# Lymphatus/caesium-clt

Hardware: AMD Instinct MI355X
Metric: megapixels/sec JPEG q=80 1920x1080 batch (higher is better)
Workload: dtype int32

## Files before the change

caesium-clt_amd/binding.py:

```python
import ctypes as C
import os

_HERE = os.path.dirname(os.path.abspath(__file__))
NPHASES = 8
NKERNELS = 36
PHASE_NAMES = ["decode", "pixel", "masks_flags_runs", "stats_tables", "sizes_scan", "pack", "stuff_assemble", "reserved"]


class CCSParameters(C.Structure):
    _fields_ = [("keep_metadata", C.c_bool), ("jpeg_quality", C.c_uint32), ("jpeg_chroma_subsampling", C.c_uint32),
                ("jpeg_progressive", C.c_bool), ("jpeg_optimize", C.c_bool), ("jpeg_preserve_icc", C.c_bool),
                ("png_quality", C.c_uint32), ("png_optimization_level", C.c_uint32), ("png_force_zopfli", C.c_bool),
                ("png_optimize", C.c_bool), ("gif_quality", C.c_uint32), ("webp_quality", C.c_uint32), ("webp_lossless", C.c_bool),
                ("tiff_compression", C.c_uint32), ("tiff_deflate_level", C.c_uint32), ("width", C.c_uint32), ("height", C.c_uint32)]


class CCSResult(C.Structure):
    _fields_ = [("success", C.c_bool), ("code", C.c_uint32), ("error_message", C.c_char_p)]


class CByteArray(C.Structure):
    _fields_ = [("data", C.POINTER(C.c_uint8)), ("length", C.c_size_t)]


class Timing(C.Structure):
    _fields_ = [("total_ms", C.c_float), ("phase_ms", C.c_float * NPHASES), ("kernel_ms", C.c_float * NKERNELS), ("in_bytes", C.c_uint64), ("out_bytes", C.c_uint64),
                ("pixels", C.c_uint64), ("coef_bytes", C.c_uint64), ("n_images", C.c_uint32), ("n_failed", C.c_uint32), ("n_seq_decoded", C.c_uint32), ("n_par_fallback", C.c_uint32), ("n_par_short", C.c_uint32), ("n_prog_decoded", C.c_uint32), ("n_refine_chains", C.c_uint32), ("n_search_extra", C.c_uint32), ("n_fused_lists", C.c_uint32), ("n_list_refine", C.c_uint32), ("n_ac_in_lists", C.c_uint32), ("n_list_runs", C.c_uint32)]


class PngTiming(C.Structure):
    _fields_ = [("total_ms", C.c_float), ("kernel_ms", C.c_float * 16), ("in_bytes", C.c_uint64), ("out_bytes", C.c_uint64), ("pixels", C.c_uint64),
                ("raw_bytes", C.c_uint64), ("n_images", C.c_uint32), ("n_failed", C.c_uint32), ("n_trials", C.c_uint32)]


class CaesiumError(RuntimeError):
    def __init__(self, code, message):
        super().__init__(f"[{code}] {message}")
        self.code = code


def library_path():
    return os.path.join(_HERE, "libcaesium_hip.so")


EXPORTS = ["cs_default_parameters", "cs_compress_in_memory", "cs_compress_to_size_in_memory", "cs_convert_in_memory",
           "cs_batch_compress", "cs_batch_extent", "cs_free_bytes", "cs_free_result", "csh_device_count", "csh_last_error", "csh_kernel_name", "csh_kernel_name_webp", "csh_release_cached_memory", "csh_warmup", "csh_batch_create",
           "csh_batch_run", "csh_batch_fetch", "csh_batch_destroy", "csh_batch_retain_dct", "csh_batch_set_quality", "csh_batch_rerun_encode", "cs_batch_compress_to_size", "csh_batch_geometry", "csh_batch_read_coefs",
           "csp_kernel_name", "csp_batch_create", "csp_batch_create_webp", "csp_batch_create_pixels", "csh_batch_create_pixels", "csh_batch_pixels", "csh_batch_create_from_pixels", "csp_png_to_jpeg", "csp_png_to_lossless_webp", "csp_batch_run", "csp_batch_fetch", "csp_batch_destroy", "csp_batch_geometry", "csp_batch_read_rows", "csp_batch_read_stream",
           "csp_batch_trials", "csp_batch_read_scores", "csp_batch_chunk_bits", "csh_batch_create_webp", "cs_batch_convert",
           "cswd_batch_create", "cswd_batch_run", "cswd_batch_pixels", "cswd_batch_read_pixels", "cswd_batch_alpha", "cswd_batch_read_rgba", "cswd_batch_destroy", "cswd_batch_frames", "cswd_batch_read_canvas", "cswd_batch_encode_anim", "cswd_rgba_join", "cswd_rgba_destroy", "csh_batch_create_webp_from_pixels", "csh_batch_create_from_pixels_rgb", "csl_encode_pixels", "csl_attach_alpha"]


def _declare(L):
    P = C.POINTER
    L.cs_default_parameters.argtypes = [P(CCSParameters)]
    L.cs_default_parameters.restype = None
    L.cs_compress_in_memory.argtypes = [C.c_char_p, C.c_size_t, P(CCSParameters), P(CByteArray)]
    L.cs_compress_in_memory.restype = CCSResult
    L.cs_compress_to_size_in_memory.argtypes = [C.c_char_p, C.c_size_t, P(CCSParameters), C.c_size_t, C.c_bool, P(CByteArray)]
    L.cs_compress_to_size_in_memory.restype = CCSResult
    L.cs_convert_in_memory.argtypes = [C.c_char_p, C.c_size_t, P(CCSParameters), C.c_uint32, P(CByteArray)]
    L.cs_convert_in_memory.restype = CCSResult
    L.cs_batch_compress.argtypes = [P(CByteArray), C.c_size_t, P(CCSParameters), C.c_int, P(CByteArray), P(CCSResult)]
    L.cs_batch_extent.argtypes = [P(CByteArray), C.c_size_t]
    L.cs_batch_extent.restype = C.c_size_t
    L.cs_free_bytes.argtypes = [P(CByteArray)]
    L.cs_free_bytes.restype = None
    L.cs_free_result.argtypes = [P(CCSResult)]
    L.cs_free_result.restype = None
    L.csh_last_error.restype = C.c_char_p
    L.csh_kernel_name.argtypes = [C.c_int]
    L.csh_kernel_name.restype = C.c_char_p
    L.csh_kernel_name_webp.argtypes = [C.c_int]
    L.csh_kernel_name_webp.restype = C.c_char_p
    L.csh_batch_create.argtypes = [P(CByteArray), C.c_size_t, P(CCSParameters), C.c_int, P(C.c_void_p)]
    L.csh_batch_run.argtypes = [C.c_void_p, P(Timing)]
    L.csh_batch_fetch.argtypes = [C.c_void_p, P(CByteArray), P(CCSResult)]
    L.csh_batch_retain_dct.argtypes = [C.c_void_p, C.c_int]
    L.csh_batch_set_quality.argtypes = [C.c_void_p, P(C.c_uint32)]
    L.csh_batch_rerun_encode.argtypes = [C.c_void_p, P(Timing)]
    L.cs_batch_compress_to_size.argtypes = [P(CByteArray), C.c_size_t, P(CCSParameters), C.c_size_t, C.c_bool, C.c_int, P(CByteArray), P(CCSResult)]
    L.csh_batch_destroy.argtypes = [C.c_void_p]
    L.csh_batch_destroy.restype = None
    L.csh_batch_geometry.argtypes = [C.c_void_p, C.c_size_t, C.c_int, C.c_int, P(C.c_int), P(C.c_int), P(C.c_int), P(C.c_int)]
    L.csh_batch_read_coefs.argtypes = [C.c_void_p, C.c_size_t, C.c_int, C.c_int, C.c_void_p]
    L.csh_batch_create_webp.argtypes = [P(CByteArray), C.c_size_t, P(CCSParameters), C.c_int, P(C.c_void_p)]
    L.cs_batch_convert.argtypes = [P(CByteArray), C.c_size_t, P(CCSParameters), C.c_uint32, C.c_int, P(CByteArray), P(CCSResult)]
    L.csp_kernel_name.argtypes = [C.c_int]
    L.csp_kernel_name.restype = C.c_char_p
    L.csp_batch_create.argtypes = [P(CByteArray), C.c_size_t, P(CCSParameters), C.c_int, P(C.c_void_p)]
    L.csp_batch_run.argtypes = [C.c_void_p, P(PngTiming)]
    L.csp_batch_fetch.argtypes = [C.c_void_p, P(CByteArray), P(CCSResult)]
    L.csp_batch_destroy.argtypes = [C.c_void_p]
    L.csp_batch_destroy.restype = None
    L.csp_batch_geometry.argtypes = [C.c_void_p, C.c_size_t, P(C.c_uint32), P(C.c_uint32), P(C.c_uint32)]
    L.csp_batch_read_rows.argtypes = [C.c_void_p, C.c_size_t, C.c_void_p]
    L.csp_batch_read_stream.argtypes = [C.c_void_p, C.c_size_t, C.c_int, C.c_void_p]
    L.csp_batch_read_scores.argtypes = [C.c_void_p, C.c_size_t, C.c_void_p, P(C.c_int)]
    L.csp_batch_chunk_bits.argtypes = [C.c_void_p, C.c_size_t, C.c_int, P(C.c_uint64), C.c_size_t, P(C.c_size_t)]
    L.csp_batch_trials.argtypes = [C.c_void_p, C.c_size_t, P(C.c_int), P(C.c_uint64), P(C.c_int), P(C.c_int)]
    L.cswd_batch_create.argtypes = [P(CByteArray), C.c_size_t, C.c_int, P(C.c_void_p)]
    L.cswd_batch_run.argtypes = [C.c_void_p]
    L.cswd_batch_pixels.argtypes = [C.c_void_p, C.c_size_t, P(C.c_void_p), P(C.c_uint32), P(C.c_uint32), P(C.c_uint32), P(C.c_char_p)]
    L.cswd_batch_read_pixels.argtypes = [C.c_void_p, C.c_size_t, C.c_void_p]
    L.cswd_batch_alpha.argtypes = [C.c_void_p, C.c_size_t, P(C.c_void_p), P(C.c_void_p)]
    L.cswd_batch_read_rgba.argtypes = [C.c_void_p, C.c_size_t, C.c_void_p]
    L.cswd_batch_destroy.argtypes = [C.c_void_p]
    L.cswd_batch_destroy.restype = None
    L.cswd_batch_frames.argtypes = [C.c_void_p, C.c_size_t, P(C.c_uint32), P(C.c_uint32), P(C.c_uint32)]
    L.cswd_batch_read_canvas.argtypes = [C.c_void_p, C.c_size_t, C.c_uint32, C.c_void_p]
# ... 381 lines not shown
```

caesium-clt_amd/csrc/batch.hpp:

```cpp
#pragma once
#include <array>
#include <chrono>
#include <map>
#include <string>
#include <vector>

#include "../../include/caesium_hip.h"
#include "devmem.hpp"
#include "jpeg_host.hpp"
#include "kernels.h"
#include "webp_kernels.h"

namespace csh {

struct Item {
    int code = 0;
    std::string msg;
    JpegInfo in;
    JpegInfo out;
    int image = -1;
    size_t file_size = 0;
    std::vector<uint8_t> meta_out;
};

struct DecodePlan {
    PinnedBytes bits_pool;
    std::vector<DecScan> dscans;
    std::vector<DevHuffSet> hsets;
    std::vector<ParHuffSet> phsets;
    std::vector<char> phset_fits;
    std::vector<ParHuffSet4> phsets4;
    std::vector<std::array<int8_t, 8>> slot4;
    bool use4 = true;
    std::vector<ParScan> pscans;
    std::vector<uint32_t> need_seq_init;
    std::vector<ProgChain> chains;
    std::vector<int> chain_scans;
    std::vector<RefineUnit> refine_units;
    uint32_t refine_hist = 0, refine_pos = 0, refine_max_blocks = 0;
    uint32_t total_sub = 0, max_sub = 0, max_par_blocks = 0, dc_total = 0;

    DevBuf<uint8_t> d_bits, d_clean;
    DevBuf<ParScan> d_pscans;
    DevBuf<uint64_t> d_pstate, d_relax_list[2], d_unstuff_off, d_blk_off, d_dc_off;
    DevBuf<uint32_t> d_unstuff_cnt, d_nblk, d_need_seq, d_need_seq_init, d_relax_cnt, d_scan_pending, d_cut_block, d_claim;
    DevBuf<uint16_t> d_hyp;
    DevBuf<int32_t> d_dcdiff;
    DevBuf<DecScan> d_dscans;
    DevBuf<ProgChain> d_chains;
    DevBuf<int> d_chain_scans;
    DevBuf<uint64_t> d_refine_hist;
    DevBuf<uint32_t> d_refine_pos, d_refine_prog;
    DevBuf<RefineUnit> d_refine_units;
    DevBuf<DevHuffSet> d_hsets;
    DevBuf<ParHuffSet> d_phsets;
    DevBuf<ParHuffSet4> d_phsets4;
};

struct PixelPlan {
    std::vector<PlaneWork> pwork;
    std::vector<ResizeWork> rwork;
    std::vector<ResizeTap> rtaps;
    std::vector<float> rweights;
    uint64_t rgb_bytes = 0, tmp_floats = 0, max_tmp = 0, max_dst = 0;
    uint32_t max_row_in = 0, max_out_w = 0, max_nh = 0;
    uint32_t max_src_px = 0;
    uint64_t plane_bytes = 0, oplane_bytes = 0;
    uint32_t max_quads = 0;
    bool any_layout = false, any_layout_rgb = false;
    bool any_space_rgb = false;

    DevBuf<uint8_t> d_planes, d_oplanes, d_rgb;
    DevBuf<PlaneWork> d_pwork;
    DevBuf<ResizeWork> d_rwork;
    DevBuf<ResizeTap> d_rtaps;
    DevBuf<float> d_rweights, d_rtmp;
    DevBuf<int16_t> d_dct_raw;
};

struct Stage {
    uint32_t work0 = 0, nwork = 0, slot0 = 0, nslots = 0, ech0 = 0, nech = 0, table0 = 0, ntables = 0, plan0 = 0, nplans = 0, nzc0 = 0, nnzc = 0, ls0 = 0, nls = 0, ts0 = 0, nts = 0, rs0 = 0, nrs = 0, lr0 = 0, nlr = 0, rr0 = 0, nrr = 0;
    bool nz_build[2] = {true, true}, nz_filter[2] = {true, true};
};
struct SearchImg {
    int cand_work[64]; int ncand;
    int Al_luma = 0, Al_chroma = 0;
    uint64_t best_luma = 0, best_chroma = 0;
    int split_luma = 0, split_chroma = 0;
    bool luma_on = false, chroma_on = false;
    bool fixed = false;
};

struct EncodePlan {
    std::vector<EncScan> script;
    std::vector<ScanWork> swork;
    uint32_t nslots = 0, nlist_slots = 0, ntok_slots = 0;
    uint32_t nref_slots = 0;
    uint32_t last_run_refine = 0;
    uint32_t list_run = CSH_LIST_RUN;
    uint32_t nlist_runs = 0, nref_runs = 0;
    bool ac_runs_slot = false;
    uint32_t last_run_list_runs = 0;
    uint64_t total_corr = 0;
    uint64_t total_units = 0, total_words = 0;
    uint32_t max_units = 0;
    int ntables = 0;
    std::vector<TokPlan> plans;
    std::vector<int> plan_comp, plan_image;
    std::vector<EChunk> echunks;
    uint64_t tok_cap = 0;
    uint32_t tok_scale = 1;
    std::vector<TokRegion> regions;
    std::vector<uint32_t> region_est;
    uint32_t hist_rows = 0;
    std::vector<NzList> nzlists;
    std::vector<NzSet> nzsets;
    std::vector<int> nzset_of;
    std::vector<uint32_t> nzset_built;
    std::vector<int> nzset_comp, nzset_image;
    std::vector<NzChunk> nzchunks;
    std::vector<NzChunk> nzchunks_fused;
    uint32_t n_fused = 0;
    uint32_t last_run_fused = 0;
    uint32_t n_ac_lists = 0;
    uint32_t last_run_ac_lists = 0;
    std::vector<uint8_t> nzset_ac_lists;
    std::vector<uint32_t> nz_est, nz_worst;
    uint32_t nz_nrec = 0;
    uint64_t nz_cap = 0;
    bool search = false;
    enum { ST_1 = 0, ST_1B = 1, ST_2 = 2, ST_2B = 3, ST_2C = 4, ST_N = 5 };
    Stage stage[ST_N];
    void stage_begin(Stage &sg) {
        sg.work0 = uint32_t(swork.size()); sg.slot0 = nslots; sg.ech0 = uint32_t(echunks.size()); sg.table0 = uint32_t(ntables); sg.plan0 = uint32_t(plans.size());
        sg.nzc0 = uint32_t(nzchunks.size()); sg.ls0 = nlist_slots; sg.ts0 = ntok_slots; sg.rs0 = nref_slots; sg.lr0 = nlist_runs; sg.rr0 = nref_runs;
    }
    void stage_end(Stage &sg) {
        sg.nwork = uint32_t(swork.size()) - sg.work0; sg.nslots = nslots - sg.slot0; sg.nech = uint32_t(echunks.size()) - sg.ech0;
        sg.ntables = uint32_t(ntables) - sg.table0; sg.nplans = uint32_t(plans.size()) - sg.plan0;
        sg.nnzc = uint32_t(nzchunks.size()) - sg.nzc0; sg.nls = nlist_slots - sg.ls0; sg.nts = ntok_slots - sg.ts0; sg.nrs = nref_slots - sg.rs0; sg.nlr = nlist_runs - sg.lr0; sg.nrr = nref_runs - sg.rr0;
    }
    std::vector<SearchImg> simg;
    std::vector<uint8_t> work_active;
    uint32_t n_gated_runs = 0;
    std::vector<uint32_t> img_list, img_nlist, h_cost;
    std::map<std::array<int, 5>, int> cand_script;
    std::vector<uint8_t> hdr_pool;
    std::vector<uint32_t> hdr_off;

    DevBuf<uint8_t> d_hdr, d_tail, d_scan_tmp, d_work_active;
    DevBuf<EncScan> d_script;
    DevBuf<ScanWork> d_swork;
    DevBuf<uint32_t> d_slot_work;
    DevBuf<EChunk> d_echunks;
    DevBuf<SlotRec> d_slots;
    DevBuf<TokPlan> d_plans;
    DevBuf<uint64_t> d_corr, d_symbits, d_eobbits, d_tok_off, d_chunk_off, d_scan_raw_off;
    DevBuf<uint32_t> d_tok_cursor;
    DevBuf<TokRegion> d_regions;
    DevBuf<uint16_t> d_eobrun, d_slot_hist;
    DevBuf<uint32_t> d_img_list, d_img_nlist, d_scan_cost, d_slot_raw, d_slot_eobh, d_long_runs, d_long_cnt, d_tokens, d_chunk_ntok, d_chunk_bits, d_raw, d_scan_pad, d_chunk_ff, d_hdr_off;
    DevBuf<DevEncTable> d_tables;
    DevBuf<NzList> d_nzlists;
    DevBuf<NzSet> d_nzsets;
    DevBuf<NzChunk> d_nzchunks, d_nzchunks_fused;
    DevBuf<uint32_t> d_nz_pool, d_nz_cursor, d_nz_chunk_off, d_nz_chunk_cnt, d_list_slots, d_tok_slots, d_ref_slots, d_list_runs, d_ref_runs;
};

struct TrellisPlan {
    bool trellis = false, dering = false;
    Stage tstage;
    std::vector<TrellisWork> twork;
    std::vector<TrellisRun> truns;
    uint32_t t_units = 0, t_max_rows = 0;
    std::vector<uint32_t> trows;
    bool t_sort = false;
    bool nz_once = false;

    DevBuf<TrellisWork> d_twork;
    DevBuf<TrellisRun> d_truns;
    DevBuf<uint32_t> d_tqueue, d_trows, d_tperm, d_tspill;
    DevBuf<uint8_t> d_tblk_cnt;
    DevBuf<uint16_t> d_tblk_off;
    DevBuf<uint64_t> d_tlambda, d_tdcbt;
};

struct WebpTail {
    uint32_t webp_mb_bytes = 768;
    std::vector<csw::WebpImg> wimgs;
    uint64_t wwork_bytes = 0, wlevels = 0;
    uint32_t wmax_luma = 0, wmax_mbh = 0;

    DevBuf<csw::WebpImg> d_wimgs;
    DevBuf<uint8_t> d_wwork, d_wscratch, d_wprobs, d_wupdate;
    DevBuf<uint32_t> d_wpart, d_wstats;
    DevBuf<int16_t> d_wlevels;
};

struct Outputs {
    uint64_t raw_bytes_cap = 0, out_cap = 0;
    DevBuf<uint8_t> d_out;
    DevBuf<uint64_t> d_img_off;
    DevBuf<uint32_t> d_img_size, d_img_size_pad, d_status, d_overflow;
    std::vector<uint32_t> h_img_size;
    std::vector<uint64_t> h_img_off;
    std::vector<uint32_t> h_status;
    bool ran = false;
};

}

struct csh_batch {
    int device = 0;
    hipStream_t stream = 0;
    bool have_stream = false;
    CCSParameters params;
    std::vector<csh::Item> items;
    int nimg = 0;
    bool lossless = false;
    bool rgb_out = false;
    bool webp = false;
    int test_pool_shift = -1;
    bool progressive = true;
    bool retain_dct = false;
    bool have_dct = false;
    int q_base = 0;

    std::vector<csh::ImgDesc> imgs;
    std::vector<csh::DevQuant> quants;
    uint32_t ntiles = 0, ntiles_in = 0, ntiles_out = 0, max_tiles = 0, max_dummy = 0;
    csh::DevBuf<csh::ImgDesc> d_imgs;
    csh::DevBuf<csh::DevQuant> d_quants;
    csh::DevBuf<int16_t> d_coef;

    csh::DecodePlan dec;
    csh::PixelPlan pix;
    csh::EncodePlan enc;
    csh::TrellisPlan tr;
    csh::WebpTail wp;
    csh::Outputs out;

    ~csh_batch() { if (have_stream) { (void)hipStreamSynchronize(stream); (void)hipStreamDestroy(stream); } }
};

namespace csh {

enum KernelSlot {
    KS_MEMSET_COEF, KS_UNSTUFF, KS_DEC_SPEC, KS_DEC_RELAX0, KS_DEC_RELAX, KS_DEC_WRITE, KS_DC_SCATTER, KS_REFINE_CHAINS, KS_DECODE_PROG_SEQ,
    KS_IDCT_PLANE, KS_RESIZE, KS_XFORM_DIRECT, KS_RESAMPLE_FDCT, KS_FIX_DUMMY, KS_MEMSET_ENC, KS_TRELLIS_STATS, KS_TRELLIS_AC, KS_TRELLIS_DC,
    KS_NZLIST, KS_TOKENS, KS_LIST_STATS, KS_AC_RUNS, KS_GEN_TABLES, KS_CHUNK_SIZES, KS_SCAN_CHUNK_BITS, KS_SCAN_LAYOUT, KS_PACK, KS_LIST_PACK,
    KS_FF_COUNT, KS_SCAN_SEARCH, KS_LAYOUT, KS_SCAN_IMAGES, KS_EMIT, KS_SPARE0, KS_SPARE1, KS_SPARE2, KS_COUNT,
    KS_WEBP_YUV = KS_XFORM_DIRECT, KS_WEBP_ENCODE = KS_RESAMPLE_FDCT, KS_WEBP_ASSEMBLE = KS_FIX_DUMMY
};
struct KernelSlotRow { KernelSlot slot; const char *name; int phase; };
constexpr KernelSlotRow kKernelSlots[] = {
    {KS_MEMSET_COEF, "memset_coef", 0},        {KS_UNSTUFF, "unstuff", 0},                 {KS_DEC_SPEC, "k_dec_spec", 0},
    {KS_DEC_RELAX0, "k_dec_relax0", 0},        {KS_DEC_RELAX, "k_dec_relax1_4", 0},        {KS_DEC_WRITE, "k_dec_write", 0},
    {KS_DC_SCATTER, "k_dc_scatter", 0},        {KS_REFINE_CHAINS, "k_refine_chains", 0},   {KS_DECODE_PROG_SEQ, "k_decode_prog+seq", 0},
    {KS_IDCT_PLANE, "k_idct_plane", 1},        {KS_RESIZE, "resize", 1},                   {KS_XFORM_DIRECT, "k_xform_direct", 1},
    {KS_RESAMPLE_FDCT, "k_resample+k_plane_fdct", 1}, {KS_FIX_DUMMY, "k_fix_dummy", 1},    {KS_MEMSET_ENC, "memset_enc", 2},
    {KS_TRELLIS_STATS, "trellis_stats", 1},    {KS_TRELLIS_AC, "k_trellis_ac", 1},         {KS_TRELLIS_DC, "k_trellis_dc", 1},
    {KS_NZLIST, "k_nzlist", 2},                {KS_TOKENS, "k_tokens", 2},                 {KS_LIST_STATS, "k_list_stats", 2},
    {KS_AC_RUNS, "k_ac_runs", 2},              {KS_GEN_TABLES, "k_gen_tables", 3},         {KS_CHUNK_SIZES, "k_chunk_sizes", 4},
    {KS_SCAN_CHUNK_BITS, "scan_chunk_bits", 4}, {KS_SCAN_LAYOUT, "scan_layout", 4},        {KS_PACK, "k_pack", 5},
    {KS_LIST_PACK, "k_list_pack", 5},          {KS_FF_COUNT, "k_ff_count", 6},             {KS_SCAN_SEARCH, "scan_search_stage2", 7},
    {KS_LAYOUT, "k_layout", 6},                {KS_SCAN_IMAGES, "scan_images", 6},         {KS_EMIT, "k_emit", 6},
    {KS_SPARE0, "", 7},                        {KS_SPARE1, "", 7},                         {KS_SPARE2, "", 7}};
constexpr bool kernel_slots_in_order() {
    for (int i = 0; i < int(sizeof kKernelSlots / sizeof kKernelSlots[0]); i++) if (kKernelSlots[i].slot != i) return false;
    return true;
}
static_assert(sizeof kKernelSlots / sizeof kKernelSlots[0] == CSH_NKERNELS && int(KS_COUNT) == int(CSH_NKERNELS), "one row per csh_timing.kernel_ms slot");
static_assert(kernel_slots_in_order(), "row i of kKernelSlots describes slot i");

struct PlanSwitches {
    std::string profile;
    bool nz_once = true;
    bool tr_sort = true;
    int prog_par = -1;
    bool fused_420 = true;
    bool nz_fused = true;
    bool ref_list = true;
    uint32_t list_run = CSH_LIST_RUN;
    bool ac_runs_slot = false;
    bool ac_tiles = false;
    static PlanSwitches read();
};

struct Laps {
    const bool trace;
    std::chrono::steady_clock::time_point at = std::chrono::steady_clock::now();
    std::string text;
    Laps();
    void lap(const char *what);
};

struct BatchPlanner {
    csh_batch *const b;
    const CByteArray *const inputs;
    const size_t count;
    const CCSParameters *const p;
    const csp_pixels *const px;
    const PlanSwitches sw;
    const bool progressive;
    uint16_t qout_nat[64];
    int script_base3 = 0, script_base1 = 0;
    std::map<int, int> other_scripts;
    std::vector<std::pair<std::vector<uint8_t>, int>> hset_keys;
    std::map<std::vector<uint16_t>, int> quant_index;
    uint64_t plane_off = 64, oplane_off = 0;

    BatchPlanner(csh_batch *b, const CByteArray *inputs, size_t count, const CCSParameters *p, const csp_pixels *px);
    void begin();
    void parse();
    int reserve_pinned();
    int plan_image(size_t n);
    int plan_search_stages();
    int plan_trellis();
    void finish_descriptors();
    int upload(Laps &laps);

private:
    void image_geometry(Item &it, ImgDesc &im);
    int decode_scans(Item &it, ImgDesc &im, const uint8_t *d);
    int huff_set(const JScan &js);
    void place_blocks(ParScan &ps, const JpegInfo &in, const JScan &js, uint32_t units, bool dc_rows, bool subseqs);
    int sequential_split(const Item &it, const ImgDesc &im, const uint8_t *d, int img_index, bool &par_ok);
    bool progressive_plan(const Item &it, const ImgDesc &im, int img_index);
    void plane_work(ImgDesc &im, const JpegInfo &in, const JpegInfo &o, int img_index, bool resized);
    void resize_work(const JpegInfo &in, const JpegInfo &o, int img_index);
    void output_scans(Item &it, ImgDesc &im, int img_index, size_t in_len);
    void frame_header(Item &it);
    template <class Fill> int enc_scan(const std::array<int, 5> &key, Fill fill);
    int space_script(int ncomp, int space, int &ns);
    int cand_index(int comp, int Ss, int Se, int Ah, int Al, int cls = -1);
    int dc_scan_index(int ncomp);
    int seq1_index(int comp, int cls = -1);
    uint32_t nz_list(int img_index, int comp, int Al, const ImgDesc &im, size_t in_len);
    void add_works(Item &it, ImgDesc &im, int img_index, const std::vector<int> &list, size_t in_len, const JpegInfo &o, bool stats_only = false);
    template <class Make> void add_stage(int sid, Make make);
    template <class Add> void splits(const ImgDesc &im, Add &add, int i0, int i1, bool whole);
};

void layout_token_pool(csh_batch *b);

int run_once(csh_batch *b, csh_timing *t, bool requant_only);

int search_costs(csh_batch *b, AsmCtx &a, int stage);
uint32_t search_gate(csh_batch *b, int stage, int (*want)(const SearchImg &));
int search_decide(csh_batch *b, int stage);
int search_lists(csh_batch *b);

}
```

caesium-clt_amd/csrc/batch_plan.cpp:

```cpp
#include <algorithm>
#include <atomic>
#include <cmath>
#include <thread>

#include "batch.hpp"
#include "resize_host.h"
#include "result.h"

namespace csh {

static void build_dev_huff(const HuffSpec &h, DevHuff &d) {
    memset(&d, 0, sizeof d);
    for (int l = 0; l < 18; l++) d.maxcode[l] = -1;
    if (!h.present) return;
    int code = 0, p = 0;
    for (int l = 1; l <= 16; l++) {
        if (h.bits[l]) {
            d.valptr[l] = p - code;
            for (int i = 0; i < h.bits[l]; i++, p++, code++)
                if (l <= 9) {
                    int base = code << (9 - l);
                    for (int k = 0; k < (1 << (9 - l)); k++) d.look[(base + k) & 511] = uint16_t((l << 8) | h.vals[p]);
                }
            d.maxcode[l] = code - 1;
// ... 114 lines not shown
static int plan_item(Item &it, const CCSParameters &p, bool lossless, bool to_rgb) {
    const JpegInfo &in = it.in;
    if (in.ncomp != 1 && in.ncomp != 3 && in.ncomp != 4) { it.msg = "unsupported component count"; return CS_ERR_JPEG_FEATURE; }
    if (uint64_t(in.width) * uint64_t(in.height) > (1ull << 28)) { it.msg = "image dimensions too large for the device path"; return CS_ERR_JPEG_FEATURE; }
    const bool other_space = in.space != CSH_CS_GREY && in.space != CSH_CS_YCC;
    const bool converted = other_space && to_rgb;
    it.out = JpegInfo();
    JpegInfo &o = it.out;
    o.width = in.width; o.height = in.height; o.ncomp = converted ? 3 : in.ncomp;
    o.space = converted ? CSH_CS_YCC : in.space;
    if (other_space && !converted) { o.write_jfif = false; o.write_adobe = in.adobe_transform; }
    if (p.width || p.height) {
        if (lossless) { it.msg = "resize + lossless transcode not on the device path"; return CS_ERR_UNSUPPORTED; }
        csh_compute_dimensions(in.width, in.height, int(p.width), int(p.height), o.width, o.height);
        if (o.width > 65500 || o.height > 65500 || uint64_t(o.width) * uint64_t(o.height) > (1ull << 28)) { it.msg = "resize target too large for JPEG"; return CS_ERR_JPEG_FEATURE; }
    }
    if (in.ncomp >= 3 && (!lossless || in.ncomp == 4)) {
        int blocks = 0;
        for (int c = 0; c < in.ncomp; c++) {
            const JComp &k = in.comp[c];
            blocks += k.h * k.v;
            if (in.hmax % k.h || in.vmax % k.v) { it.msg = "fractional chroma sampling ratio (component factors do not divide the largest ones)"; return CS_ERR_JPEG_FEATURE; }
            if (in.hmax / k.h > 4 || in.vmax / k.v > 4) { it.msg = "chroma sampling ratio above 4"; return CS_ERR_JPEG_FEATURE; }
        }
        if (blocks > 10) { it.msg = "more than 10 blocks per MCU"; return CS_ERR_JPEG_FEATURE; }
    }
    if (lossless) {
        for (int c = 0; c < in.ncomp; c++)
            if (memcmp(in.comp[c].qt, in.qt[in.comp[c].tq], sizeof in.comp[c].qt)) { it.msg = "a component was decoded with a quantisation table that its slot no longer holds"; return CS_ERR_JPEG_FEATURE; }
        for (int c = 0; c < in.ncomp; c++) o.comp[c] = in.comp[c];
        jpeg_geometry(o);
        return 0;
    }
    int ss = int(p.jpeg_chroma_subsampling);
    if (ss == 0) ss = 420;
    static const char kRgbIds[] = "RGB", kCmykIds[] = "CMYK";
    for (int c = 0; c < o.ncomp; c++) {
        o.comp[c].id = o.space == CSH_CS_RGB ? kRgbIds[c] : (o.space == CSH_CS_CMYK ? kCmykIds[c] : c + 1);
        o.comp[c].h = o.comp[c].v = 1; o.comp[c].tq = table_class(o.space, c);
    }
    if (o.space == CSH_CS_YCC || o.space == CSH_CS_YCCK) {
        int h = 1, v = 1;
        if (ss == 420) { h = 2; v = 2; }
        else if (ss == 422) { h = 2; v = 1; }
        else if (ss == 411) { h = 4; v = 1; }
        else if (ss != 444) { it.msg = "unknown output chroma subsampling"; return CS_ERR_JPEG_FEATURE; }
        o.comp[0].h = h; o.comp[0].v = v;
        if (o.space == CSH_CS_YCCK) { o.comp[3].h = h; o.comp[3].v = v; }
    }
    jpeg_geometry(o);
    return 0;
}

void layout_token_pool(csh_batch *b) {
    b->enc.regions.resize(b->enc.region_est.size());
    if (b->test_pool_shift < 0) b->test_pool_shift = getenv("CSH_TEST_POOL_SHIFT") ? std::min(16, std::max(0, atoi(getenv("CSH_TEST_POOL_SHIFT")))) : 0;
    const int shift = b->test_pool_shift;
    uint64_t at = 0;
    for (size_t i = 0; i < b->enc.regions.size(); i++) {
        const uint64_t cap = std::min<uint64_t>(std::max<uint64_t>((uint64_t(b->enc.region_est[i]) * b->enc.tok_scale) >> shift, 64), 0xFFFFFFF0ull);
        b->enc.regions[i].base = at; b->enc.regions[i].cap = uint32_t(cap); b->enc.regions[i].pad = 0;
        at += (cap + 3) & ~uint64_t(3);
    }
    b->enc.tok_cap = at + 64;
    at = 0;
    for (size_t i = 0; i < b->enc.nzlists.size(); i++) {
        const uint64_t cap = std::min<uint64_t>(std::max<uint64_t>((uint64_t(b->enc.nz_est[i]) * b->enc.tok_scale) >> shift, 64), b->enc.nz_worst[i]);
        b->enc.nzlists[i].base = at; b->enc.nzlists[i].cap = uint32_t(cap);
        at += (cap + 3) & ~uint64_t(3);
    }
    b->enc.nz_cap = at + 64;
}

PlanSwitches PlanSwitches::read() {
    auto is = [](const char *name, const char *v) { const char *e = getenv(name); return e && !strcmp(e, v); };
    PlanSwitches s;
    const char *penv = getenv("CSH_PROFILE");
    s.profile = penv && *penv ? penv : "mozjpeg";
    s.nz_once = !is("CSH_NZ_ONCE", "0");
    s.tr_sort = !is("CSH_TR_SORT", "0");
    s.nz_fused = !is("CSH_NZ_FUSED", "0");
    s.ac_tiles = is("CSH_AC_TILES", "1");
    s.ref_list = is("CSH_REF_LIST", "1") || (s.ref_list && !is("CSH_REF_LIST", "0"));
    const char *pp = getenv("CSH_PROG_PAR");
    s.prog_par = pp && !strcmp(pp, "0") ? 0 : (pp && !strcmp(pp, "1") ? 1 : -1);
    s.fused_420 = !getenv("CSH_NO_FUSED_420");
    if (const char *lr = getenv("CSH_LIST_RUN")) { if (*lr) s.list_run = uint32_t(std::min(32, std::max(1, atoi(lr)))); }
    s.ac_runs_slot = is("CSH_AC_RUNS", "slot");
    return s;
}

Laps::Laps() : trace(getenv("CSH_TRACE") != nullptr) {}
void Laps::lap(const char *what) {
    if (!trace) return;
    const auto now = std::chrono::steady_clock::now();
    char buf[64];
    snprintf(buf, sizeof buf, " %s %.1f", what, std::chrono::duration<double, std::milli>(now - at).count());
    text += buf; at = now;
}

BatchPlanner::BatchPlanner(csh_batch *b_, const CByteArray *inputs_, size_t count_, const CCSParameters *p_, const csp_pixels *px_)
    : b(b_), inputs(inputs_), count(count_), p(p_), px(px_), sw(PlanSwitches::read()), progressive(p_->jpeg_progressive) {}

void BatchPlanner::begin() {
    b->items.resize(count);
    quality_table(int(p->jpeg_quality), qout_nat);
    DevQuant qo; make_quant(qout_nat, qo);
    b->quants.push_back(qo);
    b->q_base = int(b->quants.size()) - 1;
    for (int q = 1; q <= 100; q++) { uint16_t tq[64]; quality_table(q, tq); DevQuant dq; make_quant(tq, dq); b->quants.push_back(dq); }
    b->progressive = progressive;
    b->enc.list_run = sw.list_run;
    b->enc.ac_runs_slot = sw.ac_runs_slot;

    add_script(b->enc.script, 3, true, CSH_CS_YCC);
    add_script(b->enc.script, 1, true, CSH_CS_GREY);
    add_script(b->enc.script, 3, false, CSH_CS_YCC);
    add_script(b->enc.script, 1, false, CSH_CS_GREY);
    script_base3 = progressive ? 0 : 16; script_base1 = progressive ? 10 : 17;
    const bool webp = b->webp, rgb_out = b->rgb_out;
    const std::string &profile = sw.profile;
    b->enc.search = progressive && !webp && !rgb_out && profile != "plain";
    const bool lossy_jpeg = !b->lossless && !webp && !rgb_out;
    b->tr.trellis = lossy_jpeg && (profile == "mozjpeg" || profile == "mozjpeg-trellis");
    b->tr.dering = lossy_jpeg && (profile == "mozjpeg" || profile == "mozjpeg-dering");
    b->tr.nz_once = b->tr.trellis && progressive && sw.nz_once && sw.tr_sort;
}

template <class Fill>
int BatchPlanner::enc_scan(const std::array<int, 5> &key, Fill fill) {
    auto f = b->enc.cand_script.find(key);
    if (f != b->enc.cand_script.end()) return f->second;
    EncScan e;
    memset(&e, 0, sizeof e);
    fill(e);
    b->enc.script.push_back(e);
    return b->enc.cand_script[key] = int(b->enc.script.size()) - 1;
}
int BatchPlanner::space_script(int ncomp, int space, int &ns) {
    ns = progressive ? (space == CSH_CS_YCC ? 10 : 2 + 4 * ncomp) : 1;
    if (space == CSH_CS_YCC) return script_base3;
    if (space == CSH_CS_GREY) return script_base1;
    auto f = other_scripts.find(space);
    if (f == other_scripts.end()) {
        f = other_scripts.emplace(space, int(b->enc.script.size())).first;
        add_script(b->enc.script, ncomp, progressive, space);
    }
    return f->second;
}
int BatchPlanner::cand_index(int comp, int Ss, int Se, int Ah, int Al, int cls) {
    const int ycc = comp ? 1 : 0;
    if (cls < 0) cls = ycc;
    return enc_scan({cls == ycc ? comp : comp + 16 * (1 + cls), Ss, Se, Ah, Al}, [&](EncScan &e) {
        const int id = cls;
        e.ncomp = 1; e.comp[0] = comp; e.Ss = Ss; e.Se = Se; e.Ah = Ah; e.Al = Al;
        e.ntables = 1; e.dht_id[0] = 0x10 | id; e.sos_tdta[0] = id;
    });
}
int BatchPlanner::dc_scan_index(int ncomp) {
    return enc_scan({-ncomp, 0, 0, 0, 0}, [&](EncScan &e) {
        e.ncomp = ncomp;
        for (int k = 0; k < ncomp; k++) {
            e.comp[k] = k;
            const int id = k ? 1 : 0;
            int idx = -1;
            for (int t = 0; t < e.ntables; t++) if (e.dht_id[t] == id) idx = t;
            if (idx < 0) { idx = e.ntables; e.dht_id[e.ntables++] = id; }
            e.dc_tbl[k] = idx; e.sos_tdta[k] = id << 4;
        }
    });
}
int BatchPlanner::seq1_index(int comp, int cls) {
    const int ycc = comp ? 1 : 0;
    if (cls < 0) cls = ycc;
    return enc_scan({cls == ycc ? comp : comp + 16 * (1 + cls), 0, 63, -1, -1}, [&](EncScan &e) {
        const int id = cls;
        e.ncomp = 1; e.comp[0] = comp; e.Ss = 0; e.Se = 63; e.sequential = 1;
        e.ntables = 2; e.dht_id[0] = id; e.dht_id[1] = 0x10 | id; e.dc_tbl[0] = 0; e.ac_tbl[0] = 1; e.sos_tdta[0] = (id << 4) | id;
    });
}

static uint64_t blocks_of(const ImgDesc &im) {
    uint64_t n = 0;
    for (int k = 0; k < im.ncomp; k++) n += uint64_t(im.out[k].real_bw) * im.out[k].real_bh;
    return n;
}

uint32_t BatchPlanner::nz_list(int img_index, int comp, int Al, const ImgDesc &im, size_t in_len) {
    if (b->enc.nzset_of.size() < size_t(img_index + 1) * CSH_MAX_COMPS) b->enc.nzset_of.resize(size_t(img_index + 1) * CSH_MAX_COMPS, -1);
    int &si = b->enc.nzset_of[size_t(img_index) * CSH_MAX_COMPS + size_t(comp)];
    const uint32_t nu = uint32_t(im.out[comp].real_bw * im.out[comp].real_bh);
    if (si < 0) {
        NzSet S;
        memset(&S, 0, sizeof S);
        for (int L = 0; L < CSH_NZ_LEVELS; L++) S.list[L] = 0xFFFFFFFFu;
        S.cnt_base = 0xFFFFFFFFu;
        S.nunits = nu; S.real_bw = im.out[comp].real_bw; S.bw = im.out[comp].bw; S.tile_base = im.out[comp].tile_base;
        si = int(b->enc.nzsets.size());
        b->enc.nzsets.push_back(S); b->enc.nzset_built.push_back(0u); b->enc.nzset_comp.push_back(comp); b->enc.nzset_image.push_back(img_index);
    }
    const uint64_t blocks_all = blocks_of(im);
    static const uint32_t kShare[CSH_NZ_LEVELS] = {20, 16, 12, 9};
    for (int L : {0, Al}) {
        if (b->enc.nzsets[size_t(si)].list[L] != 0xFFFFFFFFu) continue;
        const uint32_t nch = (nu + 255) / 256;
        NzList R;
        memset(&R, 0, sizeof R);
        R.chunk0 = b->enc.nz_nrec; b->enc.nz_nrec += nch;
        b->enc.nzsets[size_t(si)].list[L] = uint32_t(b->enc.nzlists.size());
        b->enc.nzlists.push_back(R);
        const uint64_t est = uint64_t(in_len) * kShare[L] / 8 * nu / std::max<uint64_t>(1, blocks_all) + nu + 4ull * nch + 256;
        const uint64_t worst = uint64_t(nu) * 64 + 4ull * nch;
        b->enc.nz_est.push_back(uint32_t(std::min<uint64_t>(est, worst)));
        b->enc.nz_worst.push_back(uint32_t(std::min<uint64_t>(worst, 0xFFFFFFF0ull)));
    }
    return b->enc.nzsets[size_t(si)].list[Al];
}

void BatchPlanner::add_works(Item &it, ImgDesc &im, int img_index, const std::vector<int> &list, size_t in_len, const JpegInfo &o, bool stats_only) {
    const int w_first = int(b->enc.swork.size());
    uint32_t nz_need[CSH_MAX_COMPS] = {0, 0, 0}, nz_gate[CSH_MAX_COMPS] = {0, 0, 0};
    for (int sidx : list) {
        const EncScan &e = b->enc.script[sidx];
        ScanWork w;
        memset(&w, 0, sizeof w);
        w.image = img_index; w.scan = sidx;
        w.out_off = 0xFFFFFFFFu;
        const bool from_list = e.Ss > 0 && !e.sequential && e.Ah == 0;
        const bool ref_list = sw.ref_list && e.Ss > 0 && !e.sequential && e.Ah != 0;
        w.list = 0xFFFFFFFFu; w.rs_base = 0xFFFFFFFFu; w.lr_base = 0xFFFFFFFFu; w.rr_base = 0xFFFFFFFFu;
        if (from_list || ref_list) {
            if (e.Al >= CSH_NZ_LEVELS) { it.code = CS_ERR_JPEG_FEATURE; it.msg = "internal: output scan script outside what the list coder carries"; }
            else {
                w.list = nz_list(img_index, e.comp[0], e.Al, im, in_len);
                if (!nz_need[e.comp[0]]) nz_gate[e.comp[0]] = uint32_t(b->enc.swork.size());
                nz_need[e.comp[0]] |= 1u << e.Al;
            }
        }
        if (e.Ss == 0 && e.ncomp > 1) w.nunits = uint32_t(im.omcus_x * im.omcus_y);
        else w.nunits = uint32_t(im.out[e.comp[0]].real_bw * im.out[e.comp[0]].real_bh);
        w.unit_base = uint32_t(b->enc.total_units);
        b->enc.total_units += w.nunits;
        w.corr_base = 0xFFFFFFFFu;
        if (e.Ss > 0 && !e.sequential && e.Ah) { w.corr_base = uint32_t(b->enc.total_corr); b->enc.total_corr += w.nunits; }
        w.word_base = uint32_t(b->enc.total_words);
        if (e.Ss) b->enc.total_words += (w.nunits + 63) / 64;
        w.table_base = uint32_t(b->enc.ntables);
        b->enc.ntables += e.ntables;
        b->enc.max_units = std::max(b->enc.max_units, w.nunits);
        {
            const uint32_t nch = (w.nunits + 255) / 256;
            w.first_chunk = b->enc.nslots; b->enc.nslots += nch;
            w.hist_row0 = b->enc.hist_rows; b->enc.hist_rows += nch * uint32_t(e.ntables);
            uint32_t &cursor = (from_list && w.list != 0xFFFFFFFFu) ? b->enc.nlist_slots : b->enc.ntok_slots;
            w.ls_base = cursor; cursor += nch;
            if (ref_list && w.list != 0xFFFFFFFFu) { w.rs_base = b->enc.nref_slots; b->enc.nref_slots += nch; }
            const uint32_t nruns = (nch + b->enc.list_run - 1) / b->enc.list_run;
            if (from_list && w.list != 0xFFFFFFFFu) { w.lr_base = b->enc.nlist_runs; b->enc.nlist_runs += nruns; }
            if (ref_list && w.list != 0xFFFFFFFFu) { w.rr_base = b->enc.nref_runs; b->enc.nref_runs += nruns; }
        }
        if (e.Ss == 0 || e.sequential) {
            uint32_t blocks = 0;
            for (int k = 0; k < e.ncomp; k++) blocks += e.ncomp > 1 ? uint32_t(o.comp[e.comp[k]].h * o.comp[e.comp[k]].v) : 1u;
            const uint32_t per_unit = e.sequential ? blocks * 20u : (e.Ah ? (blocks + 14u) / 15u : blocks);
            for (uint32_t j = 0; j < (w.nunits + 255) / 256; j++) b->enc.echunks.push_back(EChunk{uint32_t(b->enc.swork.size()), 0, 1, j, 0, uint32_t(b->enc.region_est.size())});
            b->enc.region_est.push_back(stats_only ? 64u : w.nunits * per_unit + 64);
        }
        b->enc.swork.push_back(w);
    }
    for (int c = 0; c < im.ncomp; c++) {
        if (!nz_need[c]) continue;
        const int si = b->enc.nzset_of[size_t(img_index) * CSH_MAX_COMPS + size_t(c)];
        uint32_t levels = stats_only ? (nz_need[c] | 1u) : ((nz_need[c] | 1u) & ~b->enc.nzset_built[size_t(si)]);
        b->enc.nzset_built[size_t(si)] |= levels;
        if (!stats_only && b->tr.nz_once && (levels & 1u)) levels = (levels & ~1u) | CSH_NZ_COMPACT0;
        const uint32_t nu = b->enc.nzsets[size_t(si)].nunits;
        for (uint32_t j = 0; levels && j < (nu + 255) / 256; j++) b->enc.nzchunks.push_back(NzChunk{uint32_t(si), j, levels, nz_gate[c]});
    }
    for (int c = 0; c < im.ncomp; c++) {
        int nac = 0;
        for (int sidx : list) { const EncScan &e = b->enc.script[sidx]; if (e.Ss > 0 && !e.sequential && e.Ah && e.comp[0] == c) { nac++; if (e.Al > 3 && !sw.ref_list) nac = 99; } }
        const bool too_many = !sw.ref_list && nac > CSH_TK_MAXSLOT;
        if (too_many) { it.code = CS_ERR_JPEG_FEATURE; it.msg = "internal: output scan script outside what the token kernel carries"; }
        const uint32_t nu = uint32_t(im.out[c].real_bw * im.out[c].real_bh);
        if (!nac || too_many) continue;
        const uint64_t blocks_all = blocks_of(im);
        const uint64_t scripts = b->enc.search ? uint64_t(nac + 1) / 2 : 1;
        const uint64_t est = uint64_t(in_len) * 3 * scripts * nu / std::max<uint64_t>(1, blocks_all) + uint64_t(nu) * nac + 1024;
        if (sw.ref_list) {
            for (size_t k = 0; k < list.size(); k++) {
                const EncScan &e = b->enc.script[list[k]];
                if (e.Ss > 0 && !e.sequential && e.Ah && e.comp[0] == c && b->enc.swork[size_t(w_first) + k].rs_base != 0xFFFFFFFFu) b->enc.swork[size_t(w_first) + k].region = uint32_t(b->enc.region_est.size());
            }
            b->enc.region_est.push_back(stats_only ? 64u : uint32_t(std::min<uint64_t>(est, 0x3FFFFFFFu)));
            continue;
        }
        TokPlan P;
        memset(&P, 0, sizeof P);
        P.nunits = nu; P.real_bw = im.out[c].real_bw; P.bw = im.out[c].bw; P.tile_base = im.out[c].tile_base;
        P.work0 = 0xFFFFFFFFu;
        for (size_t k = 0; k < list.size(); k++) {
            const EncScan &e = b->enc.script[list[k]];
            if (!(e.Ss > 0 && !e.sequential && e.Ah && e.comp[0] == c)) continue;
            const ScanWork &w = b->enc.swork[size_t(w_first) + k];
            if (P.work0 == 0xFFFFFFFFu) P.work0 = uint32_t(w_first) + uint32_t(k);
            AcSlot &a = P.s[P.nslot++];
            a.unit_base = w.unit_base; a.word_base = w.word_base; a.first_chunk = w.first_chunk; a.table_base = w.table_base; a.nunits_work = w.nunits; a.corr_base = w.corr_base;
            a.Ss = uint8_t(e.Ss); a.Se = uint8_t(e.Se); a.Ah = uint8_t(e.Ah); a.Al = uint8_t(e.Al);
        }
        for (uint32_t j = 0; j < (nu + 255) / 256; j++) b->enc.echunks.push_back(EChunk{uint32_t(img_index), uint16_t(c), 0, j, uint32_t(b->enc.plans.size()), uint32_t(b->enc.region_est.size())});
        b->enc.region_est.push_back(stats_only ? 64u : uint32_t(std::min<uint64_t>(est, 0x3FFFFFFFu)));
        b->enc.plan_comp.push_back(c); b->enc.plan_image.push_back(img_index);
        b->enc.plans.push_back(P);
    }
}

void BatchPlanner::parse() {
    std::atomic<size_t> next{0};
    auto worker = [&]() {
        for (size_t n; (n = next++) < count;) {
            Item &it = b->items[n];
            it.file_size = inputs[n].length;
            int type = sniff(inputs[n].data, inputs[n].length);
            if (type == CS_TYPE_UNKN) { it.code = CS_ERR_UNKNOWN_TYPE; it.msg = "unknown file type"; }
            else if (type != CS_TYPE_JPEG) { it.code = CS_ERR_UNSUPPORTED; it.msg = "this input format has no device path in this build (built: JPEG, PNG)"; }
            else it.code = parse_jpeg(inputs[n].data, inputs[n].length, it.in, it.msg);
        }
    };
    size_t nthreads = std::min<size_t>(std::min<size_t>(16, std::max(1u, std::thread::hardware_concurrency())), (count + 15) / 16);
    std::vector<std::thread> pool;
    for (size_t t = 1; t < nthreads; t++) pool.emplace_back(worker);
    worker();
    for (auto &t : pool) t.join();
}

int BatchPlanner::reserve_pinned() {
    size_t total = 0;
    for (size_t n = 0; n < count; n++) total += inputs[n].length;
    if (total + total / 16 + (64u << 10) >= 0xF0000000ull) { csh_set_error("csh_batch_create: more than 3.75 GiB of input in one device batch (cs_batch_extent sizes groups)"); return CS_ERR_POOL_OVERFLOW; }
    if (!b->dec.bits_pool.reserve(total + total / 16 + (64u << 10))) { csh_set_error("out of pinned host memory"); return CS_ERR_NO_DEVICE; }
    return 0;
}

void BatchPlanner::image_geometry(Item &it, ImgDesc &im) {
    const JpegInfo &in = it.in, &o = it.out;
    im.width = in.width; im.height = in.height; im.ncomp = o.ncomp; im.ncomp_in = in.ncomp;
    im.mcus_x = in.mcus_x; im.mcus_y = in.mcus_y;
    im.progressive_in = in.progressive;
    for (int c = 0; c < in.ncomp; c++) {
        fill_geom(in.comp[c], im.in[c], b->ntiles_in);
        std::vector<uint16_t> key(in.comp[c].qt, in.comp[c].qt + 64);
        auto f = quant_index.find(key);
        if (f == quant_index.end()) {
            DevQuant q; make_quant(key.data(), q);
            f = quant_index.emplace(key, int(b->quants.size())).first;
            b->quants.push_back(q);
        }
        im.qt_in[c] = f->second;
        b->max_tiles = std::max<uint32_t>(b->max_tiles, im.in[c].ntiles);
    }
    for (int c = 0; c < o.ncomp; c++) {
        if (b->lossless) im.out[c] = im.in[c];
        else fill_geom(o.comp[c], im.out[c], b->ntiles_out);
        im.comp_id[c] = o.comp[c].id;
        im.qt_out[c] = 0;
        b->max_tiles = std::max<uint32_t>(b->max_tiles, im.out[c].ntiles);
        uint32_t nd = uint32_t(im.out[c].bw * im.out[c].bh - im.out[c].real_bw * im.out[c].real_bh);
        b->max_dummy = std::max(b->max_dummy, nd);
    }
    im.omcus_x = o.mcus_x; im.omcus_y = o.mcus_y;
    im.enc_w = o.width; im.enc_h = o.height;
// ... 529 lines not shown
    for (size_t i = 0; i < b->enc.nzsets.size(); i++) b->enc.nzsets[i].tile_base = b->imgs[size_t(b->enc.nzset_image[i])].out[b->enc.nzset_comp[i]].tile_base;
    {
        b->enc.nzchunks_fused = b->enc.nzchunks;
        const bool allowed = sw.nz_fused && !b->lossless && !b->webp && !b->rgb_out && !(b->tr.trellis && progressive && !b->tr.nz_once);
        std::vector<uint8_t> fused(b->enc.nzsets.size(), 0);
        const bool lists_only = progressive && !sw.ac_tiles && sw.ref_list && sw.nz_once && sw.tr_sort && (!b->tr.trellis || (b->tr.t_sort && b->tr.nz_once));
        std::vector<uint8_t> planned(b->enc.nzsets.size(), 0);
        for (size_t i = 0; i < b->enc.plans.size(); i++) {
            const size_t at = size_t(b->enc.plan_image[i]) * CSH_MAX_COMPS + size_t(b->enc.plan_comp[i]);
            if (at < b->enc.nzset_of.size() && b->enc.nzset_of[at] >= 0) planned[size_t(b->enc.nzset_of[at])] = 1;
        }
        b->enc.nzset_ac_lists.assign(b->enc.nzsets.size(), 0);
        for (PlaneWork &w : b->pix.pwork) {
            w.ac_lists = 0u;
            const size_t at = size_t(w.image) * CSH_MAX_COMPS + size_t(w.comp);
            const int si = allowed && at < b->enc.nzset_of.size() ? b->enc.nzset_of[at] : -1;
            if (si < 0) continue;
            const NzSet &S = b->enc.nzsets[size_t(si)];
            if (S.real_bw != S.bw || S.list[0] == 0xFFFFFFFFu) continue;
            w.nzset = uint32_t(si); fused[size_t(si)] = 1; b->enc.n_fused++;
            if (lists_only && !planned[size_t(si)]) { w.ac_lists = 1u; b->enc.nzset_ac_lists[size_t(si)] = 1; b->enc.n_ac_lists++; }
        }
        for (TrellisWork &tw : b->tr.twork) tw.ac_lists = (tw.nzset != 0xFFFFFFFFu && b->enc.nzset_ac_lists[tw.nzset]) ? 1u : 0u;
        for (NzChunk &ch : b->enc.nzchunks_fused) if (fused[ch.set]) ch.levels &= ~1u;
        auto flags = [&](Stage &sg) {
            for (int f = 0; f < 2; f++) {
                const std::vector<NzChunk> &v = f ? b->enc.nzchunks_fused : b->enc.nzchunks;
                sg.nz_build[f] = sg.nz_filter[f] = false;
                for (uint32_t i = sg.nzc0; i < sg.nzc0 + sg.nnzc; i++) { sg.nz_build[f] |= (v[i].levels & 1u) != 0u; sg.nz_filter[f] |= (v[i].levels & ~1u) != 0u; }
            }
        };
        for (Stage &sg : b->enc.stage) flags(sg);
        flags(b->tr.tstage);
    }
    for (ParScan &ps : b->dec.pscans)
        for (int m = 0; m < ps.nb_mcu && m < 10; m++) {
            int dcs = ps.dct[m] & 3, acs = 4 + (ps.act[m] & 3);
            if (b->dec.use4) { dcs = std::max<int>(0, b->dec.slot4[ps.huff_set][dcs]); acs = std::max<int>(0, b->dec.slot4[ps.huff_set][acs]); }
            ps.sel |= uint64_t(dcs | (acs << 3)) << (6 * m);
        }
    {
        std::vector<int> last(b->dec.chains.size(), -1);
        for (int s = 0;; s++) {
            bool any = false;
            for (size_t c = 0; c < b->dec.chains.size(); c++)
                if (b->dec.chains[c].refine && b->dec.chains[c].count > s) {
                    RefineUnit u; u.chain = int(c); u.s = s; u.prev = last[c];
                    last[c] = int(b->dec.refine_units.size());
                    b->dec.refine_units.push_back(u);
                    any = true;
                }
            if (!any) break;
        }
    }
    b->ntiles = b->ntiles_in + b->ntiles_out;
    b->pix.plane_bytes = plane_off;
    b->pix.oplane_bytes = oplane_off;
    b->out.out_cap = b->out.raw_bytes_cap;
    layout_token_pool(b);
}

int BatchPlanner::upload(Laps &laps) {
    hipStream_t st = b->stream;
    if (!b->nimg) return 0;
    b->dec.bits_pool.flush_copies();
    laps.lap("copy_in");
    if (b->dec.d_bits.alloc(b->dec.bits_pool.size()) || (b->dec.bits_pool.size() && hipMemcpyAsync(b->dec.d_bits.p, b->dec.bits_pool.p, b->dec.bits_pool.size(), hipMemcpyHostToDevice, st) != hipSuccess) ||
        b->d_imgs.upload(b->imgs, st) || b->dec.d_dscans.upload(b->dec.dscans, st) || b->dec.d_chains.upload(b->dec.chains, st) || b->dec.d_chain_scans.upload(b->dec.chain_scans, st) ||
        b->dec.d_hsets.upload(b->dec.hsets, st) || b->dec.d_phsets.upload(b->dec.phsets, st) || (b->dec.use4 && b->dec.d_phsets4.upload(b->dec.phsets4, st)) || b->d_quants.upload(b->quants, st) || b->pix.d_pwork.upload(b->pix.pwork, st) ||
        b->enc.d_script.upload(b->enc.script, st) || b->enc.d_swork.upload(b->enc.swork, st) || b->enc.d_slot_work.alloc(size_t(b->enc.nslots) + 1) || b->enc.d_slots.alloc(size_t(b->enc.nslots) + 1) || b->enc.d_plans.upload(b->enc.plans, st) || b->enc.d_echunks.upload(b->enc.echunks, st) || b->enc.d_hdr.upload(b->enc.hdr_pool, st) ||
        b->enc.d_hdr_off.upload(b->enc.hdr_off, st) || b->dec.d_pscans.upload(b->dec.pscans, st) || b->pix.d_rwork.upload(b->pix.rwork, st) || b->pix.d_rtaps.upload(b->pix.rtaps, st) ||
        b->pix.d_rweights.upload(b->pix.rweights, st) || b->pix.d_rgb.alloc(b->pix.rgb_bytes + 64) || b->pix.d_rtmp.alloc((resize_is_fused(b->pix.max_row_in) ? 0 : b->pix.tmp_floats) + 16) || b->dec.d_need_seq_init.upload(b->dec.need_seq_init, st))
        return CS_ERR_NO_DEVICE;
    size_t nchunks = b->dec.bits_pool.size() / 64 + 1, nst = size_t(b->dec.total_sub) + b->dec.pscans.size() + 1;
    if (b->dec.d_clean.alloc(b->dec.bits_pool.size() + 64) || b->dec.d_unstuff_cnt.alloc(nchunks + 1) || b->dec.d_unstuff_off.alloc(nchunks + 2) ||
        b->dec.d_pstate.alloc(nst) || b->dec.d_relax_list[0].alloc(nst) || b->dec.d_relax_list[1].alloc(nst) || b->dec.d_relax_cnt.alloc(512) || b->dec.d_scan_pending.alloc(b->dec.pscans.size() + 1) || b->dec.d_cut_block.alloc(b->dec.pscans.size() + 1) || b->dec.d_claim.alloc(size_t(b->dec.total_sub) + 1) || b->dec.d_hyp.alloc((size_t(b->dec.total_sub) + 1) * 10) ||
        b->dec.d_nblk.alloc(size_t(b->dec.total_sub) + 1) || b->dec.d_blk_off.alloc(size_t(b->dec.total_sub) + 2) || b->dec.d_need_seq.alloc(b->nimg + 1) ||
        b->dec.d_dcdiff.alloc(size_t(b->dec.dc_total) + 1) || b->dec.d_dc_off.alloc(size_t(b->dec.dc_total) + 2) ||
        b->dec.d_refine_hist.alloc(size_t(b->dec.refine_hist) + 1) || b->dec.d_refine_pos.alloc(size_t(b->dec.refine_pos) + 1) || b->dec.d_refine_units.upload(b->dec.refine_units, st) ||
        b->dec.d_refine_prog.alloc(b->dec.refine_units.size() + 1))
        return CS_ERR_NO_DEVICE;
    if (b->d_coef.alloc(size_t(b->ntiles) * CSH_TILE_I16) || b->pix.d_planes.alloc(b->pix.plane_bytes + 64) || b->pix.d_oplanes.alloc(b->pix.oplane_bytes + 64) ||
        b->enc.d_symbits.alloc(b->enc.total_words + 1) || b->enc.d_eobbits.alloc(b->enc.total_words + 1) ||
        b->enc.d_long_runs.alloc(2 * (b->enc.total_units / 512 + b->enc.swork.size() + 16)) || b->enc.d_long_cnt.alloc(4) || b->enc.d_tail.alloc(b->enc.total_units + 1) || b->enc.d_eobrun.alloc(b->enc.total_units + 1) || b->enc.d_corr.alloc(b->enc.total_corr + 1) ||
        b->enc.d_tok_off.alloc(4 * size_t(b->enc.nslots) + 4) || b->enc.d_chunk_ntok.alloc(4 * size_t(b->enc.nslots) + 4) || b->enc.d_slot_hist.alloc(size_t(b->enc.hist_rows) * 256 + 256) ||
        b->enc.d_slot_raw.alloc(size_t(b->enc.nslots) + 1) || b->enc.d_img_list.upload(b->enc.img_list, st) || b->enc.d_img_nlist.upload(b->enc.img_nlist, st) || b->enc.d_scan_cost.alloc(b->enc.swork.size() + 1) || b->enc.d_slot_eobh.alloc(16 * size_t(b->enc.nslots) + 16) || b->enc.d_chunk_bits.alloc(size_t(b->enc.nslots) + 1) || b->enc.d_chunk_off.alloc(size_t(b->enc.nslots) + 2) || b->enc.d_tok_cursor.alloc(b->enc.region_est.size() + 1) || b->enc.d_regions.upload(b->enc.regions, st) ||
        b->enc.d_tables.alloc(b->enc.ntables) || b->enc.d_scan_pad.alloc(b->enc.swork.size() + 1) ||
        b->enc.d_nzlists.upload(b->enc.nzlists, st) || b->enc.d_nzsets.upload(b->enc.nzsets, st) || b->enc.d_nzchunks.upload(b->enc.nzchunks, st) || (b->enc.n_fused && b->enc.d_nzchunks_fused.upload(b->enc.nzchunks_fused, st)) || b->enc.d_list_slots.alloc(size_t(b->enc.nlist_slots) + 1) || b->enc.d_tok_slots.alloc(size_t(b->enc.ntok_slots) + 1) || b->enc.d_ref_slots.alloc(size_t(b->enc.nref_slots) + 1) || b->enc.d_list_runs.alloc(size_t(b->enc.nlist_runs) + 1) || b->enc.d_ref_runs.alloc(size_t(b->enc.nref_runs) + 1) ||
        b->enc.d_nz_cursor.alloc(b->enc.nzlists.size() + 1) || b->enc.d_nz_chunk_off.alloc(size_t(b->enc.nz_nrec) + 1) || b->enc.d_nz_chunk_cnt.alloc(size_t(b->enc.nz_nrec) + 1) ||
        b->enc.d_scan_raw_off.alloc(b->enc.swork.size() + 2) || b->out.d_img_size.alloc(b->nimg + 1) || b->out.d_img_size_pad.alloc(b->nimg + 1) ||
        b->out.d_img_off.alloc(b->nimg + 2) || b->out.d_status.alloc(b->nimg) || b->out.d_overflow.alloc(4))
        return CS_ERR_NO_DEVICE;
    if (hipMemsetAsync(b->enc.d_slots.p, 0, (size_t(b->enc.nslots) + 1) * sizeof(SlotRec), st) != hipSuccess ||
        hipMemsetAsync(b->enc.d_slot_work.p, 0, (size_t(b->enc.nslots) + 1) * sizeof(uint32_t), st) != hipSuccess) { csh_set_error("hipMemsetAsync failed"); return CS_ERR_NO_DEVICE; }
    launch_make_slots(st, b->enc.d_swork.p, uint32_t(b->enc.swork.size()), b->enc.d_script.p, b->enc.d_nzlists.p, b->enc.d_slots.p, b->enc.d_slot_work.p, b->enc.d_list_slots.p, b->enc.d_tok_slots.p, b->enc.d_ref_slots.p, b->enc.d_list_runs.p, b->enc.d_ref_runs.p, b->enc.list_run);
    if (b->tr.trellis && (b->tr.d_trows.upload(b->tr.trows, st) || (b->tr.t_sort && (b->tr.d_tperm.alloc(size_t(b->tr.t_units) + 1) || b->tr.d_tblk_cnt.alloc(size_t(b->tr.t_units) + 1) || (b->tr.nz_once && b->tr.d_tblk_off.alloc(size_t(b->tr.t_units) + 1)))))) return CS_ERR_NO_DEVICE;
    if (b->tr.trellis && (b->tr.d_twork.upload(b->tr.twork, st) || b->tr.d_truns.upload(b->tr.truns, st) || b->tr.d_tqueue.alloc(1) || b->tr.d_tlambda.alloc(size_t(b->tr.t_units) + 1) || b->tr.d_tdcbt.alloc(size_t(b->tr.t_units) + 1) ||
                       b->tr.d_tspill.alloc(trellis_spill_words(trellis_ac_slots())) || b->pix.d_dct_raw.alloc(size_t(b->ntiles_out) * CSH_TILE_I16)))
        return CS_ERR_NO_DEVICE;
    for (size_t n = 0; px && n < count; n++) {
        const Item &it = b->items[n];
        if (it.image < 0) continue;
        const ResizeWork &rw = b->pix.rwork[size_t(it.image)];
        if (rw.image != it.image) { csh_set_error("internal: resize work out of order"); return CS_ERR_NO_DEVICE; }
        if (hipMemcpyAsync(b->pix.d_rgb.p + rw.rgb_src_off, px[n].device_pixels, size_t(px[n].width) * px[n].height * px[n].channels, hipMemcpyDeviceToDevice, st) != hipSuccess) { csh_set_error("pixel copy failed"); return CS_ERR_NO_DEVICE; }
    }
    laps.lap("alloc+enqueue");
    if (hipStreamSynchronize(st) != hipSuccess) { csh_set_error("upload failed"); return CS_ERR_NO_DEVICE; }
    laps.lap("upload_wait");
    return 0;
}

}
```

caesium-clt_amd/csrc/batch_run.cpp:

```cpp
#include <algorithm>

#include "batch.hpp"

namespace csh {
namespace {

class KernelMarks {
    hipEvent_t ev[CSH_NKERNELS + 1];
    int created = 0, next = 0;
    const hipStream_t st;

public:
    explicit KernelMarks(hipStream_t s) : st(s) {}
    KernelMarks(const KernelMarks &) = delete;
    KernelMarks &operator=(const KernelMarks &) = delete;
    ~KernelMarks() { for (int i = 0; i < created; i++) (void)hipEventDestroy(ev[i]); }
    int start() {
        for (; created <= CSH_NKERNELS; created++) CSH_CHECK(hipEventCreate(&ev[created]));
        CSH_CHECK(hipEventRecord(ev[0], st));
        return 0;
    }
    int claim(KernelSlot slot, hipEvent_t *e) {
        if (int(slot) != next || next >= CSH_NKERNELS) {
            csh_set_error("internal: timing mark '%s' out of order (slot %d is next)", slot < KS_COUNT ? kKernelSlots[slot].name : "?", next);
// ... 102 lines not shown
                eobrun_cleared = b->enc.d_eobrun.n != 0;
            }
            launch_dec_dense(st, 1, nps, b->dec.max_sub, da);
            da.zero_bytes = 0; da.zero2_bytes = 0;
            MARK(KS_DEC_RELAX0);
            const int kMaxRounds = int(b->dec.d_relax_cnt.n) - 2;
            int R = 0;
            for (int group = 12; nps && R < kMaxRounds; group = 8) {
                for (int g = 0; g < group && R < kMaxRounds; g++, R++)
                    launch_dec_relax_list(st, b->dec.d_clean.p, b->dec.d_pscans.p, b->dec.total_sub, da.huffs, da.compact, b->dec.d_pstate.p, b->dec.d_nblk.p, b->dec.d_relax_list[R & 1].p,
                                          b->dec.d_relax_cnt.p + R, b->dec.d_relax_list[(R & 1) ^ 1].p, b->dec.d_relax_cnt.p + R + 1, b->dec.d_pstate.n, b->dec.d_claim.p, uint32_t(R + 1));
                uint32_t left = 0;
                CSH_CHECK(hipMemcpyAsync(&left, b->dec.d_relax_cnt.p + R, sizeof left, hipMemcpyDeviceToHost, st));
                CSH_CHECK(hipStreamSynchronize(st));
                if (!left) break;
            }
            if (nps) {
                if (b->dec.d_scan_pending.zero(st)) return -1;
                launch_dec_mark_pending(st, b->dec.d_pscans.p, b->dec.total_sub, b->dec.d_relax_list[R & 1].p, b->dec.d_relax_cnt.p + R, b->dec.d_scan_pending.p);
                da.hyp = b->dec.d_hyp.p; da.scan_pending = b->dec.d_scan_pending.p;
                launch_dec_dense(st, 3, nps, b->dec.max_sub, da);
                launch_dec_chain(st, b->dec.d_pscans.p, nps, b->dec.d_pstate.p, b->dec.d_nblk.p, b->dec.d_hyp.p, b->dec.d_scan_pending.p, b->dec.d_need_seq.p);
            }
            MARK(KS_DEC_RELAX);
            if (nps) launch_exclusive_scan(st, b->dec.d_nblk.p, b->dec.d_blk_off.p, b->dec.total_sub, b->enc.d_scan_tmp.p, b->enc.d_scan_tmp.n);
            launch_dec_dense(st, 2, nps, b->dec.max_sub, da);
            MARK(KS_DEC_WRITE);
            if (nps) launch_exclusive_scan(st, reinterpret_cast<uint32_t *>(b->dec.d_dcdiff.p), b->dec.d_dc_off.p, b->dec.dc_total, b->enc.d_scan_tmp.p, b->enc.d_scan_tmp.n);
            launch_dc_scatter(st, b->dec.d_pscans.p, nps, b->dec.max_par_blocks, b->d_imgs.p, b->dec.d_dc_off.p, b->d_coef.p, b->dec.d_need_seq.p, b->dec.d_cut_block.p);
            launch_dc_refine(st, b->dec.d_clean.p, b->dec.d_pscans.p, nps, b->dec.max_par_blocks, b->d_imgs.p, b->d_coef.p, b->dec.d_need_seq.p);
            MARK(KS_DC_SCATTER);
        }
        launch_refine_chains(st, b->dec.d_clean.p, b->dec.d_pscans.p, b->dec.d_phsets.p, b->dec.d_dscans.p, b->dec.d_chains.p, b->dec.d_chain_scans.p, int(b->dec.chains.size()), b->dec.d_refine_units.p,
                             int(b->dec.refine_units.size()), b->dec.refine_max_blocks, b->d_imgs.p, b->d_coef.p, b->dec.d_need_seq.p, b->dec.d_refine_hist.p, b->dec.d_refine_pos.p, b->dec.d_refine_prog.p);
        MARK(KS_REFINE_CHAINS);
        launch_decode_prog(st, b->dec.d_clean.p, b->dec.d_pscans.p, b->dec.d_phsets.p, b->dec.d_dscans.p, b->dec.d_chains.p, b->dec.d_chain_scans.p, int(b->dec.chains.size()), b->d_imgs.p,
                           b->d_coef.p, b->dec.d_need_seq.p);
        launch_decode_seq(st, b->dec.d_bits.p, b->d_imgs.p, b->dec.d_dscans.p, b->dec.d_hsets.p, b->d_coef.p, nimg, b->dec.d_need_seq.p);
        MARK(KS_DECODE_PROG_SEQ);
        return 0;
    }

    int planes() {
        int nw = b->lossless ? 0 : int(b->pix.pwork.size());
        launch_idct_plane(st, b->d_imgs.p, b->pix.d_pwork.p, nw, b->max_tiles, b->d_quants.p, b->d_coef.p, b->pix.d_planes.p);
        MARK(KS_IDCT_PLANE);
        launch_resize(st, b->d_imgs.p, b->pix.d_rwork.p, int(b->pix.rwork.size()), b->pix.d_rtaps.p, b->pix.d_rweights.p, b->pix.d_planes.p, b->pix.d_rgb.p, b->pix.d_rtmp.p,
                      b->pix.max_src_px, b->pix.max_tmp, b->pix.max_dst, b->pix.max_row_in, b->pix.max_out_w, b->pix.max_nh, !(b->webp || b->rgb_out), b->pix.any_layout_rgb, b->pix.any_space_rgb);
        MARK(KS_RESIZE);
        return 0;
    }
    int pixels() {
        const int nw = b->lossless ? 0 : int(b->pix.pwork.size());
        int16_t *rawp = ((b->retain_dct || b->tr.trellis) && !b->lossless) ? b->pix.d_dct_raw.p : nullptr;
        NzFuse nzf;
        memset(&nzf, 0, sizeof nzf);
        fused = nw && b->enc.n_fused;
        if (fused) {
            if (b->enc.d_nz_cursor.zero(st) || b->enc.d_nz_chunk_cnt.zero(st)) return -1;
            nzf.nzsets = b->enc.d_nzsets.p; nzf.nzlists = b->enc.d_nzlists.p; nzf.nz_pool = b->enc.d_nz_pool.p; nzf.nz_cursor = b->enc.d_nz_cursor.p;
            nzf.nz_chunk_off = b->enc.d_nz_chunk_off.p; nzf.nz_chunk_cnt = b->enc.d_nz_chunk_cnt.p; nzf.overflow = b->out.d_overflow.p;
            nzf.blk_cnt = (b->tr.trellis && b->tr.t_sort) ? b->tr.d_tblk_cnt.p : nullptr;
            nzf.blk_off = (nzf.blk_cnt && b->tr.nz_once) ? b->tr.d_tblk_off.p : nullptr;
        }
        if (nw && getenv("CSH_DEBUG") && (uint32_t(atoi(getenv("CSH_DEBUG"))) & 32768u))
            CSH_CHECK(hipMemsetAsync(b->d_coef.p + size_t(b->ntiles_in) * CSH_TILE_I16, 0x5A, size_t(b->ntiles - b->ntiles_in) * CSH_TILE_I16 * sizeof(int16_t), st));
        launch_xform_direct(st, b->d_imgs.p, b->pix.d_pwork.p, nw, b->max_tiles, b->d_quants.p, b->d_coef.p, b->d_coef.p, rawp, b->ntiles_in, b->tr.dering, nzf);
        MARK(KS_XFORM_DIRECT);
        launch_resample_plane(st, b->d_imgs.p, b->pix.d_pwork.p, nw, b->pix.max_quads, b->pix.d_planes.p, b->pix.d_oplanes.p);
        if (b->pix.any_layout) launch_resample_any(st, b->d_imgs.p, b->pix.d_pwork.p, nw, b->pix.max_quads, b->pix.d_planes.p, b->pix.d_oplanes.p);
        launch_plane_fdct(st, b->d_imgs.p, b->pix.d_pwork.p, nw, b->max_tiles, b->d_quants.p, b->pix.d_oplanes.p, b->d_coef.p, rawp, b->ntiles_in, b->tr.dering, nzf);
        launch_resample_fdct_420(st, b->d_imgs.p, b->pix.d_pwork.p, nw, b->max_tiles, b->d_quants.p, b->pix.d_planes.p, b->d_coef.p, rawp, b->ntiles_in, b->tr.dering, nzf);
        MARK(KS_RESAMPLE_FDCT);
        if (!b->lossless) launch_fix_dummy(st, b->d_imgs.p, nimg, b->max_dummy, b->d_coef.p);
        MARK(KS_FIX_DUMMY);
        return 0;
    }

    void fill_enc_ctx() {
        memset(&c, 0, sizeof c);
        c.imgs = b->d_imgs.p; c.script = b->enc.d_script.p; c.work = b->enc.d_swork.p; c.nwork = int(b->enc.swork.size());
        c.echunks = b->enc.d_echunks.p; c.plans = b->enc.d_plans.p; c.nechunks = uint32_t(b->enc.echunks.size()); c.slot_work = b->enc.d_slot_work.p; c.slots = b->enc.d_slots.p; c.nslots = b->enc.nslots;
        c.coef = b->d_coef.p; c.sym_bits = b->enc.d_symbits.p; c.eob_bits = b->enc.d_eobbits.p; c.tail = b->enc.d_tail.p;
        c.eobrun = b->enc.d_eobrun.p; c.long_runs = b->enc.d_long_runs.p; c.long_cnt = b->enc.d_long_cnt.p; c.corr = b->enc.d_corr.p;
        c.tokens = b->enc.d_tokens.p; c.regions = b->enc.d_regions.p; c.tok_cursor = b->enc.d_tok_cursor.p; c.tok_off = b->enc.d_tok_off.p; c.chunk_ntok = b->enc.d_chunk_ntok.p; c.slot_hist = b->enc.d_slot_hist.p; c.slot_raw = b->enc.d_slot_raw.p; c.slot_eobh = b->enc.d_slot_eobh.p;
        c.chunk_bits = b->enc.d_chunk_bits.p; c.chunk_off = b->enc.d_chunk_off.p; c.tables = b->enc.d_tables.p;
        c.raw = b->enc.d_raw.p; c.raw_words = raw_chunks * 16; c.status = b->out.d_status.p; c.overflow = b->out.d_overflow.p;
        c.nzlists = b->enc.d_nzlists.p; c.nzsets = b->enc.d_nzsets.p; c.nz_pool = b->enc.d_nz_pool.p; c.nz_cursor = b->enc.d_nz_cursor.p; c.nz_chunk_off = b->enc.d_nz_chunk_off.p; c.nz_chunk_cnt = b->enc.d_nz_chunk_cnt.p;
        c.debug = getenv("CSH_DEBUG") ? uint32_t(atoi(getenv("CSH_DEBUG"))) : 0u;
    }
    void fill_asm_ctx() {
        memset(&a, 0, sizeof a);
        a.imgs = b->d_imgs.p; a.script = b->enc.d_script.p; a.work = b->enc.d_swork.p; a.nimg = nimg;
        a.nwork = b->tr.trellis ? int(b->tr.tstage.work0) : c.nwork;
        a.tables = b->enc.d_tables.p; a.chunk_off = b->enc.d_chunk_off.p; a.scan_pad_bytes = b->enc.d_scan_pad.p; a.scan_raw_off = b->enc.d_scan_raw_off.p;
        a.raw = b->enc.d_raw.p; a.raw_chunks = raw_chunks; a.chunk_ff = b->enc.d_chunk_ff.p;
        a.hdr_pool = b->enc.d_hdr.p; a.hdr_off = b->enc.d_hdr_off.p; a.img_size = b->out.d_img_size.p; a.img_size_pad = b->out.d_img_size_pad.p;
        a.img_off = b->out.d_img_off.p; a.out = b->out.d_out.p; a.out_cap = b->out.out_cap; a.status = b->out.d_status.p; a.overflow = b->out.d_overflow.p;
        a.img_list = b->enc.d_img_list.p; a.img_nlist = b->enc.d_img_nlist.p; a.scan_cost = b->enc.d_scan_cost.p;
    }
    void fill_trellis_ctx(TrellisCtx &tc) {
        memset(&tc, 0, sizeof tc);
        tc.imgs = b->d_imgs.p; tc.quant = b->d_quants.p; tc.work = b->tr.d_twork.p; tc.nwork = int(b->tr.twork.size()); tc.runs = b->tr.d_truns.p; tc.nruns = uint32_t(b->tr.truns.size());
        tc.tables = b->enc.d_tables.p; tc.raw = b->pix.d_dct_raw.p; tc.raw_tile0 = b->ntiles_in; tc.coef = b->d_coef.p; tc.dcrec = b->tr.d_tlambda.p; tc.dcbt = b->tr.d_tdcbt.p;
        tc.spill = b->tr.d_tspill.p; tc.nslots = uint32_t(b->tr.d_tspill.n / trellis_spill_words(1)); tc.max_rows = b->tr.t_max_rows;
        tc.queue = b->tr.d_tqueue.p;
        tc.rows = b->tr.d_trows.p; tc.nrows = uint32_t(b->tr.trows.size());
        if (b->tr.t_sort) { tc.blk_cnt = b->tr.d_tblk_cnt.p; tc.perm = b->tr.d_tperm.p; }
        if (b->tr.t_sort && b->tr.nz_once) {
            tc.nz_pool = b->enc.d_nz_pool.p; tc.nzlists = b->enc.d_nzlists.p; tc.nzsets = b->enc.d_nzsets.p; tc.nz_chunk_off = b->enc.d_nz_chunk_off.p; tc.nz_chunk_cnt = b->enc.d_nz_chunk_cnt.p;
            tc.blk_off = b->tr.d_tblk_off.p;
        }
        tc.ac_lists = fused ? 1u : 0u;
        tc.debug = getenv("CSH_TR_DEBUG") ? uint32_t(atoi(getenv("CSH_TR_DEBUG"))) : 0u;
    }

    int encode_begin() {
        fill_enc_ctx();
        launch_reset_works(st, b->enc.d_swork.p, c.nwork);
        if (!fused && (b->enc.d_nz_cursor.zero(st) || b->enc.d_nz_chunk_cnt.zero(st))) return -1;
        if (b->enc.d_symbits.zero(st) || b->enc.d_eobbits.zero(st) || (!eobrun_cleared && b->enc.d_eobrun.zero(st)) || b->enc.d_tables.zero(st) || b->enc.d_tok_cursor.zero(st) || b->enc.d_slot_eobh.zero(st) || b->enc.d_scan_pad.zero(st)) return -1;
#ifdef CSH_EMUL
        if (b->enc.d_raw.zero(st)) return -1;
#else
        if ((c.debug & 8192u) && b->enc.d_raw.zero(st)) return -1;
#endif
        MARK(KS_MEMSET_ENC);
        return 0;
    }

    void count_list_runs(const Stage &sg, bool gate) {
        for (uint32_t wi = sg.work0; (sg.nlr || sg.nrr) && wi < sg.work0 + sg.nwork; wi++) {
            const ScanWork &w = b->enc.swork[wi];
            if ((w.lr_base != 0xFFFFFFFFu || w.rr_base != 0xFFFFFFFFu) && (!gate || b->enc.work_active[wi])) b->enc.last_run_list_runs += ((w.nunits + 255u) / 256u + b->enc.list_run - 1u) / b->enc.list_run;
        }
    }

    void set_stage(const Stage &sg) {
        c.echunks = b->enc.d_echunks.p + sg.ech0; c.nechunks = sg.nech; c.slot0 = sg.slot0; c.nslots = sg.nslots;
        c.nzchunks = (fused ? b->enc.d_nzchunks_fused.p : b->enc.d_nzchunks.p) + sg.nzc0; c.nnzchunks = sg.nnzc;
        c.nz_build = sg.nz_build[fused ? 1 : 0]; c.nz_filter = sg.nz_filter[fused ? 1 : 0];
        c.list_slots = b->enc.d_list_slots.p + sg.ls0; c.nlist_slots = sg.nls; c.tok_slots = b->enc.d_tok_slots.p + sg.ts0; c.ntok_slots = sg.nts;
        c.ref_slots = b->enc.d_ref_slots.p + sg.rs0; c.nref_slots = sg.nrs;
        c.list_runs = b->enc.d_list_runs.p + sg.lr0; c.nlist_runs = sg.nlr; c.ref_runs = b->enc.d_ref_runs.p + sg.rr0; c.nref_runs = sg.nrr; c.list_run = b->enc.list_run;
        c.ac_runs_slot = b->enc.ac_runs_slot ? 1u : 0u;
    }

    int trellis() {
        const Stage &tg = b->tr.tstage;
        set_stage(tg);
        c.stats_only = 1;
        if (b->enc.d_long_cnt.zero(st)) return -1;
        c.nz_blk_cnt = b->tr.t_sort ? b->tr.d_tblk_cnt.p : nullptr;
        c.nz_blk_off = (b->tr.t_sort && b->tr.nz_once) ? b->tr.d_tblk_off.p : nullptr;
        launch_nzlist(st, c);
        c.nz_blk_cnt = nullptr; c.nz_blk_off = nullptr;
        if (b->tr.t_sort) {
            TrellisCtx ts;
            memset(&ts, 0, sizeof ts);
            ts.work = b->tr.d_twork.p; ts.nwork = int(b->tr.twork.size()); ts.blk_cnt = b->tr.d_tblk_cnt.p; ts.perm = b->tr.d_tperm.p;
            launch_trellis_sort(st, ts);
        }
        launch_tokens(st, c);
        launch_list_stats(st, c);
        count_list_runs(tg, false);
        launch_ac_runs(st, c);
        launch_gen_tables(st, b->enc.d_tables.p + tg.table0, int(tg.ntables));
        c.stats_only = 0;
        if (b->enc.d_nz_cursor.zero(st)) return -1;
        MARK(KS_TRELLIS_STATS);
        TrellisCtx tc;
        fill_trellis_ctx(tc);
        if (b->tr.d_tqueue.zero(st)) return -1;
        launch_trellis_ac(st, tc);
        MARK(KS_TRELLIS_AC);
        launch_trellis_dc(st, tc);
        launch_fix_dummy(st, b->d_imgs.p, nimg, b->max_dummy, b->d_coef.p);
        MARK(KS_TRELLIS_DC);
        return 0;
    }

    int stage(const Stage &sg, bool mark, bool gate) {
#define SMARK(slot) do { if (mark) MARK(slot); } while (0)
        set_stage(sg);
        c.work_active = gate ? b->enc.d_work_active.p : nullptr;
        a.work0 = int(sg.work0); a.nwork_run = int(sg.nwork);
        if (b->enc.d_long_cnt.zero(st)) return -1;
        launch_nzlist(st, c);
        SMARK(KS_NZLIST);
        launch_list_refine(st, c);
        for (uint32_t wi = sg.work0; sg.nrs && wi < sg.work0 + sg.nwork; wi++)
            if (b->enc.swork[wi].rs_base != 0xFFFFFFFFu && (!gate || b->enc.work_active[wi])) b->enc.last_run_refine++;
        count_list_runs(sg, gate);
        launch_tokens(st, c);
        SMARK(KS_TOKENS);
        launch_list_stats(st, c);
        SMARK(KS_LIST_STATS);
        launch_ac_runs(st, c);
        SMARK(KS_AC_RUNS);
        launch_gen_tables(st, b->enc.d_tables.p + sg.table0, int(sg.ntables));
        SMARK(KS_GEN_TABLES);
        launch_chunk_sizes(st, c);
        SMARK(KS_CHUNK_SIZES);
        launch_exclusive_scan(st, b->enc.d_chunk_bits.p + sg.slot0, b->enc.d_chunk_off.p + sg.slot0, sg.nslots, b->enc.d_scan_tmp.p, b->enc.d_scan_tmp.n);
        SMARK(KS_SCAN_CHUNK_BITS);
        launch_scan_sizes(st, a);
        launch_exclusive_scan(st, b->enc.d_scan_pad.p, b->enc.d_scan_raw_off.p, uint64_t(a.nwork), b->enc.d_scan_tmp.p, b->enc.d_scan_tmp.n);
        launch_scan_place(st, a);
        launch_zero_edges(st, c);
        SMARK(KS_SCAN_LAYOUT);
        launch_pack(st, c);
        SMARK(KS_PACK);
        launch_list_pack(st, c);
        SMARK(KS_LIST_PACK);
        launch_ff_count(st, a);
        SMARK(KS_FF_COUNT);
#undef SMARK
        return 0;
    }

    int gated_stage(int sid, int (*want)(const SearchImg &)) {
        if (!search_gate(b, sid, want)) return 0;
        b->enc.n_gated_runs++;
        if (b->enc.d_work_active.upload(b->enc.work_active, st)) return -1;
        if (stage(b->enc.stage[sid], false, true) || search_costs(b, a, sid)) return -1;
        return search_decide(b, sid);
    }
    int search() {
        b->enc.n_gated_runs = 0;
        if (search_costs(b, a, EncodePlan::ST_1) || search_decide(b, EncodePlan::ST_1)) return -1;
        if (gated_stage(EncodePlan::ST_1B, [](const SearchImg &si) { return si.luma_on ? 1 : 0; })) return -1;
        if (stage(b->enc.stage[EncodePlan::ST_2], false, false)) return -1;
        if (search_costs(b, a, EncodePlan::ST_2) || search_decide(b, EncodePlan::ST_2)) return -1;
        for (int sid : {int(EncodePlan::ST_2B), int(EncodePlan::ST_2C)})
            if (gated_stage(sid, [](const SearchImg &si) { return (si.luma_on ? 1 : 0) | (si.chroma_on ? 2 : 0); })) return -1;
        if (search_lists(b)) return -1;
        return 0;
    }

    int emit() {
        MARK(KS_SCAN_SEARCH);
        launch_layout(st, a);
        MARK(KS_LAYOUT);
        launch_exclusive_scan(st, b->out.d_img_size_pad.p, b->out.d_img_off.p, uint64_t(nimg), b->enc.d_scan_tmp.p, b->enc.d_scan_tmp.n);
        MARK(KS_SCAN_IMAGES);
        launch_emit(st, a);
        MARK(KS_EMIT);
        return 0;
    }

    int finish(bool phases) {
        CSH_CHECK(hipStreamSynchronize(st));
        CSH_CHECK(hipGetLastError());
        if (t && marks.read(t, phases)) return -1;
        if (t && !phases) t->n_images = uint32_t(nimg);
        return 0;
    }

    int webp() {
        const int nwimg = int(b->wp.wimgs.size());
        uint64_t out_bytes = 0;
        std::vector<uint64_t> off(size_t(b->nimg) + 1, 0);
        for (auto &wi : b->wp.wimgs) {
            const uint64_t cap = 4096 + uint64_t(wi.mbw) * wi.mbh * (b->wp.webp_mb_bytes + 2);
            wi.out_cap = uint32_t(std::min<uint64_t>(cap, 0xFFFFFF00u)); wi.out_off = out_bytes;
            off[wi.image] = out_bytes;
            out_bytes += (wi.out_cap + 63) & ~uint64_t(63);
            const int q = int(b->params.webp_quality);
            wi.quality = q < 0 ? 0 : q > 100 ? 100 : q;
        }
        off[b->nimg] = out_bytes;
        if (b->out.d_out.n < out_bytes + 64 && b->out.d_out.alloc(out_bytes + 64)) return -1;
        if ((b->wp.d_wscratch.n < out_bytes + 64 && b->wp.d_wscratch.alloc(out_bytes + 64)) || (b->wp.d_wpart.n < size_t(b->nimg) * 9 + 9 && b->wp.d_wpart.alloc(size_t(b->nimg) * 9 + 9)) ||
            (b->wp.d_wstats.n < size_t(b->nimg) * 2112 + 8 && (b->wp.d_wstats.alloc(size_t(b->nimg) * 2112 + 8) || b->wp.d_wprobs.alloc(size_t(b->nimg) * 1056 + 8) || b->wp.d_wupdate.alloc(size_t(b->nimg) * 1056 + 8))))
            return -1;
        if (b->wp.d_wstats.zero(st)) return -1;
        if (b->wp.d_wimgs.upload(b->wp.wimgs, st) || (b->wp.d_wwork.n < b->wp.wwork_bytes + 64 && b->wp.d_wwork.alloc(b->wp.wwork_bytes + 64)) ||
            (b->wp.d_wlevels.n < b->wp.wlevels + 64 && b->wp.d_wlevels.alloc(b->wp.wlevels + 64)))
            return -1;
        CSH_CHECK(hipMemcpyAsync(b->out.d_img_off.p, off.data(), off.size() * sizeof(uint64_t), hipMemcpyHostToDevice, st));
        if (b->out.d_img_size.zero(st)) return -1;
        csw::launch_webp_yuv(st, b->wp.d_wimgs.p, nwimg, b->wp.wmax_luma, b->pix.d_rgb.p, b->wp.d_wwork.p);
        MARK(KS_WEBP_YUV);
        hipEvent_t mid;
        if (marks.claim(KS_WEBP_ENCODE, &mid)) return -1;
        if (csw::launch_webp_encode(st, b->wp.wimgs.data(), nwimg, b->wp.d_wimgs.p, b->wp.d_wwork.p, b->wp.d_wlevels.p, b->wp.d_wscratch.p, b->wp.d_wpart.p, b->out.d_out.p, b->out.d_img_size.p, b->out.d_status.p, mid)) return -1;
        MARK(KS_WEBP_ASSEMBLE);
        return finish(false);
    }
};

}

int run_once(csh_batch *b, csh_timing *t, bool requant_only) {
    Run r(b, t);
    b->enc.last_run_list_runs = 0;
    b->enc.last_run_fused = 0; b->enc.last_run_refine = 0; b->enc.last_run_ac_lists = 0;
    if (r.pools() || r.marks.start()) return -1;
    const bool from_pixels = requant_only && b->tr.dering;
    if (requant_only && !from_pixels) {
        if (r.requant()) return -1;
    } else {
        if (from_pixels ? r.skip_decode() : r.decode()) return -1;
        if (r.planes()) return -1;
        if (b->webp) return r.webp();
        if (b->rgb_out) return (r.marks.mark(KS_XFORM_DIRECT) || r.finish(false)) ? -1 : 0;
        if (r.pixels()) return -1;
    }
    if (r.encode_begin()) return -1;
    b->enc.last_run_fused = r.fused ? b->enc.n_fused : 0u;
    b->enc.last_run_ac_lists = r.fused ? b->enc.n_ac_lists : 0u;
    if (b->tr.trellis ? r.trellis() : r.marks.skip_to(KS_NZLIST)) return -1;
    r.fill_asm_ctx();
    if (r.stage(b->enc.stage[0], true, false)) return -1;
    if (b->enc.search && r.search()) return -1;
    return (r.emit() || r.finish(true)) ? -1 : 0;
}

}
```

caesium-clt_amd/csrc/k_aclist.hip:

```cpp
#include "kernels.h"
#include "wave.h"

namespace csh {

#define CSH_LP_WORDS 1024

__device__ __forceinline__ static uint32_t lbitlen(uint32_t v) { return 32u - uint32_t(__clz(v)); }
__device__ __forceinline__ static int lwave() { return int(threadIdx.x) / CSP_WAVE_THREADS; }

#define CSH_NZ_HALF 16
__device__ __forceinline__ static uint4 nz_load(const EncCtx &c, const NzSet &S, uint32_t u, int bx, int by, uint32_t oct) {
    uint4 q; q.x = q.y = q.z = q.w = 0u;
    if (u < S.nunits) {
        const int b = by * S.bw + bx;
        q = *reinterpret_cast<const uint4 *>(c.coef + (size_t(S.tile_base) + size_t(b >> 6)) * CSH_TILE_I16 + size_t((b & 63) * CSH_BLK_STRIDE) + size_t(oct) * CSH_OCT_STRIDE);
    }
    return q;
}
__device__ __forceinline__ static uint32_t nz_mask8(const uint4 &q, uint32_t oct) {
    uint32_t m = 0;
    m |= (q.x & 0xFFFFu) ? 1u : 0u;   m |= (q.x >> 16) ? 2u : 0u;
    m |= (q.y & 0xFFFFu) ? 4u : 0u;   m |= (q.y >> 16) ? 8u : 0u;
    m |= (q.z & 0xFFFFu) ? 16u : 0u;  m |= (q.z >> 16) ? 32u : 0u;
    m |= (q.w & 0xFFFFu) ? 64u : 0u;  m |= (q.w >> 16) ? 128u : 0u;
    return oct ? m : (m & ~1u);
}
__device__ __forceinline__ static void nz_load_half(const EncCtx &c, const NzSet &S, uint32_t u0, int half, LV<uint4> (&q)[CSH_NZ_HALF]) {
    LFOR(l) {
        const uint32_t oct = uint32_t(l & 7);
        uint32_t u = u0 + 128u * uint32_t(half) + uint32_t(l >> 3);
        int by = int(u) / S.real_bw, bx = int(u) - by * S.real_bw;
        CSH_UNROLL
        for (int s = 0; s < CSH_NZ_HALF; s++) {
            q[s][l] = nz_load(c, S, u, bx, by, oct);
            u += 8u; bx += 8;
            while (bx >= S.real_bw) { bx -= S.real_bw; by++; }
        }
    }
}
__device__ __forceinline__ static void nz_count_half(const NzSet &S, uint32_t u0, int half, const LV<uint4> (&q)[CSH_NZ_HALF], LV<uint32_t> &cnt) {
    LFOR(l) {
        const uint32_t oct = uint32_t(l & 7);
        uint32_t n = 0;
        CSH_UNROLL
        for (int s = 0; s < CSH_NZ_HALF; s++)
            n += uint32_t(__popc(nz_mask8(q[s][l], oct))) + ((oct == 7u && u0 + 128u * uint32_t(half) + 8u * uint32_t(s) + uint32_t(l >> 3) < S.nunits) ? 1u : 0u);
        cnt[l] += n;
    }
}
__device__ __forceinline__ static void nz_write_half(const NzSet &S, uint32_t u0, int half, const LV<uint4> (&q)[CSH_NZ_HALF], uint32_t *dst, uint32_t run, uint8_t *blk_cnt, uint16_t *blk_off) {
    CSH_UNROLL
    for (int s = 0; s < CSH_NZ_HALF; s++) {
        LV<uint32_t> mk, cl;
        LFOR(l) {
            const uint32_t oct = uint32_t(l & 7);
            mk[l] = nz_mask8(q[s][l], oct);
            cl[l] = uint32_t(__popc(mk[l])) + ((oct == 7u && u0 + 128u * uint32_t(half) + 8u * uint32_t(s) + uint32_t(l >> 3) < S.nunits) ? 1u : 0u);
        }
        uint32_t tot;
        const LV<uint32_t> ex = lscan(cl, tot);
        if (blk_cnt) {
            LV<uint32_t> first = ex;
            for (int d = 0; d < 7; d++) first = lprev(first, 0u);
            LFOR(l) {
                const uint32_t blk = 16u * 8u * uint32_t(half) + 8u * uint32_t(s) + uint32_t(l >> 3);
                if ((l & 7) == 7 && u0 + blk < S.nunits) blk_cnt[u0 + blk] = uint8_t(ex[l] + cl[l] - 1u - first[l]);
                if ((l & 7) == 7 && u0 + blk < S.nunits && blk_off) blk_off[u0 + blk] = uint16_t(run + first[l]);
            }
        }
        LFOR(l) {
            const uint32_t oct = uint32_t(l & 7);
            const uint32_t blk = 16u * 8u * uint32_t(half) + 8u * uint32_t(s) + uint32_t(l >> 3);
            const uint32_t base = (8u * oct) | (blk << 23);
            const uint32_t w[4] = {q[s][l].x, q[s][l].y, q[s][l].z, q[s][l].w};
            uint32_t o = run + ex[l];
            CSH_UNROLL
            for (int i = 0; i < 8; i++)
                if ((mk[l] >> i) & 1u) {
                    const int h = (i & 1) ? (int(w[i >> 1]) >> 16) : (int(w[i >> 1] << 16) >> 16);
                    const uint32_t a = h == -32768 ? 32767u : uint32_t(h < 0 ? -h : h);
                    dst[o++] = (base + uint32_t(i)) | (h < 0 ? 128u : 0u) | (a << 8);
                }
            if (oct == 7u && u0 + blk < S.nunits) dst[o] = CSH_NZ_END | (base & 0x7F800000u);
        }
// ... 392 lines not shown
                }
            }
            pos += tot;
            const uint32_t done = uint32_t(pos >> 5) - ww;
            if (done > CSH_LP_WORDS - 640) {
                CSP_WAVE_SYNC();
                LFOR(l) for (uint32_t q = uint32_t(l); q < done; q += 64) {
                    const uint32_t v = buf[q];
                    if (first_flush && q == 0) { if (v) atomicOr(out + ww, v); } else out[ww + q] = v;
                }
                const uint32_t partial = buf[done];
                CSP_WAVE_SYNC();
                LFOR(l) for (int q = l; q < CSH_LP_WORDS; q += 64) buf[q] = (q == 0) ? partial : 0u;
                CSP_WAVE_SYNC();
                ww += done; first_flush = false;
            }
        }
    }
#ifdef CSH_EMUL
    {
        const uint64_t want = (raw_bit0 & 31u) + (c.chunk_off[cs0 + nrun] - c.chunk_off[cs0]) + pad;
        if (c.overflow[1] ? pos > want : pos != want) { fprintf(stderr, "k_list_pack: a run does not end where its sizes say\n"); abort(); }
    }
#endif
    CSP_WAVE_SYNC();
    const uint32_t last = uint32_t((pos + 31) >> 5) - ww;
    LFOR(l) for (uint32_t q = uint32_t(l); q < last; q += 64) {
        const uint32_t v = buf[q];
        if ((first_flush && q == 0) || q == last - 1) { if (v) atomicOr(out + ww + q, v); } else out[ww + q] = v;
    }
}

struct RefCarry { uint32_t runH, runN, base, prevN, prevNZ; };
__device__ __forceinline__ static uint32_t ref_isN(uint32_t e, uint32_t Ss, uint32_t Se) { const uint32_t k = e & 127u; return (k >= Ss && k <= Se && ((e >> 8) & 0x7FFFu) == 1u) ? 1u : 0u; }
__device__ __forceinline__ static uint32_t ref_isH(uint32_t e, uint32_t Ss, uint32_t Se) { const uint32_t k = e & 127u; return (k >= Ss && k <= Se && ((e >> 8) & 0x7FFFu) >= 2u) ? 1u : 0u; }
__device__ __forceinline__ static uint32_t ref_same(uint32_t key, uint32_t blk) { return (key >> 6) == blk + 1u ? (key & 63u) : 0u; }
template <bool WITH_ZQ>
__device__ __forceinline__ static void ref_step(const LV<uint32_t> (&e)[4], uint32_t Ss, uint32_t Se, RefCarry &C, LV<uint32_t> (&hex)[4], LV<uint32_t> (&z)[4], LV<uint32_t> (&zp)[4],
                                                LV<uint32_t> (&zq)[4]) {
    LV<uint32_t> cnt;
    LFOR(l) {
        uint32_t s = 0;
        CSH_UNROLL
        for (int q = 0; q < 4; q++) s += ref_isH(e[q][l], Ss, Se) | (ref_isN(e[q][l], Ss, Se) << 16);
        cnt[l] = s;
    }
    uint32_t tot;
    const LV<uint32_t> ex = lscan(cnt, tot);
    LV<uint32_t> kb[4];
    LFOR(l) {
        uint32_t ph = C.runH + (ex[l] & 0xFFFFu), pn = C.runN + (ex[l] >> 16);
        CSH_UNROLL
        for (int q = 0; q < 4; q++) {
            kb[q][l] = (e[q][l] & CSH_NZ_END) ? ((ph << 14) | pn) + 1u : 0u;
            hex[q][l] = ph; z[q][l] = pn;
            ph += ref_isH(e[q][l], Ss, Se); pn += ref_isN(e[q][l], Ss, Se);
        }
    }
    C.runH += tot & 0xFFFFu; C.runN += tot >> 16;
    lscan_last4(kb, C.base);
    LFOR(l) {
        CSH_UNROLL
        for (int q = 0; q < 4; q++) {
            const uint32_t b = kb[q][l] ? kb[q][l] - 1u : 0u, blk = (e[q][l] >> 23) & 255u, nz = ref_isH(e[q][l], Ss, Se) | ref_isN(e[q][l], Ss, Se);
            const uint32_t h = hex[q][l] - (b >> 14), n = z[q][l] - (b & 0x3FFFu);
            hex[q][l] = h;
            z[q][l] = nz ? (e[q][l] & 127u) - Ss - h - n : 0u;
            const uint32_t key = ((blk + 1u) << 6) | z[q][l];
            zp[q][l] = ref_isN(e[q][l], Ss, Se) ? key : 0u;
            if (WITH_ZQ) zq[q][l] = nz ? key : 0u;
        }
    }
    lscan_last4(zp, C.prevN);
    if (WITH_ZQ) lscan_last4(zq, C.prevNZ);
    LFOR(l) {
        CSH_UNROLL
        for (int q = 0; q < 4; q++) {
            const uint32_t blk = (e[q][l] >> 23) & 255u;
            zp[q][l] = ref_same(zp[q][l], blk);
            if (WITH_ZQ) zq[q][l] = ref_same(zq[q][l], blk);
        }
    }
}
__global__ void __launch_bounds__(256, 5) k_list_refine(EncCtx c) {
    CSH_SHARED alignas(16) uint32_t s_hist[4][4][256];
    CSH_SHARED uint32_t s_lastn[4][256];
    CSH_SHARED uint32_t s_nh[4][256];
    CSH_SHARED uint32_t s_corr[4][256][2];
    const int wv = int(uni(uint32_t(lwave())));
    const uint32_t idx = blockIdx.x * 4u + uint32_t(wv);
    if (idx >= c.nref_runs) return;
    const uint32_t cs0 = c.ref_runs[idx];
    const SlotRec r = c.slots[cs0];
    if (c.work_active && !c.work_active[r.work]) return;
    const uint32_t nrun = run_chunks(c, r);
    const uint64_t lbase = c.nzlists[r.nzlist].base;
    ListSlot nx = list_chunk(c, lbase, r.nzrec);
    const TokRegion rg = c.regions[r.region];
    uint32_t *hist = &s_hist[wv][0][0], *lastn = s_lastn[wv], *nh = s_nh[wv], *corr = &s_corr[wv][0][0];
    LFOR(l) {
        uint4 zero; zero.x = zero.y = zero.z = zero.w = 0u;
        for (int i = 4 * l; i < 1024; i += 256) *reinterpret_cast<uint4 *>(hist + i) = zero;
    }
    const uint32_t Ss = r.Ss, Se = r.Se;
    LV<uint32_t> freq[4];
    LFOR(l) { freq[0][l] = 0u; freq[1][l] = 0u; freq[2][l] = 0u; freq[3][l] = 0u; }
    for (uint32_t ci = 0; ci < nrun; ci++) {
        const ListSlot ls = nx;
        if (ci + 1u < nrun) nx = list_chunk(c, lbase, r.nzrec + ci + 1u);
        const uint32_t cs = cs0 + ci, j = r.j + ci, unit0 = r.unit0 + 256u * ci, corr0 = r.corr0 + 256u * ci, hist_row = r.hist_row + ci * uint32_t(r.ntables);
        const uint32_t left = r.nunits_work - 256u * j, nun = left < 256u ? left : 256u;
        CSP_WAVE_SYNC();
        LFOR(l) for (int i = l; i < 256; i += 64) { lastn[i] = 0u; nh[i] = 0u; corr[2 * i] = 0u; corr[2 * i + 1] = 0u; }
        CSP_WAVE_SYNC();
        RefCarry C;
        C.runH = C.runN = C.base = C.prevN = C.prevNZ = 0u;
        LV<uint32_t> ntok;
        LFOR(l) ntok[l] = 0u;
        {
        LV<uint32_t> x[4];
        LFOR(l) list_load4(ls, 4u * uint32_t(l), x[0][l], x[1][l], x[2][l], x[3][l]);
        for (uint32_t g0 = 0; g0 < ls.n; g0 += 256) {
            LV<uint32_t> e[4], hex[4], z[4], zp[4], zq[4];
            LFOR(l) { e[0][l] = x[0][l]; e[1][l] = x[1][l]; e[2][l] = x[2][l]; e[3][l] = x[3][l]; }
            if (g0 + 256u < ls.n) LFOR(l) list_load4(ls, g0 + 256u + 4u * uint32_t(l), x[0][l], x[1][l], x[2][l], x[3][l]);
            ref_step<false>(e, Ss, Se, C, hex, z, zp, zq);
            LFOR(l) {
                uint32_t *h = hist + 256 * (l & 3);
                CSH_UNROLL
                for (int q = 0; q < 4; q++) {
                    const uint32_t v = e[q][l], blk = (v >> 23) & 255u;
                    if (ref_isH(v, Ss, Se)) {
                        atomicMax(&nh[blk], hex[q][l] + 1u);
                        if (v & 0x100u) atomicOr(&corr[2u * blk + (hex[q][l] >> 5)], 0x80000000u >> (hex[q][l] & 31u));
                    } else if (ref_isN(v, Ss, Se)) {
                        const uint32_t zr = z[q][l] - zp[q][l];
                        atomicMax(&lastn[blk], ((v & 127u) << 6) | hex[q][l]);
                        atomicAdd(&h[((zr & 15u) << 4) | 1u], 1u);
                        if (zr >> 4) atomicAdd(&h[0xF0], zr >> 4);
                        ntok[l] += 1u + (zr >> 4);
                    }
                }
            }
        }
        }
        CSP_WAVE_SYNC();
        for (uint32_t w4 = 0; w4 < 4; w4++) {
            LFOR(l) {
                const uint32_t i = 64u * w4 + uint32_t(l);
                if (i < nun) {
                    const uint32_t ln = lastn[i];
                    if (ls.n && (ln >> 6) != Se) ntok[l] += 1u;
                    c.tail[unit0 + i] = uint8_t(nh[i] - (ln & 63u));
                    c.corr[corr0 + i] = (uint64_t(corr[2u * i]) << 32) | corr[2u * i + 1u];
                }
            }
            const uint64_t ms = lballot([&](int b) { const uint32_t i = 64u * w4 + uint32_t(b); return i < nun && lastn[i] != 0u; });
            const uint64_t me = lballot([&](int b) { const uint32_t i = 64u * w4 + uint32_t(b); return i < nun && (lastn[i] >> 6) != Se; });
            LFOR(l) if (l == 0 && j * 4u + w4 < ((r.nunits_work + 63u) >> 6)) { c.sym_bits[r.word_base + j * 4u + w4] = ms; c.eob_bits[r.word_base + j * 4u + w4] = me; }
        }
        const uint32_t total = lsum32(ntok);
        hist_flush(hist, c.slot_hist + size_t(hist_row) * 256u, freq);
        LFOR(l) if (l == 0) c.slot_raw[cs] = C.runN + C.runH;
        if (c.stats_only) continue;
        uint32_t rel = 0;
        LFOR(l) if (l == 0) rel = atomicAdd(&c.tok_cursor[r.region], total);
        rel = uni(rel);
        const bool ok = uint64_t(rel) + total <= rg.cap;
        LFOR(l) {
            if (l < 4) { c.tok_off[cs * 4u + uint32_t(l)] = rg.base + rel; c.chunk_ntok[cs * 4u + uint32_t(l)] = (ok && l == 0) ? total : 0u; }
            if (l == 0 && !ok) c.overflow[1] = 1;
        }
        if (!ok) continue;
        uint32_t *tk = c.tokens + rg.base + rel;
        C.runH = C.runN = C.base = C.prevN = C.prevNZ = 0u;
        uint32_t curc = 0, at = 0;
        for (uint32_t g0 = 0; g0 < ls.n; g0 += 256) {
            LV<uint32_t> e[4], hex[4], z[4], zp[4], zq[4], cur[4], nt;
            LFOR(l) list_load4(ls, g0 + 4u * uint32_t(l), e[0][l], e[1][l], e[2][l], e[3][l]);
            ref_step<true>(e, Ss, Se, C, hex, z, zp, zq);
            LFOR(l) {
                uint32_t s = 0;
                CSH_UNROLL
                for (int q = 0; q < 4; q++) {
                    const uint32_t v = e[q][l], blk = (v >> 23) & 255u, lastk = lastn[blk] >> 6, isN = ref_isN(v, Ss, Se);
                    uint32_t nz = 0, n = 0;
                    if ((isN | ref_isH(v, Ss, Se)) && (v & 127u) <= lastk) { nz = ((z[q][l] - zp[q][l]) >> 4) - ((zq[q][l] - zp[q][l]) >> 4); n = nz + isN; }
                    cur[q][l] = n ? ((blk + 1u) << 6) | hex[q][l] : 0u;
                    if ((v & CSH_NZ_END) && lastk != Se) n = 1u;
                    zq[q][l] = nz | (n << 8);
                    s += n;
                }
                nt[l] = s;
            }
            lscan_last4(cur, curc);
            uint32_t tot;
            const LV<uint32_t> ex = lscan(nt, tot);
            LFOR(l) {
                uint32_t o = at + ex[l];
                CSH_UNROLL
                for (int q = 0; q < 4; q++) {
                    const uint32_t v = e[q][l], blk = (v >> 23) & 255u, nz = zq[q][l] & 255u, n = zq[q][l] >> 8;
                    if (!n) continue;
                    const uint32_t cu = ref_same(cur[q][l], blk);
                    if (v & CSH_NZ_END) {
                        if (o < total) tk[o] = TK_EOB | (blk << 3) | ((nh[blk] - cu) << 16) | (cu << 22);
                        o++;
                        continue;
                    }
                    uint32_t cnt = hex[q][l] - cu, from = cu;
                    for (uint32_t t = 0; t < nz; t++) {
                        if (o < total) tk[o] = TK_REF | (blk << 3) | (cnt << 16) | (from << 22) | (1u << 28);
                        o++; cnt = 0u; from = hex[q][l];
                    }
                    if (n > nz) {
                        if (o < total) tk[o] = TK_REF | (blk << 3) | (((z[q][l] - zp[q][l]) & 15u) << 11) | ((v & 128u) ? 0u : (1u << 15)) | (cnt << 16) | (from << 22);
                        o++;
                    }
                }
            }
            at += tot;
        }
#ifdef CSH_EMUL
        if (at != total) { fprintf(stderr, "k_list_refine: pass 2 made %u tokens, pass 1 counted %u\n", at, total); abort(); }
#endif
    }
    freq_flush(c.tables[r.table_base].freq, freq);
}

__global__ void k_reset_works(ScanWork *work, int nwork) {
    const int j = int(blockIdx.x * blockDim.x + threadIdx.x);
    if (j >= nwork) return;
    work[j].out_off = 0xFFFFFFFFu; work[j].raw_bytes = 0; work[j].hdr_bytes = 0; work[j].ff_bytes = 0; work[j].no_room = 0;
}

void launch_nzlist(hipStream_t st, const EncCtx &c) {
    if (!c.nnzchunks) return;
    if (c.nz_build) CSH_LAUNCH_PHASED(k_nzlist, 3, dim3(c.nnzchunks), dim3(2 * CSP_WAVE_THREADS), st, c);
    if (c.nz_filter) CSH_LAUNCH(k_nzfilter, dim3(c.nnzchunks), dim3(CSP_WAVE_THREADS), st, c);
}
void launch_list_stats(hipStream_t st, const EncCtx &c) { if (c.nlist_runs) CSH_LAUNCH(k_list_stats, dim3((c.nlist_runs + 3) / 4), dim3(4 * CSP_WAVE_THREADS), st, c); }
void launch_list_refine(hipStream_t st, const EncCtx &c) { if (c.nref_runs) CSH_LAUNCH(k_list_refine, dim3((c.nref_runs + 3) / 4), dim3(4 * CSP_WAVE_THREADS), st, c); }
void launch_list_pack(hipStream_t st, const EncCtx &c) { if (c.nlist_runs) CSH_LAUNCH(k_list_pack, dim3((c.nlist_runs + 3) / 4), dim3(4 * CSP_WAVE_THREADS), st, c); }
__global__ void __launch_bounds__(64) k_make_slots(const ScanWork *works, uint32_t nworks, const EncScan *script, const NzList *nzlists, SlotRec *slots, uint32_t *slot_work, uint32_t *list_slots,
                                                   uint32_t *tok_slots, uint32_t *ref_slots, uint32_t *list_runs, uint32_t *ref_runs, uint32_t list_run) {
    const uint32_t wi = blockIdx.x;
    if (wi >= nworks) return;
    const ScanWork &w = works[wi];
    const EncScan &e = script[w.scan];
    const uint32_t nch = (w.nunits + 255u) / 256u;
    const bool prog_ac = e.Ss > 0 && !e.sequential, has_list = w.list != 0xFFFFFFFFu;
    const bool ref_list = has_list && prog_ac && e.Ah;
    const bool listed = has_list && !ref_list;
    for (uint32_t j = threadIdx.x; j < nch; j += blockDim.x) {
        SlotRec r;
        r.work = wi; r.j = j; r.nch = nch; r.first_chunk = w.first_chunk; r.unit0 = w.unit_base + 256u * j;
        r.nun = w.nunits - 256u * j < 256u ? w.nunits - 256u * j : 256u; r.table_base = w.table_base; r.ntables = uint16_t(e.ntables);
        r.flags = uint16_t((prog_ac ? 1 : 0) | (prog_ac && e.Ah ? 2 : 0) | (listed ? 4 : 0) | (ref_list ? 8 : 0));
        r.hist_row = w.hist_row0 + j * uint32_t(e.ntables);
        r.word_base = w.word_base; r.unit_base = w.unit_base; r.nunits_work = w.nunits;
        r.Ss = uint8_t(e.Ss); r.Se = uint8_t(e.Se); r.Ah = uint8_t(e.Ah); r.Al = uint8_t(e.Al); r.corr0 = w.corr_base == 0xFFFFFFFFu ? 0u : w.corr_base + 256u * j;
        r.nzlist = has_list ? w.list : 0u; r.nzrec = has_list ? nzlists[w.list].chunk0 + j : 0u; r.region = ref_list ? w.region : 0u;
        slots[w.first_chunk + j] = r;
        slot_work[w.first_chunk + j] = wi;
        (listed ? list_slots : tok_slots)[w.ls_base + j] = w.first_chunk + j;
        if (ref_list) ref_slots[w.rs_base + j] = w.first_chunk + j;
        if (listed && j % list_run == 0u) list_runs[w.lr_base + j / list_run] = w.first_chunk + j;
        if (ref_list && j % list_run == 0u) ref_runs[w.rr_base + j / list_run] = w.first_chunk + j;
    }
}
__global__ void __launch_bounds__(64) k_rebind_slots(const ScanWork *works, uint32_t nworks, const NzList *nzlists, SlotRec *slots) {
    const uint32_t wi = blockIdx.x;
    if (wi >= nworks) return;
    const ScanWork &w = works[wi];
    if (w.list == 0xFFFFFFFFu) return;
    const uint32_t nch = (w.nunits + 255u) / 256u, chunk0 = nzlists[w.list].chunk0;
    for (uint32_t j = threadIdx.x; j < nch; j += blockDim.x) { slots[w.first_chunk + j].nzlist = w.list; slots[w.first_chunk + j].nzrec = chunk0 + j; }
}
void launch_rebind_slots(hipStream_t st, const ScanWork *works, uint32_t nworks, const NzList *nzlists, SlotRec *slots) {
    if (nworks) CSH_LAUNCH(k_rebind_slots, dim3(nworks), dim3(64), st, works, nworks, nzlists, slots);
}
void launch_make_slots(hipStream_t st, const ScanWork *works, uint32_t nworks, const EncScan *script, const NzList *nzlists, SlotRec *slots, uint32_t *slot_work, uint32_t *list_slots,
                       uint32_t *tok_slots, uint32_t *ref_slots, uint32_t *list_runs, uint32_t *ref_runs, uint32_t list_run) {
    if (!nworks) return;
    CSH_LAUNCH(k_make_slots, dim3(nworks), dim3(64), st, works, nworks, script, nzlists, slots, slot_work, list_slots, tok_slots, ref_slots, list_runs, ref_runs, list_run);
}

void launch_reset_works(hipStream_t st, ScanWork *work, int nwork) { if (nwork) CSH_LAUNCH(k_reset_works, dim3((nwork + 255) / 256), dim3(256), st, work, nwork); }

}
```

caesium-clt_amd/csrc/k_entropy.hip:

```cpp
#include "kernels.h"
#include "wave.h"

namespace csh {

#define CSH_PK_WORDS 1024

__device__ __forceinline__ static uint64_t band_mask(int Ss, int Se) { return (~0ull >> (63 - Se)) & (~0ull << Ss); }
__device__ __forceinline__ static int msb64(uint64_t v) { return 63 - __clzll(v); }
__device__ __forceinline__ static int bitlen32(unsigned v) { return 32 - __clz(v); }
__device__ __forceinline__ static int lane_id() { return int(threadIdx.x & 63); }

__device__ __forceinline__ static int unit_block(const CompGeom &g, uint32_t u) {
    int by = int(u) / g.real_bw, bx = int(u) - by * g.real_bw;
    return by * g.bw + bx;
}
__device__ __forceinline__ static bool get_bit(const uint64_t *w, uint32_t i) { return (w[i >> 6] >> (i & 63)) & 1; }

#ifndef CSH_EMUL
template <class Op>
__device__ __forceinline__ static uint32_t wave_scan_dpp(uint32_t v, Op op) {
    v = op(v, uint32_t(__builtin_amdgcn_update_dpp(0, int(v), 0x111, 0xf, 0xf, false)));
    v = op(v, uint32_t(__builtin_amdgcn_update_dpp(0, int(v), 0x112, 0xf, 0xf, false)));
    v = op(v, uint32_t(__builtin_amdgcn_update_dpp(0, int(v), 0x114, 0xf, 0xf, false)));
    v = op(v, uint32_t(__builtin_amdgcn_update_dpp(0, int(v), 0x118, 0xf, 0xf, false)));
    v = op(v, uint32_t(__builtin_amdgcn_update_dpp(0, int(v), 0x142, 0xa, 0xf, false)));
    v = op(v, uint32_t(__builtin_amdgcn_update_dpp(0, int(v), 0x143, 0xc, 0xf, false)));
    return v;
}
__device__ __forceinline__ static uint32_t wave_incl_sum(uint32_t v) { return wave_scan_dpp(v, [](uint32_t a, uint32_t b) { return a + b; }); }
__device__ __forceinline__ static uint32_t wave_last(uint32_t v) { return uint32_t(__builtin_amdgcn_readlane(int(v), 63 - __clzll((unsigned long long)__ballot(1)))); }
#endif

__device__ __forceinline__ static uint64_t wave_or64(uint64_t v) {
#ifdef CSH_EMUL
    (void)v;
    return ~0ull;
#else
    auto bor = [](uint32_t a, uint32_t b) { return a | b; };
    const uint32_t lo = wave_last(wave_scan_dpp(uint32_t(v), bor)), hi = wave_last(wave_scan_dpp(uint32_t(v >> 32), bor));
    return (uint64_t(hi) << 32) | lo;
#endif
}
__device__ __forceinline__ static uint32_t wave_incl_scan(const uint32_t *in, int lane) {
#ifdef CSH_EMUL
    uint32_t s = 0;
    for (int i = 0; i <= lane; i++) s += in[i] & 0xFFFFu;
    return s;
#else
    return wave_incl_sum(in[lane]);
#endif
}

struct TokOut {
    uint32_t *pool;
    uint32_t pos;
    bool dry;
    __device__ __forceinline__ void put(uint32_t t) { if (!dry) pool[pos] = t; pos++; }
};

template <bool EMIT>
struct TokSink {
    uint32_t n;
    uint32_t pend;
    bool has_pend;
    TokOut out;
    uint32_t *hist;
    int h0;
    uint32_t rawbits;
    static constexpr bool kValues = true;
    __device__ __forceinline__ void begin() { n = 0; pend = 0; has_pend = false; }
    __device__ __forceinline__ void flush() { if (has_pend) { if (EMIT) out.put(pend); n++; has_pend = false; } }
    __device__ __forceinline__ void sym(int t, int s) {
        flush();
        pend = TK_SYM | (uint32_t(s) << 3) | (uint32_t(t) << 11); has_pend = true;
        if (EMIT) atomicAdd(&hist[(h0 + t) * 257 + s], 1u);
    }
    __device__ __forceinline__ void syms(int t, int s, int cnt) { for (int i = 0; i < cnt; i++) sym(t, s); }
    __device__ __forceinline__ void raw(unsigned v, int nb) {
        if (EMIT) rawbits += uint32_t(nb);
        while (nb > 0) {
            int have = has_pend ? int((pend >> 13) & 15u) : 0;
            if (has_pend && have == 15) { flush(); have = 0; }
            if (!has_pend) { pend = TK_RAW; has_pend = true; }
            const int take = nb < 15 - have ? nb : 15 - have;
// ... 680 lines not shown
        for (int i = l; i < 256; i += 64) { ocode[i] = 0; osize[i] = 0; ovals[i] = 0; }
    }
    CSP_WAVE_SYNC();
    LV<uint32_t> f[5], cs[5], g[5];
    for (int j = 0; j < 5; j++) LFOR(l) { const int e = l + 64 * j; f[j][l] = e < n ? freq0[e] : 0u; cs[j][l] = 0; g[j][l] = uint32_t(e); if (e < n) grp[e] = uint16_t(e); }
    CSP_WAVE_SYNC();
    for (;;) {
        LV<uint64_t> key;
        LFOR(l) {
            uint64_t k1 = ~0ull;
            for (int j = 0; j < 5; j++) { const uint64_t k = (uint64_t(f[j][l]) << 32) | uint32_t(~uint32_t(l + 64 * j)); if (f[j][l] && k < k1) k1 = k; }
            key[l] = k1;
        }
        const uint64_t k1 = lmin64(key);
        const int c1 = int(~uint32_t(k1));
        LFOR(l) {
            uint64_t k2 = ~0ull;
            for (int j = 0; j < 5; j++) { const uint64_t k = (uint64_t(f[j][l]) << 32) | uint32_t(~uint32_t(l + 64 * j)); if (f[j][l] && l + 64 * j != c1 && k < k2) k2 = k; }
            key[l] = k2;
        }
        const uint64_t k2 = lmin64(key);
        if (k2 == ~0ull) break;
        const int c2 = int(~uint32_t(k2));
        const uint32_t f2 = uint32_t(k2 >> 32);
        const uint32_t g1 = grp[c1], g2 = grp[c2];
        CSP_WAVE_SYNC();
        for (int j = 0; j < 5; j++) LFOR(l) {
            const int e = l + 64 * j;
            if (e == c1) f[j][l] += f2;
            if (e == c2) f[j][l] = 0;
            if (e < n && (g[j][l] == g1 || g[j][l] == g2)) { cs[j][l]++; if (g[j][l] != g1) { g[j][l] = g1; grp[e] = uint16_t(g1); } }
        }
        CSP_WAVE_SYNC();
    }
    for (int j = 0; j < 5; j++) LFOR(l) {
        const int e = l + 64 * j;
        if (e < n) {
            csz[e] = uint16_t(cs[j][l]);
            if (cs[j][l]) atomicAdd(&bits[cs[j][l] > 32 ? 32 : cs[j][l]], 1u);
            if (e < n - 1 && cs[j][l] >= 1 && cs[j][l] <= 32) atomicAdd(&bits[33], 1u);
        }
    }
    CSP_WAVE_SYNC();
    {
        LV<uint32_t> before[5];
        for (int j = 0; j < 5; j++) LFOR(l) before[j][l] = 0;
        for (int q = 0; q < n - 1; q++) {
            const uint32_t cq = csz[q];
            for (int j = 0; j < 5; j++) LFOR(l) before[j][l] += (cq >= 1 && cq <= 32 && (cq < cs[j][l] || (cq == cs[j][l] && q < l + 64 * j))) ? 1u : 0u;
        }
        for (int j = 0; j < 5; j++) LFOR(l) { const int e = l + 64 * j; if (e < n - 1 && cs[j][l] >= 1 && cs[j][l] <= 32) ovals[before[j][l]] = uint8_t(symof[e]); }
    }
    LFOR(l) if (l == 0) {
        for (int i = 32; i > 16; i--)
            while (bits[i] > 0) {
                int j = i - 2; while (bits[j] == 0) j--;
                bits[i] -= 2; bits[i - 1]++; bits[j + 1] += 2; bits[j]--;
            }
        int i = 16; while (i > 0 && bits[i] == 0) i--;
        if (i > 0) bits[i]--;
    }
    CSP_WAVE_SYNC();
    const int nsym = int(bits[33]);
    LFOR(lane) for (int p = lane; p < nsym; p += 64) {
        int code = 0, st = 0, len = 0, mine = 0;
        for (int l = 1; l <= 16; l++) {
            const int bl = int(bits[l]);
            if (!len && p < st + bl) { len = l; mine = code + (p - st); }
            code = (code + bl) << 1; st += bl;
        }
        if (len) { ocode[ovals[p]] = uint16_t(mine); osize[ovals[p]] = uint8_t(len); }
    }
    CSP_WAVE_SYNC();
    LFOR(lane) {
        if (lane <= 16) T.bits[lane] = lane ? uint8_t(bits[lane]) : 0;
        if (lane == 0) T.nsym = nsym;
        for (int i = lane; i < 256; i += 64) { T.vals[i] = ovals[i]; T.code[i] = ocode[i]; T.size[i] = osize[i]; T.lut[i] = (uint32_t(osize[i]) << 16) | ocode[i]; }
    }
}
void launch_gen_tables(hipStream_t st, DevEncTable *tables, int ntables) {
    if (ntables) CSH_LAUNCH(k_gen_tables, dim3((ntables + 3) / 4), dim3(4 * CSP_WAVE_THREADS), st, tables, ntables);
}

struct Pieces { uint32_t v[3], n[3]; };
struct TokenCtx {
    const uint32_t *lut;
    uint32_t lut_stride;
    const uint16_t *eobrun;
    const uint64_t *corr;
};
#define CSH_LUT_STRIDE uint32_t(sizeof(DevEncTable) / 4)
__device__ __forceinline__ static void corr_pieces(Pieces &p, uint64_t corr, uint32_t t) {
    const uint32_t cnt = (t >> 16) & 63u, cur = (t >> 22) & 63u;
    if (!cnt) return;
    const uint64_t bits = (corr << cur) >> (64u - cnt);
    if (cnt > 32) { p.v[1] = uint32_t(bits >> 32); p.n[1] = cnt - 32; p.v[2] = uint32_t(bits); p.n[2] = 32; }
    else { p.v[2] = uint32_t(bits); p.n[2] = cnt; }
}
template <int MODE = 0>
__device__ __forceinline__ static Pieces token_pieces(uint32_t t, const TokenCtx &x) {
    Pieces p;
    p.v[0] = p.v[1] = p.v[2] = 0; p.n[0] = p.n[1] = p.n[2] = 0;
    uint32_t kind = t & 7u;
    if (MODE == 1) { if (kind == TK_RAW) return p; kind = kind == TK_ACF ? uint32_t(TK_ACF) : uint32_t(TK_EOB); }
    if (MODE == 2) { if (kind == TK_RAW) return p; kind = kind == TK_REF ? uint32_t(TK_REF) : uint32_t(TK_EOB); }
    if (MODE == 3) kind = kind == TK_SYM ? uint32_t(TK_SYM) : uint32_t(TK_RAW);
    if (kind == TK_SYM) {
        const uint32_t e = x.lut[((t >> 11) & 3u) * x.lut_stride + ((t >> 3) & 255u)], nr = (t >> 13) & 15u;
        p.v[0] = ((e & 0xFFFFu) << nr) | (t >> 17); p.n[0] = (e >> 16) + nr;
    } else if (kind == TK_RAW) { p.v[0] = t >> 17; p.n[0] = (t >> 13) & 15u; }
    else if (kind == TK_ACF) {
        const uint32_t r = (t >> 3) & 63u, nb = (t >> 9) & 15u, zr = r >> 4;
        if (zr) {
            const uint32_t z = x.lut[0xF0], zc = z & 0xFFFFu, zl = z >> 16;
            p.v[0] = zc; p.n[0] = zl;
            if (zr > 1) { p.v[0] = (zc << zl) | zc; p.n[0] = 2 * zl; }
            if (zr > 2) { p.v[1] = zc; p.n[1] = zl; }
        }
        const uint32_t e = x.lut[((r & 15u) << 4) | nb];
        p.v[2] = ((e & 0xFFFFu) << nb) | ((t >> 13) & 0xFFFFu); p.n[2] = (e >> 16) + nb;
    } else if (kind == TK_REF) {
        const uint32_t unit = (t >> 3) & 255u;
        if (t & (1u << 28)) { const uint32_t e = x.lut[0xF0]; p.v[0] = e & 0xFFFFu; p.n[0] = e >> 16; }
        else { const uint32_t e = x.lut[(((t >> 11) & 15u) << 4) | 1u]; p.v[0] = ((e & 0xFFFFu) << 1) | ((t >> 15) & 1u); p.n[0] = (e >> 16) + 1; }
        if ((t >> 16) & 63u) corr_pieces(p, x.corr[unit], t);
    } else {
        const uint32_t unit = (t >> 3) & 255u;
        const uint32_t run = x.eobrun[unit];
        if (run) {
            const int nb = bitlen32(run) - 1;
            const uint32_t e = x.lut[nb << 4];
            p.v[0] = ((e & 0xFFFFu) << nb) | (run & ((1u << nb) - 1u)); p.n[0] = (e >> 16) + uint32_t(nb);
        }
        if ((t >> 16) & 63u) corr_pieces(p, x.corr[unit], t);
    }
    return p;
}
__device__ __forceinline__ static TokenCtx token_ctx(const EncCtx &c, const SlotRec &r) {
    TokenCtx x;
    x.lut = c.tables[r.table_base].lut; x.lut_stride = CSH_LUT_STRIDE;
    x.eobrun = c.eobrun + r.unit0;
    x.corr = c.corr + r.corr0;
    return x;
}
__device__ __forceinline__ static void load4(const uint32_t *tk, uint32_t i, uint32_t n, uint32_t (&t)[4]) {
    CSH_UNROLL
    for (int q = 0; q < 4; q++) t[q] = i + uint32_t(q) < n ? tk[i + uint32_t(q)] : uint32_t(TK_RAW);
}

__global__ void __launch_bounds__(256) k_chunk_sizes(EncCtx c) {
    const uint32_t cs = c.slot0 + blockIdx.x * 4u + (threadIdx.x >> 6);
    const int lane = lane_id();
    if (cs >= c.slot0 + c.nslots) return;
    const SlotRec r = c.slots[cs];
    if (c.work_active && !c.work_active[r.work]) { if (lane == 0) c.chunk_bits[cs] = 0; return; }
#ifdef CSH_EMUL
    if (lane) return;
    uint32_t bits = c.slot_raw[cs];
    for (uint32_t t = 0; t < r.ntables; t++)
        for (uint32_t sy = 0; sy < 256; sy++) bits += uint32_t(c.slot_hist[size_t(r.hist_row + t) * 256u + sy]) * c.tables[r.table_base + t].size[sy];
    if (r.flags & 1u) for (uint32_t nb = 0; nb < 15; nb++) bits += c.slot_eobh[cs * 16u + nb] * (uint32_t(c.tables[r.table_base].size[nb << 4]) + nb);
    c.chunk_bits[cs] = bits;
#else
    uint32_t bits = lane == 0 ? c.slot_raw[cs] : 0u;
    for (uint32_t t = 0; t < r.ntables; t++) {
        const uint2 h = reinterpret_cast<const uint2 *>(c.slot_hist + size_t(r.hist_row + t) * 256u)[lane];
        const uint32_t z = reinterpret_cast<const uint32_t *>(c.tables[r.table_base + t].size)[lane];
        bits += (h.x & 0xFFFFu) * (z & 255u) + (h.x >> 16) * ((z >> 8) & 255u) + (h.y & 0xFFFFu) * ((z >> 16) & 255u) + (h.y >> 16) * (z >> 24);
    }
    if ((r.flags & 1u) && lane < 15) bits += c.slot_eobh[cs * 16u + uint32_t(lane)] * (uint32_t(c.tables[r.table_base].size[lane << 4]) + uint32_t(lane));
    CSH_UNROLL
    for (int o = 32; o >= 1; o >>= 1) bits += uint32_t(__shfl_xor(int(bits), o, 64));
    if (lane == 0) c.chunk_bits[cs] = bits;
#endif
}

__device__ __forceinline__ static void or_bits(uint32_t *words, uint64_t pos, uint32_t v, uint32_t n) {
    v &= n >= 32 ? 0xFFFFFFFFu : ((1u << n) - 1u);
    const uint64_t t = uint64_t(v) << (64u - n - uint32_t(pos & 31u));
    const uint32_t hi = uint32_t(t >> 32), lo = uint32_t(t);
    if (hi) atomicOr(words + (pos >> 5), hi);
    if (lo) atomicOr(words + (pos >> 5) + 1, lo);
}
#define CSH_WAVE_FENCE() do { __builtin_amdgcn_fence(__ATOMIC_ACQ_REL, "wavefront"); __builtin_amdgcn_wave_barrier(); } while (0)
template <int MODE>
__device__ __forceinline__ static bool token_main(uint32_t t, const TokenCtx &x, uint32_t &v, uint32_t &n) {
    v = 0; n = 0;
    const uint32_t kind = t & 7u;
    if (kind == TK_RAW) { v = t >> 17; n = (t >> 13) & 15u; return true; }
    if (MODE == 3) {
        const uint32_t e = x.lut[((t >> 11) & 3u) * x.lut_stride + ((t >> 3) & 255u)], nr = (t >> 13) & 15u;
        v = ((e & 0xFFFFu) << nr) | (t >> 17); n = (e >> 16) + nr;
        return true;
    }
    if (MODE == 1 && kind == TK_ACF) {
        const uint32_t r = (t >> 3) & 63u, nb = (t >> 9) & 15u;
        if (r >> 4) return false;
        const uint32_t e = x.lut[(r << 4) | nb];
        v = ((e & 0xFFFFu) << nb) | ((t >> 13) & 0xFFFFu); n = (e >> 16) + nb;
        return true;
    }
    const uint32_t unit = (t >> 3) & 255u, cnt = (t >> 16) & 63u, cur = (t >> 22) & 63u;
    if (MODE == 2 && kind == TK_REF) {
        if (t & (1u << 28)) { const uint32_t e = x.lut[0xF0]; v = e & 0xFFFFu; n = e >> 16; }
        else { const uint32_t e = x.lut[(((t >> 11) & 15u) << 4) | 1u]; v = ((e & 0xFFFFu) << 1) | ((t >> 15) & 1u); n = (e >> 16) + 1; }
    } else {
        const uint32_t run = x.eobrun[unit];
        if (run) {
            const int nb = bitlen32(run) - 1;
            const uint32_t e = x.lut[nb << 4];
            v = ((e & 0xFFFFu) << nb) | (run & ((1u << nb) - 1u)); n = (e >> 16) + uint32_t(nb);
        }
    }
    if (MODE == 2 && cnt) {
        if (n + cnt > 32) return false;
        const uint32_t bits = uint32_t((x.corr[unit] << cur) >> (64u - cnt));
        v = (n ? (v << cnt) : 0u) | bits; n += cnt;
    }
    return true;
}

#ifndef CSH_EMUL
struct PackState { uint32_t *buf, *out; uint64_t pos; uint32_t ww; bool first_flush; };
template <int MODE>
__device__ __forceinline__ static void pack_segments(const EncCtx &c, const TokenCtx &x, PackState &S, uint32_t cs, uint32_t pad, int lane) {
    uint32_t *buf = S.buf, *out = S.out;
    uint64_t pos = S.pos;
    uint32_t ww = S.ww;
    bool first_flush = S.first_flush;
    const uint32_t seg_n = lane < 4 ? c.chunk_ntok[cs * 4u + uint32_t(lane)] : 0u;
    const unsigned long long seg_o = lane < 4 ? c.tok_off[cs * 4u + uint32_t(lane)] : 0ull;
    auto step = [&](const uint32_t (&t)[4], uint32_t i, uint32_t n, bool last_seg) {
        {
            uint32_t v4[4], n4[4];
            bool slow = false;
            CSH_UNROLL
            for (int q = 0; q < 4; q++) {
                slow |= !token_main<MODE>(t[q], x, v4[q], n4[q]);
                if (pad && last_seg && i + uint32_t(q) == n) { v4[q] = (1u << pad) - 1u; n4[q] = pad; }
            }
            if (!__ballot(slow) && !(c.debug & 4096u)) {
                const uint32_t len1 = n4[0] + n4[1] + n4[2] + n4[3];
                const uint32_t incl1 = wave_incl_sum(len1);
                uint64_t at1 = pos + incl1 - len1 - uint64_t(ww) * 32u;
                CSH_UNROLL
                for (int q = 0; q < 4; q++) if (n4[q]) { or_bits(buf, at1, v4[q], n4[q]); at1 += n4[q]; }
                pos += wave_last(incl1);
                goto slide;
            }
        }
        {
        Pieces p[4];
        uint32_t len = 0;
        CSH_UNROLL
        for (int q = 0; q < 4; q++) {
            p[q] = token_pieces<MODE>(t[q], x);
            if (pad && last_seg && i + uint32_t(q) == n) { p[q].v[0] = (1u << pad) - 1u; p[q].n[0] = pad; }
            len += p[q].n[0] + p[q].n[1] + p[q].n[2];
        }
        const uint32_t incl = wave_incl_sum(len);
        uint64_t at = pos + incl - len - uint64_t(ww) * 32u;
        CSH_UNROLL
        for (int q = 0; q < 4; q++) {
            CSH_UNROLL
            for (int k = 0; k < 3; k++) if (p[q].n[k]) { or_bits(buf, at, p[q].v[k], p[q].n[k]); at += p[q].n[k]; }
        }
        pos += wave_last(incl);
        }
    slide:
        const uint32_t done = uint32_t(pos >> 5) - ww;
        if (done > CSH_PK_WORDS - 770) {
            CSH_WAVE_FENCE();
            for (uint32_t q = uint32_t(lane); q < done; q += 64) {
                const uint32_t v = buf[q];
                if (first_flush && q == 0) { if (v) atomicOr(out + ww, v); } else out[ww + q] = v;
            }
            const uint32_t partial = buf[done];
            CSH_WAVE_FENCE();
            for (int q = lane; q < CSH_PK_WORDS; q += 64) buf[q] = (q == 0) ? partial : 0u;
            CSH_WAVE_FENCE();
            ww += done; first_flush = false;
        }
    };
    uint32_t n[4]; const uint32_t *tk[4];
    CSH_UNROLL
    for (int seg = 0; seg < 4; seg++) {
        n[seg] = uint32_t(__builtin_amdgcn_readlane(int(seg_n), seg));
        tk[seg] = c.tokens + ((unsigned long long)uint32_t(__builtin_amdgcn_readlane(int(uint32_t(seg_o)), seg)) | ((unsigned long long)uint32_t(__builtin_amdgcn_readlane(int(uint32_t(seg_o >> 32)), seg)) << 32));
    }
    const uint32_t b1 = n[0], b2 = b1 + n[1], b3 = b2 + n[2], total = b3 + n[3];
    const uint32_t n_ext = total + (pad ? 1u : 0u);
    for (uint32_t g0 = 0; g0 < n_ext; g0 += 256) {
        uint32_t t[4];
        CSH_UNROLL
        for (int q = 0; q < 4; q++) {
            const uint32_t g = g0 + 4u * uint32_t(lane) + uint32_t(q);
            const uint32_t *src = g >= b3 ? tk[3] + (g - b3) : g >= b2 ? tk[2] + (g - b2) : g >= b1 ? tk[1] + (g - b1) : tk[0] + g;
            t[q] = g < total ? *src : uint32_t(TK_RAW);
        }
        step(t, g0 + 4u * uint32_t(lane), total, true);
    }
    S.pos = pos; S.ww = ww; S.first_flush = first_flush;
}
#endif
// ... 90 lines not shown
```

caesium-clt_amd/csrc/kernels.h:

```cpp
#pragma once
#include "gpu_rt.h"
#include "types.h"

namespace csh {

__host__ __device__ static inline int coef_off(int k) { return (k >> 3) * CSH_OCT_STRIDE + (k & 7); }
__host__ __device__ static inline size_t coef_index(uint32_t tile_base, int b, int k) {
    return (size_t(tile_base) + size_t(b >> 6)) * CSH_TILE_I16 + size_t((b & 63) * CSH_BLK_STRIDE) + size_t(coef_off(k));
}

#define CSH_RAW_OCT 8
__host__ __device__ static inline size_t raw_index(uint32_t tile_base, int b) { return size_t(tile_base) * CSH_TILE_I16 + size_t(b) * 64; }

__device__ __forceinline__ static int csh_plane_at(const uint8_t *p, int pitch, int cw, int ch, int y, int x) {
    y = y < 0 ? 0 : (y > ch - 1 ? ch - 1 : y);
    x = x < 0 ? 0 : (x > cw - 1 ? cw - 1 : x);
    return p[size_t(y) * pitch + x];
}
__device__ __forceinline__ static int csh_upsample_at(const uint8_t *p, int pitch, int cw, int ch, UpDesc u, int r, int xx) {
    switch (u.cls) {
    case CSH_UP_COPY: return csh_plane_at(p, pitch, cw, ch, r, xx);
    case CSH_UP_H2V1: {
        const int cx = xx >> 1, nb = (xx & 1) ? cx + 1 : cx - 1;
        return (3 * csh_plane_at(p, pitch, cw, ch, r, cx) + csh_plane_at(p, pitch, cw, ch, r, nb) + ((xx & 1) ? 2 : 1)) >> 2;
// ... 45 lines not shown

struct NzFuse {
    const NzSet *nzsets; const NzList *nzlists;
    uint32_t *nz_pool, *nz_cursor, *nz_chunk_off, *nz_chunk_cnt;
    uint8_t *blk_cnt; uint16_t *blk_off;
    uint32_t *overflow;
};
void launch_xform_direct(hipStream_t st, const ImgDesc *imgs, const PlaneWork *work, int nwork, int max_tiles, const DevQuant *quant,
                         const int16_t *coef_in, int16_t *coef_out, int16_t *dct_raw, uint32_t raw_tile0, bool dering, const NzFuse &nzf);
void launch_requant(hipStream_t st, const ImgDesc *imgs, const PlaneWork *work, int nwork, int max_tiles, const DevQuant *quant, const int16_t *dct_raw,
                    uint32_t raw_tile0, int16_t *coef_out);
void launch_idct_plane(hipStream_t st, const ImgDesc *imgs, const PlaneWork *work, int nwork, int max_tiles, const DevQuant *quant,
                       const int16_t *coef_in, uint8_t *planes);
void launch_resample_plane(hipStream_t st, const ImgDesc *imgs, const PlaneWork *work, int nwork, uint32_t max_quads, const uint8_t *planes, uint8_t *oplanes);
void launch_plane_fdct(hipStream_t st, const ImgDesc *imgs, const PlaneWork *work, int nwork, int max_tiles, const DevQuant *quant,
                       const uint8_t *oplanes, int16_t *coef_out, int16_t *dct_raw, uint32_t raw_tile0, bool dering, const NzFuse &nzf);
void launch_resample_fdct_420(hipStream_t st, const ImgDesc *imgs, const PlaneWork *work, int nwork, int max_tiles, const DevQuant *quant,
                              const uint8_t *planes, int16_t *coef_out, int16_t *dct_raw, uint32_t raw_tile0, bool dering, const NzFuse &nzf);
void launch_resample_any(hipStream_t st, const ImgDesc *imgs, const PlaneWork *work, int nwork, uint32_t max_quads, const uint8_t *planes, uint8_t *oplanes);
void launch_fix_dummy(hipStream_t st, const ImgDesc *imgs, int nimg, int max_blocks, int16_t *coef_out);

bool resize_is_fused(uint32_t max_row_in);
void launch_resize(hipStream_t st, const ImgDesc *imgs, const ResizeWork *work, int nwork, const ResizeTap *taps, const float *weights,
                   uint8_t *planes, uint8_t *rgb, float *tmp, uint32_t max_src_px, uint64_t max_tmp, uint64_t max_dst, uint32_t max_row_in, uint32_t max_out_w, uint32_t max_nh, bool to_planes,
                   bool any_layout = false, bool any_space = false);

struct EncCtx {
    const ImgDesc *imgs;
    const EncScan *script;
    const ScanWork *work;
    int nwork;
    const EChunk *echunks;
    uint32_t nechunks;
    const TokPlan *plans;
    const uint32_t *slot_work;
    const SlotRec *slots;
    uint32_t slot0, nslots;
    const int16_t *coef;
    uint64_t *sym_bits;
    uint64_t *eob_bits;
    uint8_t *tail;
    uint16_t *eobrun;
    uint32_t *long_runs, *long_cnt;
    uint64_t *corr;
    uint32_t *tokens;
    const TokRegion *regions;
    uint32_t *tok_cursor;
    uint64_t *tok_off;
    uint32_t *chunk_ntok;
    uint16_t *slot_hist;
    uint32_t *slot_raw;
    uint32_t *slot_eobh;
    uint32_t *chunk_bits;
    const uint64_t *chunk_off;
    DevEncTable *tables;
    uint32_t *raw;
    uint64_t raw_words;
    uint32_t *status;
    uint32_t *overflow;
    uint32_t debug;
    uint32_t stats_only;
    const uint8_t *work_active;
    const NzList *nzlists;
    const NzSet *nzsets;
    const NzChunk *nzchunks;
    uint32_t nnzchunks;
    uint32_t *nz_pool;
    uint32_t *nz_cursor;
    uint32_t *nz_chunk_off;
    uint32_t *nz_chunk_cnt;
    uint8_t *nz_blk_cnt;
    uint16_t *nz_blk_off;
    const uint32_t *list_slots;
    uint32_t nlist_slots;
    const uint32_t *tok_slots;
    uint32_t ntok_slots;
    const uint32_t *ref_slots;
    uint32_t nref_slots;
    const uint32_t *list_runs;
    uint32_t nlist_runs;
    const uint32_t *ref_runs;
    uint32_t nref_runs;
    uint32_t list_run;
    uint32_t ac_runs_slot;
    uint32_t nz_build, nz_filter;
};
enum : uint32_t { TK_SYM = 0u, TK_RAW = 1u, TK_ACF = 2u, TK_REF = 3u, TK_EOB = 4u };
void launch_tokens(hipStream_t st, const EncCtx &c);
void launch_ac_runs(hipStream_t st, const EncCtx &c);
void launch_gen_tables(hipStream_t st, DevEncTable *tables, int ntables);
void launch_chunk_sizes(hipStream_t st, const EncCtx &c);
void launch_zero_edges(hipStream_t st, const EncCtx &c);
void launch_pack(hipStream_t st, const EncCtx &c);
void launch_nzlist(hipStream_t st, const EncCtx &c);
void launch_list_stats(hipStream_t st, const EncCtx &c);
void launch_list_refine(hipStream_t st, const EncCtx &c);
void launch_list_pack(hipStream_t st, const EncCtx &c);
void launch_nz_to_tiles(hipStream_t st, const NzSet *nzsets, const NzList *nzlists, const uint32_t *nz_pool, const uint32_t *nz_chunk_off, const uint32_t *nz_chunk_cnt,
                        uint32_t set, uint32_t nchunks, int16_t *coef);
void launch_reset_works(hipStream_t st, ScanWork *work, int nwork);

#ifndef CSH_LIST_RUN
#define CSH_LIST_RUN 8
#endif
#ifndef CSH_TR_WG
#define CSH_TR_WG 256
#endif
#ifndef CSH_TR_RUN
#define CSH_TR_RUN 8
#endif
struct TrellisCtx {
    const ImgDesc *imgs;
    const DevQuant *quant;
    const TrellisWork *work;
    int nwork;
    const TrellisRun *runs;
    uint32_t nruns;
    uint32_t *queue;
    uint32_t nslots;
    const DevEncTable *tables;
    const int16_t *raw;
    uint32_t raw_tile0;
    int16_t *coef;
    uint64_t *dcrec;
    uint64_t *dcbt;
    uint32_t *spill;
    uint32_t max_rows;
    const uint8_t *blk_cnt;
    uint32_t *perm;
    const uint32_t *rows;
    uint32_t nrows;
    uint32_t debug;
    uint32_t *nz_pool;
    const NzList *nzlists;
    const NzSet *nzsets;
    const uint32_t *nz_chunk_off, *nz_chunk_cnt;
    const uint16_t *blk_off;
    uint32_t ac_lists;
};
void launch_trellis_sort(hipStream_t st, const TrellisCtx &c);
void launch_trellis_ac(hipStream_t st, const TrellisCtx &c);
void launch_trellis_dc(hipStream_t st, const TrellisCtx &c);
uint32_t trellis_ac_slots();
size_t trellis_spill_words(uint32_t nslots);

void launch_exclusive_scan(hipStream_t st, const uint32_t *in, uint64_t *out, uint64_t n, void *tmp, size_t tmp_bytes);
size_t exclusive_scan_tmp_bytes(uint64_t n);

struct AsmCtx {
    const ImgDesc *imgs;
    const EncScan *script;
    ScanWork *work;
    int nwork, nimg, scans_per_image;
    int work0, nwork_run;
    const uint32_t *img_list;
    const uint32_t *img_nlist;
    uint32_t *scan_cost;
    const DevEncTable *tables;
    const uint64_t *chunk_off;
    uint32_t *scan_pad_bytes;
    uint64_t *scan_raw_off;
    const uint32_t *raw;
    uint64_t raw_chunks;
    uint32_t *chunk_ff;
    const uint8_t *hdr_pool;
    const uint32_t *hdr_off;
    uint32_t *img_size_pad;
    uint32_t *img_size;
    uint64_t *img_off;
    uint8_t *out;
    uint64_t out_cap;
    uint32_t *status;
    uint32_t *overflow;
};
void launch_scan_cost(hipStream_t st, const AsmCtx &a);
void launch_scan_sizes(hipStream_t st, const AsmCtx &a);
void launch_scan_place(hipStream_t st, const AsmCtx &a);
void launch_ff_count(hipStream_t st, const AsmCtx &a);
void launch_layout(hipStream_t st, const AsmCtx &a);
void launch_emit(hipStream_t st, const AsmCtx &a);
// ... 3 lines not shown
```

caesium-clt_amd/csrc/pipeline.cpp:

```cpp
#include <algorithm>
#include <atomic>
#include <cmath>
#include <cstdarg>
#include <memory>
#include <thread>

#include "batch.hpp"
#include "../../include/vp8_tables.h"
#include "resize_host.h"

static thread_local char g_err[512];
void csh_set_error(const char *fmt, ...) {
    va_list ap;
    va_start(ap, fmt);
    vsnprintf(g_err, sizeof g_err, fmt, ap);
    va_end(ap);
}
extern "C" const char *csh_last_error(void) { return g_err; }

#ifdef CSH_EMUL
thread_local dim3 threadIdx, blockIdx, blockDim, gridDim;
int csh_emul_reverse = 0;
thread_local int csh_emul_phase = 0;
extern "C" void csh_emul_set_reverse(int r) { csh_emul_reverse = r; }
// ... 145 lines not shown
    b->retain_dct = on != 0;
    if (b->retain_dct && b->nimg && b->pix.d_dct_raw.n == 0 && b->pix.d_dct_raw.alloc(size_t(b->ntiles_out) * CSH_TILE_I16)) return -1;
    return 0;
}
extern "C" int csh_batch_set_quality(csh_batch *b, const uint32_t *quality) {
    if (b->lossless) { csh_set_error("set_quality on a lossless batch"); return -1; }
    b->enc.hdr_pool.clear(); b->enc.hdr_off.clear();
    for (size_t n = 0; n < b->items.size(); n++) {
        Item &it = b->items[n];
        if (it.image < 0) continue;
        ImgDesc &im = b->imgs[it.image];
        if (quality[n]) {
            int q = int(quality[n]) < 1 ? 1 : (quality[n] > 100 ? 100 : int(quality[n]));
            for (int c = 0; c < im.ncomp; c++) im.qt_out[c] = b->q_base + q;
        }
        JpegInfo hdr = it.out;
        int qidx = im.qt_out[0];
        uint16_t nat[64];
        for (int k = 0; k < 64; k++) nat[kZigZag[k]] = b->quants[qidx].q[k];
        memcpy(hdr.qt[0], nat, 128); memcpy(hdr.qt[1], nat, 128);
        std::vector<uint8_t> fh = build_frame_header(hdr, b->progressive, it.meta_out.empty() ? nullptr : &it.meta_out);
        b->enc.hdr_off.push_back(uint32_t(b->enc.hdr_pool.size()));
        b->enc.hdr_pool.insert(b->enc.hdr_pool.end(), fh.begin(), fh.end());
    }
    b->enc.hdr_off.push_back(uint32_t(b->enc.hdr_pool.size()));
    if (!b->nimg) return 0;
    if (hipSetDevice(b->device) != hipSuccess) return -1;
    if (b->d_imgs.upload(b->imgs, b->stream) || b->enc.d_hdr.upload(b->enc.hdr_pool, b->stream) || b->enc.d_hdr_off.upload(b->enc.hdr_off, b->stream)) return -1;
    CSH_CHECK(hipStreamSynchronize(b->stream));
    return 0;
}
extern "C" int csh_batch_rerun_encode(csh_batch *b, csh_timing *t) {
    if (!b->have_dct) { csh_set_error("rerun_encode needs a completed csh_batch_run after csh_batch_retain_dct(1)"); return -1; }
    return batch_run(b, t, true);
}

static int batch_run(csh_batch *b, csh_timing *t, bool requant_only) {
    if (t) memset(t, 0, sizeof *t);
    if (!b->nimg) { b->out.ran = true; return 0; }
    if (hipSetDevice(b->device) != hipSuccess) { csh_set_error("hipSetDevice failed"); return CS_ERR_NO_DEVICE; }
    for (int attempt = 0; attempt < 4; attempt++) {
        if (run_once(b, t, requant_only)) return CS_ERR_NO_DEVICE;
        uint32_t ovf[4] = {0, 0, 0, 0};
        if (csh_copy_wait(ovf, b->out.d_overflow.p, sizeof ovf, hipMemcpyDeviceToHost, b->stream) != hipSuccess) { csh_set_error("D2H failed"); return CS_ERR_NO_DEVICE; }
        b->out.h_status.resize(b->nimg);
        if (csh_copy_wait(b->out.h_status.data(), b->out.d_status.p, b->nimg * sizeof(uint32_t), hipMemcpyDeviceToHost, b->stream) != hipSuccess) return CS_ERR_NO_DEVICE;
        bool pool = ovf[0] != 0;
        if (ovf[1]) {
            pool = true; b->enc.tok_scale *= 4;
            layout_token_pool(b);
            if (b->enc.d_regions.upload(b->enc.regions, b->stream) || b->enc.d_nzlists.upload(b->enc.nzlists, b->stream) || hipStreamSynchronize(b->stream) != hipSuccess) return CS_ERR_NO_DEVICE;
        }
        for (uint32_t s : b->out.h_status) if (s == CS_ERR_POOL_OVERFLOW) pool = true;
        if (!pool) break;
        if (attempt == 3) { csh_set_error("device pools overflowed after 3 retries"); return CS_ERR_POOL_OVERFLOW; }
        b->out.raw_bytes_cap *= 4; b->out.out_cap = b->out.raw_bytes_cap;
        b->wp.webp_mb_bytes *= 4;
    }
    b->out.h_img_size.resize(b->nimg);
    b->out.h_img_off.resize(b->nimg + 1);
    if (csh_copy_wait(b->out.h_img_size.data(), b->out.d_img_size.p, b->nimg * sizeof(uint32_t), hipMemcpyDeviceToHost, b->stream) != hipSuccess ||
        csh_copy_wait(b->out.h_img_off.data(), b->out.d_img_off.p, (b->nimg + 1) * sizeof(uint64_t), hipMemcpyDeviceToHost, b->stream) != hipSuccess) {
        csh_set_error("D2H of sizes failed"); return CS_ERR_NO_DEVICE;
    }
    if (t) {
        std::vector<uint32_t> ns(b->nimg);
        if (csh_copy_wait(ns.data(), b->dec.d_need_seq.p, b->nimg * sizeof(uint32_t), hipMemcpyDeviceToHost, b->stream) != hipSuccess) return CS_ERR_NO_DEVICE;
        if (getenv("CSH_TRACE") && b->dec.d_relax_cnt.n) {
            std::vector<uint32_t> rc(b->dec.d_relax_cnt.n);
            if (csh_copy_wait(rc.data(), b->dec.d_relax_cnt.p, rc.size() * sizeof(uint32_t), hipMemcpyDeviceToHost, b->stream) == hipSuccess) {
                fprintf(stderr, "[csh] relax list sizes (of %u sub-sequences):", b->dec.total_sub);
                for (size_t i = 0; i < rc.size() && (i < 16 || rc[i]); i++) fprintf(stderr, " %u", rc[i]);
                fprintf(stderr, "\n");
            }
        }
        for (const ProgChain &pc : b->dec.chains) if (pc.refine && ns[size_t(pc.image)] == 4) t->n_refine_chains++;
        for (uint32_t v : ns) { if (v == 4) { t->n_prog_decoded++; continue; } if (v) t->n_seq_decoded++; if (v == 2 || v == 3) t->n_par_fallback++; if (v == 3) t->n_par_short++; }
        t->n_images = uint32_t(b->nimg);
        t->n_search_extra = b->enc.search ? b->enc.n_gated_runs : 0u;
        t->n_fused_lists = b->enc.last_run_fused;
        t->n_list_refine = b->enc.last_run_refine;
        t->n_ac_in_lists = b->enc.last_run_ac_lists;
        t->n_list_runs = b->enc.last_run_list_runs;
        for (const Item &it : b->items) if (it.image < 0) t->n_failed++;
        for (int i = 0; i < b->nimg; i++) { t->out_bytes += b->out.h_img_size[i]; t->pixels += uint64_t(b->imgs[i].width) * b->imgs[i].height; }
        t->in_bytes = b->dec.bits_pool.size();
        uint64_t in_tiles = 0;
        for (const ImgDesc &im : b->imgs) for (int c = 0; c < im.ncomp_in; c++) in_tiles += im.in[c].ntiles;
        t->coef_bytes = in_tiles * CSH_TILE_I16 * 2;
    }
    b->out.ran = true;
    if (!requant_only) b->have_dct = (b->retain_dct || b->tr.trellis) && !b->lossless;
    return 0;
}

static void set_result(CCSResult *r, int code, const std::string &msg) {
    r->success = code == 0;
    r->code = uint32_t(code);
    r->error_message = nullptr;
    if (code) { char *m = (char *)malloc(msg.size() + 1); memcpy(m, msg.c_str(), msg.size() + 1); r->error_message = m; }
}

extern "C" int csh_batch_pixels(csh_batch *b, size_t image, const uint8_t **device_pixels, uint32_t *width, uint32_t *height, uint32_t *channels, const char **message) {
    *device_pixels = nullptr; *width = *height = *channels = 0;
    if (message) *message = "";
    if (!b || !b->out.ran || !b->rgb_out || image >= b->items.size()) { csh_set_error("csh_batch_pixels: not a pixel batch that has run"); if (message) *message = "not a pixel batch that has run"; return CS_ERR_NO_DEVICE; }
    const Item &it = b->items[image];
    if (it.code) { if (message) *message = it.msg.c_str(); return it.code; }
    if (b->out.h_status[it.image]) { if (message) *message = "device reported a malformed stream"; return int(b->out.h_status[it.image]); }
    if (size_t(it.image) < b->pix.rwork.size() && b->pix.rwork[size_t(it.image)].image == it.image) {
        const ResizeWork &rw = b->pix.rwork[size_t(it.image)];
        *device_pixels = b->pix.d_rgb.p + rw.rgb_dst_off; *width = uint32_t(rw.nw); *height = uint32_t(rw.nh); *channels = uint32_t(b->imgs[it.image].ncomp);
        return 0;
    }
    if (message) *message = "image has no pixel output";
    return CS_ERR_NO_DEVICE;
}

extern "C" int csh_batch_fetch(csh_batch *b, CByteArray *outputs, CCSResult *results) {
    if (!b->out.ran) { csh_set_error("csh_batch_fetch before csh_batch_run"); return -1; }
    if (b->rgb_out) { csh_set_error("csh_batch_fetch: a pixel batch has no files (csh_batch_pixels)"); return -1; }
    struct PinnedOut { uint8_t *p = nullptr; size_t cap = 0; ~PinnedOut() { if (p) pinned_cache().put(p, cap); } uint8_t *data() const { return p; } } host;
    if (b->nimg && b->out.h_img_off[b->nimg]) {
        host.p = static_cast<uint8_t *>(pinned_cache().get(b->out.h_img_off[b->nimg], host.cap));
        if (!host.p) { csh_set_error("out of pinned host memory"); return -1; }
        if (csh_copy_wait(host.p, b->out.d_out.p, b->out.h_img_off[b->nimg], hipMemcpyDeviceToHost, b->stream) != hipSuccess) { csh_set_error("D2H of output failed"); return -1; }
    }
    std::atomic<int> failed{0};
    std::atomic<size_t> next{0};
    auto worker = [&]() {
        for (size_t n; (n = next++) < b->items.size();) {
            Item &it = b->items[n];
            outputs[n].data = nullptr; outputs[n].length = 0;
            int code = it.code;
            std::string msg = it.msg;
            if (!code && it.image >= 0 && b->out.h_status[it.image]) { code = int(b->out.h_status[it.image]); msg = "device reported a malformed stream"; }
            if (!code) {
                size_t len = b->out.h_img_size[it.image];
                outputs[n].data = (uint8_t *)malloc(len ? len : 1);
                memcpy(outputs[n].data, host.data() + b->out.h_img_off[it.image], len);
                outputs[n].length = len;
            } else failed++;
            if (results) set_result(&results[n], code, msg);
        }
    };
    size_t nthreads = std::min<size_t>(std::min<size_t>(8, std::max(1u, std::thread::hardware_concurrency())), b->items.size() / 64 + 1);
    std::vector<std::thread> pool;
    for (size_t t = 1; t < nthreads; t++) pool.emplace_back(worker);
    worker();
    for (auto &t : pool) t.join();
    return failed.load();
}

extern "C" int csh_batch_geometry(csh_batch *b, size_t image, int comp, int which, int *bw, int *bh, int *real_bw, int *real_bh) {
    if (image >= b->items.size() || b->items[image].image < 0) { csh_set_error("image not on the device"); return -1; }
    const ImgDesc &im = b->imgs[b->items[image].image];
    if (comp < 0 || comp >= (which ? im.ncomp : im.ncomp_in)) { csh_set_error("bad component"); return -1; }
    const CompGeom &g = which ? im.out[comp] : im.in[comp];
    *bw = g.bw; *bh = g.bh; *real_bw = g.real_bw; *real_bh = g.real_bh;
    return 0;
}

extern "C" int csh_batch_read_coefs(csh_batch *b, size_t image, int comp, int which, int16_t *dst) {
    int bw, bh, rbw, rbh;
    if (csh_batch_geometry(b, image, comp, which, &bw, &bh, &rbw, &rbh)) return -1;
    const ImgDesc &im = b->imgs[b->items[image].image];
// ... 17 lines not shown
```

include/caesium_hip.h:

```cpp
#ifndef CAESIUM_HIP_H
#define CAESIUM_HIP_H
#include <stdbool.h>
#include <stddef.h>
#include <stdint.h>
#ifdef __cplusplus
extern "C" {
#endif

enum { CS_TYPE_JPEG = 0, CS_TYPE_PNG = 1, CS_TYPE_GIF = 2, CS_TYPE_WEBP = 3, CS_TYPE_TIFF = 4, CS_TYPE_UNKN = 5 };

enum {
    CS_OK = 0,
    CS_ERR_NO_DEVICE = 10001,
    CS_ERR_UNKNOWN_TYPE = 10200,
    CS_ERR_UNSUPPORTED = 10201,
    CS_ERR_BAD_JPEG = 20100,
    CS_ERR_JPEG_FEATURE = 20101,
    CS_ERR_POOL_OVERFLOW = 20200,
    CS_ERR_BAD_PNG = 30100,
    CS_ERR_BAD_WEBP = 40100,
    CS_ERR_SAME_FORMAT = 10407,
    CS_ERR_TOO_BIG = 10500
};

typedef struct {
    bool keep_metadata;
    uint32_t jpeg_quality;
    uint32_t jpeg_chroma_subsampling;
    bool jpeg_progressive;
    bool jpeg_optimize;
    bool jpeg_preserve_icc;
    uint32_t png_quality;
    uint32_t png_optimization_level;
    bool png_force_zopfli;
    bool png_optimize;
    uint32_t gif_quality;
    uint32_t webp_quality;
    bool webp_lossless;
    uint32_t tiff_compression;
    uint32_t tiff_deflate_level;
    uint32_t width;
    uint32_t height;
} CCSParameters;

typedef struct {
    bool success;
    uint32_t code;
    const char *error_message;
} CCSResult;

typedef struct {
    uint8_t *data;
    size_t length;
} CByteArray;

void cs_default_parameters(CCSParameters *p);

CCSResult cs_compress_in_memory(const uint8_t *in, size_t n, const CCSParameters *p, CByteArray *out);
CCSResult cs_compress_to_size_in_memory(const uint8_t *in, size_t n, CCSParameters *p, size_t max_output_size,
                                        bool return_smallest, CByteArray *out);
CCSResult cs_convert_in_memory(const uint8_t *in, size_t n, const CCSParameters *p, uint32_t format, CByteArray *out);
int cs_batch_convert(const CByteArray *inputs, size_t count, const CCSParameters *p, uint32_t format, int device, CByteArray *outputs, CCSResult *results);

int cs_batch_compress(const CByteArray *inputs, size_t count, const CCSParameters *p, int device,
                      CByteArray *outputs, CCSResult *results);
int cs_batch_compress_to_size(const CByteArray *inputs, size_t count, CCSParameters *p, size_t max_output_size, bool return_smallest,
                              int device, CByteArray *outputs, CCSResult *results);

size_t cs_batch_extent(const CByteArray *inputs, size_t count);

void cs_free_bytes(CByteArray *b);
void cs_free_result(CCSResult *r);

typedef struct csh_batch csh_batch;

enum { CSH_NPHASES = 8, CSH_NKERNELS = 36 };
typedef struct {
    float total_ms;
    float phase_ms[CSH_NPHASES];
    float kernel_ms[CSH_NKERNELS];
    uint64_t in_bytes, out_bytes;
    uint64_t pixels;
    uint64_t coef_bytes;
    uint32_t n_images, n_failed;
    uint32_t n_seq_decoded;
    uint32_t n_par_fallback;
    uint32_t n_par_short;
    uint32_t n_prog_decoded;
    uint32_t n_refine_chains;
    uint32_t n_search_extra;
    uint32_t n_fused_lists;
    uint32_t n_list_refine;
    uint32_t n_ac_in_lists;
    uint32_t n_list_runs;
} csh_timing;

int csh_device_count(void);
const char *csh_last_error(void);
void csh_warmup(int device);
void csh_release_cached_memory(void);
const char *csh_kernel_name(int slot);
const char *csh_kernel_name_webp(int slot);
int csh_batch_create(const CByteArray *inputs, size_t count, const CCSParameters *p, int device, csh_batch **out);
int csh_batch_create_webp(const CByteArray *inputs, size_t count, const CCSParameters *p, int device, csh_batch **out);
int csh_batch_create_pixels(const CByteArray *inputs, size_t count, const CCSParameters *p, int device, csh_batch **out);
int csh_batch_pixels(csh_batch *b, size_t image, const uint8_t **device_pixels, uint32_t *width, uint32_t *height, uint32_t *channels, const char **message);
struct csp_pixels_s;
int csh_batch_create_from_pixels(const struct csp_pixels_s *sources, size_t count, const CCSParameters *p, int device, csh_batch **out);
int csh_batch_run(csh_batch *b, csh_timing *t);
int csh_batch_fetch(csh_batch *b, CByteArray *outputs, CCSResult *results);
void csh_batch_destroy(csh_batch *b);

int csh_batch_retain_dct(csh_batch *b, int on);
int csh_batch_set_quality(csh_batch *b, const uint32_t *quality);
int csh_batch_rerun_encode(csh_batch *b, csh_timing *t);

int csh_batch_geometry(csh_batch *b, size_t image, int comp, int which, int *bw, int *bh, int *real_bw, int *real_bh);
int csh_batch_read_coefs(csh_batch *b, size_t image, int comp, int which, int16_t *dst);

typedef struct csp_batch csp_batch;
enum { CSP_NKERNELS = 16 };
typedef struct {
    float total_ms;
    float kernel_ms[CSP_NKERNELS];
    uint64_t in_bytes, out_bytes;
    uint64_t pixels, raw_bytes;
    uint32_t n_images, n_failed, n_trials;
} csp_timing;
const char *csp_kernel_name(int slot);
int csp_batch_create(const CByteArray *inputs, size_t count, const CCSParameters *p, int device, csp_batch **out);
int csp_batch_create_webp(const CByteArray *inputs, size_t count, const CCSParameters *p, int device, csp_batch **out);
typedef struct csp_pixels_s { const uint8_t *device_pixels; uint32_t width, height, channels; } csp_pixels;
int csp_batch_create_pixels(const csp_pixels *sources, size_t count, const CCSParameters *p, int device, csp_batch **out);
int csp_png_to_jpeg(const CByteArray *inputs, size_t count, const CCSParameters *p, int device, CByteArray *outputs, CCSResult *results);
int csp_png_to_lossless_webp(const CByteArray *inputs, size_t count, const CCSParameters *p, int device, CByteArray *outputs, CCSResult *results);
int csp_batch_run(csp_batch *b, csp_timing *t);
int csp_batch_fetch(csp_batch *b, CByteArray *outputs, CCSResult *results);
void csp_batch_destroy(csp_batch *b);
int csp_batch_geometry(csp_batch *b, size_t image, uint32_t *width, uint32_t *height, uint32_t *rowbytes);
int csp_batch_read_rows(csp_batch *b, size_t image, uint8_t *dst);
int csp_batch_read_stream(csp_batch *b, size_t image, int strategy, uint8_t *dst);
int csp_batch_read_scores(csp_batch *b, size_t image, uint64_t *dst, int *have);
int csp_batch_trials(csp_batch *b, size_t image, int *strategies, uint64_t *zlib_bytes, int *ntrials, int *winner);
int csp_batch_chunk_bits(csp_batch *b, size_t image, int trial, uint64_t *dst, size_t cap, size_t *nchunks);

int csl_encode_pixels(const struct csp_pixels_s *sources, size_t count, int device, CByteArray *outputs, CCSResult *results);
int csl_attach_alpha(CByteArray *lossy, const CByteArray *alpha_vp8l, uint32_t width, uint32_t height);

typedef struct cswd_batch cswd_batch;
int cswd_batch_create(const CByteArray *inputs, size_t count, int device, cswd_batch **out);
int cswd_batch_run(cswd_batch *b);
int cswd_batch_pixels(cswd_batch *b, size_t image, const uint8_t **device_pixels, uint32_t *width, uint32_t *height, uint32_t *channels, const char **message);
int cswd_batch_read_pixels(cswd_batch *b, size_t image, uint8_t *dst );
int cswd_batch_alpha(cswd_batch *b, size_t image, const uint8_t **device_rgba, const uint8_t **device_alpha);
int cswd_batch_read_rgba(cswd_batch *b, size_t image, uint8_t *dst );
void cswd_batch_destroy(cswd_batch *b);
int cswd_batch_frames(cswd_batch *b, size_t file, uint32_t *nframes, uint32_t *canvas_w, uint32_t *canvas_h);
int cswd_batch_read_canvas(cswd_batch *b, size_t file, uint32_t frame, uint8_t *dst_rgba);
int cswd_batch_encode_anim(cswd_batch *b, const CByteArray *sources, const size_t *files, size_t nfiles, const CCSParameters *p, int device, CByteArray *outputs, CCSResult *results);
typedef struct cswd_rgba cswd_rgba;
int cswd_rgba_join(const uint8_t *device_rgb, const uint8_t *device_alpha, uint32_t width, uint32_t height, int device, cswd_rgba **out, const uint8_t **device_rgba);
void cswd_rgba_destroy(cswd_rgba *r);
int csh_batch_create_webp_from_pixels(const struct csp_pixels_s *sources, size_t count, const CCSParameters *p, int device, csh_batch **out);
int csh_batch_create_from_pixels_rgb(const struct csp_pixels_s *sources, size_t count, const CCSParameters *p, int device, csh_batch **out);

#ifdef __cplusplus
}
#endif
#endif
```

Baseline: 44910.

## Fuse refinement-scan token generation into a new list-refine pack kernel

Adds a k_list_refine_pack kernel that regenerates refinement tokens in shared memory and packs them directly. It saves per-unit lastn values from k_list_refine, which now runs a stats-only template variant when packing is enabled. Refinement works no longer reserve global token slots or region estimates. The aim is to avoid writing and re-reading the token stream for progressive refinement scans, at the cost of recomputing tokens in the pack stage and an extra lastn buffer.

```diff
diff --git a/caesium-clt_amd/binding.py b/caesium-clt_amd/binding.py
--- a/caesium-clt_amd/binding.py
+++ b/caesium-clt_amd/binding.py
@@ -25,7 +25,7 @@
 
 class Timing(C.Structure):
     _fields_ = [("total_ms", C.c_float), ("phase_ms", C.c_float * NPHASES), ("kernel_ms", C.c_float * NKERNELS), ("in_bytes", C.c_uint64), ("out_bytes", C.c_uint64),
-                ("pixels", C.c_uint64), ("coef_bytes", C.c_uint64), ("n_images", C.c_uint32), ("n_failed", C.c_uint32), ("n_seq_decoded", C.c_uint32), ("n_par_fallback", C.c_uint32), ("n_par_short", C.c_uint32), ("n_prog_decoded", C.c_uint32), ("n_refine_chains", C.c_uint32), ("n_search_extra", C.c_uint32), ("n_fused_lists", C.c_uint32), ("n_list_refine", C.c_uint32), ("n_ac_in_lists", C.c_uint32), ("n_list_runs", C.c_uint32)]
+                ("pixels", C.c_uint64), ("coef_bytes", C.c_uint64), ("n_images", C.c_uint32), ("n_failed", C.c_uint32), ("n_seq_decoded", C.c_uint32), ("n_par_fallback", C.c_uint32), ("n_par_short", C.c_uint32), ("n_prog_decoded", C.c_uint32), ("n_refine_chains", C.c_uint32), ("n_search_extra", C.c_uint32), ("n_fused_lists", C.c_uint32), ("n_list_refine", C.c_uint32), ("n_ac_in_lists", C.c_uint32), ("n_list_runs", C.c_uint32), ("n_ref_packed", C.c_uint32)]
 
 
 class PngTiming(C.Structure):
diff --git a/caesium-clt_amd/csrc/batch.hpp b/caesium-clt_amd/csrc/batch.hpp
--- a/caesium-clt_amd/csrc/batch.hpp
+++ b/caesium-clt_amd/csrc/batch.hpp
@@ -97,6 +97,8 @@
     uint32_t nslots = 0, nlist_slots = 0, ntok_slots = 0;
     uint32_t nref_slots = 0;
     uint32_t last_run_refine = 0;
+    uint32_t last_run_ref_packed = 0;
+    bool ref_pack = true;
     uint32_t list_run = CSH_LIST_RUN;
     uint32_t nlist_runs = 0, nref_runs = 0;
     bool ac_runs_slot = false;
@@ -158,7 +160,7 @@
     DevBuf<uint64_t> d_corr, d_symbits, d_eobbits, d_tok_off, d_chunk_off, d_scan_raw_off;
     DevBuf<uint32_t> d_tok_cursor;
     DevBuf<TokRegion> d_regions;
-    DevBuf<uint16_t> d_eobrun, d_slot_hist;
+    DevBuf<uint16_t> d_eobrun, d_slot_hist, d_lastn;
     DevBuf<uint32_t> d_img_list, d_img_nlist, d_scan_cost, d_slot_raw, d_slot_eobh, d_long_runs, d_long_cnt, d_tokens, d_chunk_ntok, d_chunk_bits, d_raw, d_scan_pad, d_chunk_ff, d_hdr_off;
     DevBuf<DevEncTable> d_tables;
     DevBuf<NzList> d_nzlists;
@@ -281,6 +283,7 @@
     bool fused_420 = true;
     bool nz_fused = true;
     bool ref_list = true;
+    bool ref_pack = true;
     uint32_t list_run = CSH_LIST_RUN;
     bool ac_runs_slot = false;
     bool ac_tiles = false;
diff --git a/caesium-clt_amd/csrc/batch_plan.cpp b/caesium-clt_amd/csrc/batch_plan.cpp
--- a/caesium-clt_amd/csrc/batch_plan.cpp
+++ b/caesium-clt_amd/csrc/batch_plan.cpp
@@ -220,6 +220,7 @@
     s.nz_fused = !is("CSH_NZ_FUSED", "0");
     s.ac_tiles = is("CSH_AC_TILES", "1");
     s.ref_list = is("CSH_REF_LIST", "1") || (s.ref_list && !is("CSH_REF_LIST", "0"));
+    s.ref_pack = s.ref_list && (is("CSH_REF_PACK", "1") || (s.ref_pack && !is("CSH_REF_PACK", "0")));
     const char *pp = getenv("CSH_PROG_PAR");
     s.prog_par = pp && !strcmp(pp, "0") ? 0 : (pp && !strcmp(pp, "1") ? 1 : -1);
     s.fused_420 = !getenv("CSH_NO_FUSED_420");
@@ -250,6 +251,7 @@
     b->progressive = progressive;
     b->enc.list_run = sw.list_run;
     b->enc.ac_runs_slot = sw.ac_runs_slot;
+    b->enc.ref_pack = sw.ref_pack;
 
     add_script(b->enc.script, 3, true, CSH_CS_YCC);
     add_script(b->enc.script, 1, true, CSH_CS_GREY);
@@ -390,8 +392,11 @@
             const uint32_t nch = (w.nunits + 255) / 256;
             w.first_chunk = b->enc.nslots; b->enc.nslots += nch;
             w.hist_row0 = b->enc.hist_rows; b->enc.hist_rows += nch * uint32_t(e.ntables);
-            uint32_t &cursor = (from_list && w.list != 0xFFFFFFFFu) ? b->enc.nlist_slots : b->enc.ntok_slots;
-            w.ls_base = cursor; cursor += nch;
+            if (ref_list && sw.ref_pack && w.list != 0xFFFFFFFFu) w.ls_base = 0xFFFFFFFFu;
+            else {
+                uint32_t &cursor = (from_list && w.list != 0xFFFFFFFFu) ? b->enc.nlist_slots : b->enc.ntok_slots;
+                w.ls_base = cursor; cursor += nch;
+            }
             if (ref_list && w.list != 0xFFFFFFFFu) { w.rs_base = b->enc.nref_slots; b->enc.nref_slots += nch; }
             const uint32_t nruns = (nch + b->enc.list_run - 1) / b->enc.list_run;
             if (from_list && w.list != 0xFFFFFFFFu) { w.lr_base = b->enc.nlist_runs; b->enc.nlist_runs += nruns; }
@@ -425,6 +430,7 @@
         const uint64_t blocks_all = blocks_of(im);
         const uint64_t scripts = b->enc.search ? uint64_t(nac + 1) / 2 : 1;
         const uint64_t est = uint64_t(in_len) * 3 * scripts * nu / std::max<uint64_t>(1, blocks_all) + uint64_t(nu) * nac + 1024;
+        if (sw.ref_list && sw.ref_pack) continue;
         if (sw.ref_list) {
             for (size_t k = 0; k < list.size(); k++) {
                 const EncScan &e = b->enc.script[list[k]];
@@ -1120,7 +1126,7 @@
         return CS_ERR_NO_DEVICE;
     if (b->d_coef.alloc(size_t(b->ntiles) * CSH_TILE_I16) || b->pix.d_planes.alloc(b->pix.plane_bytes + 64) || b->pix.d_oplanes.alloc(b->pix.oplane_bytes + 64) ||
         b->enc.d_symbits.alloc(b->enc.total_words + 1) || b->enc.d_eobbits.alloc(b->enc.total_words + 1) ||
-        b->enc.d_long_runs.alloc(2 * (b->enc.total_units / 512 + b->enc.swork.size() + 16)) || b->enc.d_long_cnt.alloc(4) || b->enc.d_tail.alloc(b->enc.total_units + 1) || b->enc.d_eobrun.alloc(b->enc.total_units + 1) || b->enc.d_corr.alloc(b->enc.total_corr + 1) ||
+        b->enc.d_long_runs.alloc(2 * (b->enc.total_units / 512 + b->enc.swork.size() + 16)) || b->enc.d_long_cnt.alloc(4) || b->enc.d_tail.alloc(b->enc.total_units + 1) || b->enc.d_eobrun.alloc(b->enc.total_units + 1) || b->enc.d_corr.alloc(b->enc.total_corr + 1) || b->enc.d_lastn.alloc((b->enc.ref_pack ? b->enc.total_corr : 0) + 1) ||
         b->enc.d_tok_off.alloc(4 * size_t(b->enc.nslots) + 4) || b->enc.d_chunk_ntok.alloc(4 * size_t(b->enc.nslots) + 4) || b->enc.d_slot_hist.alloc(size_t(b->enc.hist_rows) * 256 + 256) ||
         b->enc.d_slot_raw.alloc(size_t(b->enc.nslots) + 1) || b->enc.d_img_list.upload(b->enc.img_list, st) || b->enc.d_img_nlist.upload(b->enc.img_nlist, st) || b->enc.d_scan_cost.alloc(b->enc.swork.size() + 1) || b->enc.d_slot_eobh.alloc(16 * size_t(b->enc.nslots) + 16) || b->enc.d_chunk_bits.alloc(size_t(b->enc.nslots) + 1) || b->enc.d_chunk_off.alloc(size_t(b->enc.nslots) + 2) || b->enc.d_tok_cursor.alloc(b->enc.region_est.size() + 1) || b->enc.d_regions.upload(b->enc.regions, st) ||
         b->enc.d_tables.alloc(b->enc.ntables) || b->enc.d_scan_pad.alloc(b->enc.swork.size() + 1) ||
diff --git a/caesium-clt_amd/csrc/batch_run.cpp b/caesium-clt_amd/csrc/batch_run.cpp
--- a/caesium-clt_amd/csrc/batch_run.cpp
+++ b/caesium-clt_amd/csrc/batch_run.cpp
@@ -208,7 +208,7 @@
         c.imgs = b->d_imgs.p; c.script = b->enc.d_script.p; c.work = b->enc.d_swork.p; c.nwork = int(b->enc.swork.size());
         c.echunks = b->enc.d_echunks.p; c.plans = b->enc.d_plans.p; c.nechunks = uint32_t(b->enc.echunks.size()); c.slot_work = b->enc.d_slot_work.p; c.slots = b->enc.d_slots.p; c.nslots = b->enc.nslots;
         c.coef = b->d_coef.p; c.sym_bits = b->enc.d_symbits.p; c.eob_bits = b->enc.d_eobbits.p; c.tail = b->enc.d_tail.p;
-        c.eobrun = b->enc.d_eobrun.p; c.long_runs = b->enc.d_long_runs.p; c.long_cnt = b->enc.d_long_cnt.p; c.corr = b->enc.d_corr.p;
+        c.eobrun = b->enc.d_eobrun.p; c.long_runs = b->enc.d_long_runs.p; c.long_cnt = b->enc.d_long_cnt.p; c.corr = b->enc.d_corr.p; c.lastn = b->enc.d_lastn.p; c.ref_pack = b->enc.ref_pack ? 1u : 0u;
         c.tokens = b->enc.d_tokens.p; c.regions = b->enc.d_regions.p; c.tok_cursor = b->enc.d_tok_cursor.p; c.tok_off = b->enc.d_tok_off.p; c.chunk_ntok = b->enc.d_chunk_ntok.p; c.slot_hist = b->enc.d_slot_hist.p; c.slot_raw = b->enc.d_slot_raw.p; c.slot_eobh = b->enc.d_slot_eobh.p;
         c.chunk_bits = b->enc.d_chunk_bits.p; c.chunk_off = b->enc.d_chunk_off.p; c.tables = b->enc.d_tables.p;
         c.raw = b->enc.d_raw.p; c.raw_words = raw_chunks * 16; c.status = b->out.d_status.p; c.overflow = b->out.d_overflow.p;
@@ -316,7 +316,7 @@
         SMARK(KS_NZLIST);
         launch_list_refine(st, c);
         for (uint32_t wi = sg.work0; sg.nrs && wi < sg.work0 + sg.nwork; wi++)
-            if (b->enc.swork[wi].rs_base != 0xFFFFFFFFu && (!gate || b->enc.work_active[wi])) b->enc.last_run_refine++;
+            if (b->enc.swork[wi].rs_base != 0xFFFFFFFFu && (!gate || b->enc.work_active[wi])) { b->enc.last_run_refine++; if (b->enc.ref_pack) b->enc.last_run_ref_packed++; }
         count_list_runs(sg, gate);
         launch_tokens(st, c);
         SMARK(KS_TOKENS);
@@ -336,6 +336,7 @@
         launch_zero_edges(st, c);
         SMARK(KS_SCAN_LAYOUT);
         launch_pack(st, c);
+        launch_list_refine_pack(st, c);
         SMARK(KS_PACK);
         launch_list_pack(st, c);
         SMARK(KS_LIST_PACK);
@@ -421,7 +422,7 @@
 int run_once(csh_batch *b, csh_timing *t, bool requant_only) {
     Run r(b, t);
     b->enc.last_run_list_runs = 0;
-    b->enc.last_run_fused = 0; b->enc.last_run_refine = 0; b->enc.last_run_ac_lists = 0;
+    b->enc.last_run_fused = 0; b->enc.last_run_refine = 0; b->enc.last_run_ref_packed = 0; b->enc.last_run_ac_lists = 0;
     if (r.pools() || r.marks.start()) return -1;
     const bool from_pixels = requant_only && b->tr.dering;
     if (requant_only && !from_pixels) {
diff --git a/caesium-clt_amd/csrc/k_aclist.hip b/caesium-clt_amd/csrc/k_aclist.hip
--- a/caesium-clt_amd/csrc/k_aclist.hip
+++ b/caesium-clt_amd/csrc/k_aclist.hip
@@ -1,5 +1,6 @@
 #include "kernels.h"
 #include "wave.h"
+#include "tok_bits.h"
 
 namespace csh {
 
@@ -558,6 +559,53 @@
         }
     }
 }
+template <class TL, class TN>
+__device__ __forceinline__ static uint32_t ref_step_tokens(const LV<uint32_t> (&e)[4], const LV<uint32_t> (&hex)[4], const LV<uint32_t> (&z)[4], const LV<uint32_t> (&zp)[4], LV<uint32_t> (&zq)[4],
+                                                           uint32_t Ss, uint32_t Se, const TL *lastn, const TN *nh, uint32_t &curc, uint32_t *tk, uint32_t at, uint32_t limit) {
+    LV<uint32_t> cur[4], nt;
+    LFOR(l) {
+        uint32_t s = 0;
+        CSH_UNROLL
+        for (int q = 0; q < 4; q++) {
+            const uint32_t v = e[q][l], blk = (v >> 23) & 255u, lastk = uint32_t(lastn[blk]) >> 6, isN = ref_isN(v, Ss, Se);
+            uint32_t nz = 0, n = 0;
+            if ((isN | ref_isH(v, Ss, Se)) && (v & 127u) <= lastk) { nz = ((z[q][l] - zp[q][l]) >> 4) - ((zq[q][l] - zp[q][l]) >> 4); n = nz + isN; }
+            cur[q][l] = n ? ((blk + 1u) << 6) | hex[q][l] : 0u;
+            if ((v & CSH_NZ_END) && lastk != Se) n = 1u;
+            zq[q][l] = nz | (n << 8);
+            s += n;
+        }
+        nt[l] = s;
+    }
+    lscan_last4(cur, curc);
+    uint32_t tot;
+    const LV<uint32_t> ex = lscan(nt, tot);
+    LFOR(l) {
+        uint32_t o = at + ex[l];
+        CSH_UNROLL
+        for (int q = 0; q < 4; q++) {
+            const uint32_t v = e[q][l], blk = (v >> 23) & 255u, nz = zq[q][l] & 255u, n = zq[q][l] >> 8;
+            if (!n) continue;
+            const uint32_t cu = ref_same(cur[q][l], blk);
+            if (v & CSH_NZ_END) {
+                if (o < limit) tk[o] = TK_EOB | (blk << 3) | ((uint32_t(nh[blk]) - cu) << 16) | (cu << 22);
+                o++;
+                continue;
+            }
+            uint32_t cnt = hex[q][l] - cu, from = cu;
+            for (uint32_t t = 0; t < nz; t++) {
+                if (o < limit) tk[o] = TK_REF | (blk << 3) | (cnt << 16) | (from << 22) | (1u << 28);
+                o++; cnt = 0u; from = hex[q][l];
+            }
+            if (n > nz) {
+                if (o < limit) tk[o] = TK_REF | (blk << 3) | (((z[q][l] - zp[q][l]) & 15u) << 11) | ((v & 128u) ? 0u : (1u << 15)) | (cnt << 16) | (from << 22);
+                o++;
+            }
+        }
+    }
+    return tot;
+}
+template <bool TOKENS>
 __global__ void __launch_bounds__(256, 5) k_list_refine(EncCtx c) {
     CSH_SHARED alignas(16) uint32_t s_hist[4][4][256];
     CSH_SHARED uint32_t s_lastn[4][256];
@@ -572,7 +620,9 @@
     const uint32_t nrun = run_chunks(c, r);
     const uint64_t lbase = c.nzlists[r.nzlist].base;
     ListSlot nx = list_chunk(c, lbase, r.nzrec);
-    const TokRegion rg = c.regions[r.region];
+    TokRegion rg;
+    rg.base = 0; rg.cap = 0; rg.pad = 0;
+    if (TOKENS) rg = c.regions[r.region];
     uint32_t *hist = &s_hist[wv][0][0], *lastn = s_lastn[wv], *nh = s_nh[wv], *corr = &s_corr[wv][0][0];
     LFOR(l) {
         uint4 zero; zero.x = zero.y = zero.z = zero.w = 0u;
@@ -629,6 +679,7 @@
                     if (ls.n && (ln >> 6) != Se) ntok[l] += 1u;
                     c.tail[unit0 + i] = uint8_t(nh[i] - (ln & 63u));
                     c.corr[corr0 + i] = (uint64_t(corr[2u * i]) << 32) | corr[2u * i + 1u];
+                    if (!TOKENS) c.lastn[corr0 + i] = uint16_t(ln);
                 }
             }
             const uint64_t ms = lballot([&](int b) { const uint32_t i = 64u * w4 + uint32_t(b); return i < nun && lastn[i] != 0u; });
@@ -638,7 +689,7 @@
         const uint32_t total = lsum32(ntok);
         hist_flush(hist, c.slot_hist + size_t(hist_row) * 256u, freq);
         LFOR(l) if (l == 0) c.slot_raw[cs] = C.runN + C.runH;
-        if (c.stats_only) continue;
+        if (c.stats_only || !TOKENS) continue;
         uint32_t rel = 0;
         LFOR(l) if (l == 0) rel = atomicAdd(&c.tok_cursor[r.region], total);
         rel = uni(rel);
@@ -652,56 +703,159 @@
         C.runH = C.runN = C.base = C.prevN = C.prevNZ = 0u;
         uint32_t curc = 0, at = 0;
         for (uint32_t g0 = 0; g0 < ls.n; g0 += 256) {
-            LV<uint32_t> e[4], hex[4], z[4], zp[4], zq[4], cur[4], nt;
+            LV<uint32_t> e[4], hex[4], z[4], zp[4], zq[4];
             LFOR(l) list_load4(ls, g0 + 4u * uint32_t(l), e[0][l], e[1][l], e[2][l], e[3][l]);
             ref_step<true>(e, Ss, Se, C, hex, z, zp, zq);
-            LFOR(l) {
-                uint32_t s = 0;
-                CSH_UNROLL
-                for (int q = 0; q < 4; q++) {
-                    const uint32_t v = e[q][l], blk = (v >> 23) & 255u, lastk = lastn[blk] >> 6, isN = ref_isN(v, Ss, Se);
-                    uint32_t nz = 0, n = 0;
-                    if ((isN | ref_isH(v, Ss, Se)) && (v & 127u) <= lastk) { nz = ((z[q][l] - zp[q][l]) >> 4) - ((zq[q][l] - zp[q][l]) >> 4); n = nz + isN; }
-                    cur[q][l] = n ? ((blk + 1u) << 6) | hex[q][l] : 0u;
-                    if ((v & CSH_NZ_END) && lastk != Se) n = 1u;
-                    zq[q][l] = nz | (n << 8);
-                    s += n;
-                }
-                nt[l] = s;
-            }
-            lscan_last4(cur, curc);
-            uint32_t tot;
-            const LV<uint32_t> ex = lscan(nt, tot);
-            LFOR(l) {
-                uint32_t o = at + ex[l];
-                CSH_UNROLL
-                for (int q = 0; q < 4; q++) {
-                    const uint32_t v = e[q][l], blk = (v >> 23) & 255u, nz = zq[q][l] & 255u, n = zq[q][l] >> 8;
-                    if (!n) continue;
-                    const uint32_t cu = ref_same(cur[q][l], blk);
-                    if (v & CSH_NZ_END) {
-                        if (o < total) tk[o] = TK_EOB | (blk << 3) | ((nh[blk] - cu) << 16) | (cu << 22);
-                        o++;
-                        continue;
-                    }
-                    uint32_t cnt = hex[q][l] - cu, from = cu;
-                    for (uint32_t t = 0; t < nz; t++) {
-                        if (o < total) tk[o] = TK_REF | (blk << 3) | (cnt << 16) | (from << 22) | (1u << 28);
-                        o++; cnt = 0u; from = hex[q][l];
-                    }
-                    if (n > nz) {
-                        if (o < total) tk[o] = TK_REF | (blk << 3) | (((z[q][l] - zp[q][l]) & 15u) << 11) | ((v & 128u) ? 0u : (1u << 15)) | (cnt << 16) | (from << 22);
-                        o++;
-                    }
-                }
-            }
-            at += tot;
+            at += ref_step_tokens(e, hex, z, zp, zq, Ss, Se, lastn, nh, curc, tk, at, total);
         }
 #ifdef CSH_EMUL
         if (at != total) { fprintf(stderr, "k_list_refine: pass 2 made %u tokens, pass 1 counted %u\n", at, total); abort(); }
 #endif
     }
     freq_flush(c.tables[r.table_base].freq, freq);
+}
+
+#define CSH_RP_TOKENS 704
+#define CSH_RP_SUB 64
+#define CSH_RP_WORDS 256
+#define CSH_RP_STEP 192
+__global__ void __launch_bounds__(256, 5) k_list_refine_pack(EncCtx c) {
+    CSH_SHARED alignas(16) uint32_t s_win[4][CSH_RP_WORDS];
+    CSH_SHARED uint32_t s_lut[4][256];
+    CSH_SHARED uint64_t s_corr[4][256];
+    CSH_SHARED uint16_t s_eob[4][256];
+    CSH_SHARED uint16_t s_lastn[4][256];
+    CSH_SHARED uint8_t s_nh[4][256];
+    CSH_SHARED uint32_t s_tok[4][CSH_RP_TOKENS];
+    const int wv = int(uni(uint32_t(lwave())));
+    const uint32_t idx = blockIdx.x * 4u + uint32_t(wv);
+    if (idx >= c.nref_runs) return;
+    const uint32_t cs0 = c.ref_runs[idx];
+    const SlotRec r = c.slots[cs0];
+    if (c.work_active && !c.work_active[r.work]) return;
+    const ScanWork &w = c.work[r.work];
+    if (w.no_room) { LFOR(l) if (l == 0) c.status[w.image] = 20200; return; }
+    const uint32_t nrun = run_chunks(c, r);
+    const uint64_t lbase = c.nzlists[r.nzlist].base;
+    ListSlot nx = list_chunk(c, lbase, r.nzrec);
+    const uint64_t scan0 = c.chunk_off[r.first_chunk];
+    const uint64_t raw_bit0 = w.raw_off * 8 + (c.chunk_off[cs0] - scan0);
+    uint32_t pad = 0;
+    if (r.j + nrun == r.nch) { const uint64_t total = c.chunk_off[r.first_chunk + r.nch] - scan0; pad = uint32_t((8 - (total & 7)) & 7); }
+    uint32_t *buf = s_win[wv], *lut = s_lut[wv];
+    uint64_t *corr = s_corr[wv];
+    uint16_t *eobrun = s_eob[wv], *lastn = s_lastn[wv];
+    uint8_t *nh = s_nh[wv];
+    uint32_t *tok = s_tok[wv];
+    LFOR(l) {
+        for (int i = l; i < 256; i += 64) lut[i] = c.tables[r.table_base].lut[i];
+        uint4 zero; zero.x = zero.y = zero.z = zero.w = 0u;
+        for (int i = 4 * l; i < CSH_RP_WORDS; i += 256) *reinterpret_cast<uint4 *>(buf + i) = zero;
+    }
+    CSP_WAVE_SYNC();
+    TokenCtx x;
+    x.lut = lut; x.lut_stride = 256; x.eobrun = eobrun; x.corr = corr;
+    uint32_t *out = c.raw + (raw_bit0 >> 5);
+    uint64_t pos = raw_bit0 & 31u;
+    uint32_t ww = 0;
+    bool first_flush = true;
+    const uint32_t Ss = r.Ss, Se = r.Se;
+    for (uint32_t ci = 0; ci < nrun; ci++) {
+        const ListSlot ls = nx;
+        const bool more = ci + 1u < nrun;
+        if (more) nx = list_chunk(c, lbase, r.nzrec + ci + 1u);
+#ifdef CSH_EMUL
+        {
+            const uint64_t want = (raw_bit0 & 31u) + (c.chunk_off[cs0 + ci] - c.chunk_off[cs0]);
+            if (c.overflow[1] ? pos > want : pos != want) { fprintf(stderr, "k_list_refine_pack: chunk %u of a run does not start where the one before it ended\n", ci); abort(); }
+        }
+#endif
+        CSP_WAVE_SYNC();
+        {
+            const uint32_t u0 = r.unit0 + 256u * ci, corr0 = r.corr0 + 256u * ci, left = r.nunits_work - 256u * (r.j + ci), nun = left < 256u ? left : 256u;
+            LFOR(l) for (int i = l; i < 256; i += 64) {
+                const bool in = uint32_t(i) < nun;
+                const uint32_t ln = in ? uint32_t(c.lastn[corr0 + uint32_t(i)]) : 0u;
+                eobrun[i] = in ? c.eobrun[u0 + uint32_t(i)] : uint16_t(0);
+                corr[i] = in ? c.corr[corr0 + uint32_t(i)] : uint64_t(0);
+                lastn[i] = uint16_t(ln);
+                nh[i] = in ? uint8_t(uint32_t(c.tail[u0 + uint32_t(i)]) + (ln & 63u)) : uint8_t(0);
+            }
+        }
+        CSP_WAVE_SYNC();
+        LV<uint32_t> xn[4];
+        LFOR(l) list_load4(ls, 4u * uint32_t(l), xn[0][l], xn[1][l], xn[2][l], xn[3][l]);
+        RefCarry C;
+        C.runH = C.runN = C.base = C.prevN = C.prevNZ = 0u;
+        uint32_t curc = 0;
+        for (uint32_t g0 = 0; g0 < ls.n; g0 += 256) {
+            uint32_t ntok;
+            {
+                LV<uint32_t> e[4], hex[4], z[4], zp[4], zq[4];
+                LFOR(l) { e[0][l] = xn[0][l]; e[1][l] = xn[1][l]; e[2][l] = xn[2][l]; e[3][l] = xn[3][l]; }
+                if (g0 + 256u < ls.n) LFOR(l) list_load4(ls, g0 + 256u + 4u * uint32_t(l), xn[0][l], xn[1][l], xn[2][l], xn[3][l]);
+                ref_step<true>(e, Ss, Se, C, hex, z, zp, zq);
+                ntok = ref_step_tokens(e, hex, z, zp, zq, Ss, Se, lastn, nh, curc, tok, 0u, uint32_t(CSH_RP_TOKENS));
+            }
+#ifdef CSH_EMUL
+            if (ntok > CSH_RP_TOKENS) { fprintf(stderr, "k_list_refine_pack: a step of %u tokens\n", ntok); abort(); }
+#endif
+            CSP_WAVE_SYNC();
+            for (uint32_t s0 = 0; s0 < ntok; s0 += CSH_RP_SUB) {
+                LV<uint32_t> t, pv[3], pn[3], slow, len;
+                LFOR(l) {
+                    const uint32_t i = s0 + uint32_t(l);
+                    t[l] = i < ntok ? tok[i] : uint32_t(TK_RAW);
+                    uint32_t v, n;
+                    slow[l] = token_main<2>(t[l], x, v, n) ? 0u : 1u;
+                    pv[0][l] = v; pn[0][l] = n; pv[1][l] = 0u; pn[1][l] = 0u; pv[2][l] = 0u; pn[2][l] = 0u;
+                }
+                if (lballot([&](int b) { return slow[b] != 0u; })) {
+                    LFOR(l) {
+                        const Pieces p = token_pieces<2>(t[l], x);
+                        CSH_UNROLL
+                        for (int k = 0; k < 3; k++) { pv[k][l] = p.v[k]; pn[k][l] = p.n[k]; }
+                    }
+                }
+                LFOR(l) len[l] = pn[0][l] + pn[1][l] + pn[2][l];
+                uint32_t tot;
+                const LV<uint32_t> ex = lscan(len, tot);
+                LFOR(l) {
+                    uint64_t at = pos + ex[l] - uint64_t(ww) * 32u;
+                    CSH_UNROLL
+                    for (int k = 0; k < 3; k++) if (pn[k][l]) { lor_bits(buf, at, pv[k][l], pn[k][l]); at += pn[k][l]; }
+                }
+                pos += tot;
+                const uint32_t done = uint32_t(pos >> 5) - ww;
+                if (done > CSH_RP_WORDS - CSH_RP_STEP) {
+                    CSP_WAVE_SYNC();
+                    LFOR(l) for (uint32_t q = uint32_t(l); q < done; q += 64) {
+                        const uint32_t v = buf[q];
+                        if (first_flush && q == 0) { if (v) atomicOr(out + ww, v); } else out[ww + q] = v;
+                    }
+                    const uint32_t partial = buf[done];
+                    CSP_WAVE_SYNC();
+                    LFOR(l) for (int q = l; q < CSH_RP_WORDS; q += 64) buf[q] = (q == 0) ? partial : 0u;
+                    CSP_WAVE_SYNC();
+                    ww += done; first_flush = false;
+                }
+            }
+            CSP_WAVE_SYNC();
+        }
+    }
+    if (pad) { LFOR(l) if (l == 0) lor_bits(buf, pos - uint64_t(ww) * 32u, (1u << pad) - 1u, pad); pos += pad; }
+#ifdef CSH_EMUL
+    {
+        const uint64_t want = (raw_bit0 & 31u) + (c.chunk_off[cs0 + nrun] - c.chunk_off[cs0]) + pad;
+        if (c.overflow[1] ? pos > want : pos != want) { fprintf(stderr, "k_list_refine_pack: a run does not end where its sizes say\n"); abort(); }
+    }
+#endif
+    CSP_WAVE_SYNC();
+    const uint32_t last = uint32_t((pos + 31) >> 5) - ww;
+    LFOR(l) for (uint32_t q = uint32_t(l); q < last; q += 64) {
+        const uint32_t v = buf[q];
+        if ((first_flush && q == 0) || q == last - 1) { if (v) atomicOr(out + ww + q, v); } else out[ww + q] = v;
+    }
 }
 
 __global__ void k_reset_works(ScanWork *work, int nwork) {
@@ -716,7 +870,12 @@
     if (c.nz_filter) CSH_LAUNCH(k_nzfilter, dim3(c.nnzchunks), dim3(CSP_WAVE_THREADS), st, c);
 }
 void launch_list_stats(hipStream_t st, const EncCtx &c) { if (c.nlist_runs) CSH_LAUNCH(k_list_stats, dim3((c.nlist_runs + 3) / 4), dim3(4 * CSP_WAVE_THREADS), st, c); }
-void launch_list_refine(hipStream_t st, const EncCtx &c) { if (c.nref_runs) CSH_LAUNCH(k_list_refine, dim3((c.nref_runs + 3) / 4), dim3(4 * CSP_WAVE_THREADS), st, c); }
+void launch_list_refine(hipStream_t st, const EncCtx &c) {
+    if (!c.nref_runs) return;
+    if (c.ref_pack) CSH_LAUNCH(k_list_refine<false>, dim3((c.nref_runs + 3) / 4), dim3(4 * CSP_WAVE_THREADS), st, c);
+    else CSH_LAUNCH(k_list_refine<true>, dim3((c.nref_runs + 3) / 4), dim3(4 * CSP_WAVE_THREADS), st, c);
+}
+void launch_list_refine_pack(hipStream_t st, const EncCtx &c) { if (c.nref_runs && c.ref_pack) CSH_LAUNCH(k_list_refine_pack, dim3((c.nref_runs + 3) / 4), dim3(4 * CSP_WAVE_THREADS), st, c); }
 void launch_list_pack(hipStream_t st, const EncCtx &c) { if (c.nlist_runs) CSH_LAUNCH(k_list_pack, dim3((c.nlist_runs + 3) / 4), dim3(4 * CSP_WAVE_THREADS), st, c); }
 __global__ void __launch_bounds__(64) k_make_slots(const ScanWork *works, uint32_t nworks, const EncScan *script, const NzList *nzlists, SlotRec *slots, uint32_t *slot_work, uint32_t *list_slots,
                                                    uint32_t *tok_slots, uint32_t *ref_slots, uint32_t *list_runs, uint32_t *ref_runs, uint32_t list_run) {
@@ -739,7 +898,7 @@
         r.nzlist = has_list ? w.list : 0u; r.nzrec = has_list ? nzlists[w.list].chunk0 + j : 0u; r.region = ref_list ? w.region : 0u;
         slots[w.first_chunk + j] = r;
         slot_work[w.first_chunk + j] = wi;
-        (listed ? list_slots : tok_slots)[w.ls_base + j] = w.first_chunk + j;
+        if (w.ls_base != 0xFFFFFFFFu) (listed ? list_slots : tok_slots)[w.ls_base + j] = w.first_chunk + j;
         if (ref_list) ref_slots[w.rs_base + j] = w.first_chunk + j;
         if (listed && j % list_run == 0u) list_runs[w.lr_base + j / list_run] = w.first_chunk + j;
         if (ref_list && j % list_run == 0u) ref_runs[w.rr_base + j / list_run] = w.first_chunk + j;
diff --git a/caesium-clt_amd/csrc/k_entropy.hip b/caesium-clt_amd/csrc/k_entropy.hip
--- a/caesium-clt_amd/csrc/k_entropy.hip
+++ b/caesium-clt_amd/csrc/k_entropy.hip
@@ -1,5 +1,6 @@
 #include "kernels.h"
 #include "wave.h"
+#include "tok_bits.h"
 
 namespace csh {
 
@@ -846,60 +847,6 @@
     if (ntables) CSH_LAUNCH(k_gen_tables, dim3((ntables + 3) / 4), dim3(4 * CSP_WAVE_THREADS), st, tables, ntables);
 }
 
-struct Pieces { uint32_t v[3], n[3]; };
-struct TokenCtx {
-    const uint32_t *lut;
-    uint32_t lut_stride;
-    const uint16_t *eobrun;
-    const uint64_t *corr;
-};
-#define CSH_LUT_STRIDE uint32_t(sizeof(DevEncTable) / 4)
-__device__ __forceinline__ static void corr_pieces(Pieces &p, uint64_t corr, uint32_t t) {
-    const uint32_t cnt = (t >> 16) & 63u, cur = (t >> 22) & 63u;
-    if (!cnt) return;
-    const uint64_t bits = (corr << cur) >> (64u - cnt);
-    if (cnt > 32) { p.v[1] = uint32_t(bits >> 32); p.n[1] = cnt - 32; p.v[2] = uint32_t(bits); p.n[2] = 32; }
-    else { p.v[2] = uint32_t(bits); p.n[2] = cnt; }
-}
-template <int MODE = 0>
-__device__ __forceinline__ static Pieces token_pieces(uint32_t t, const TokenCtx &x) {
-    Pieces p;
-    p.v[0] = p.v[1] = p.v[2] = 0; p.n[0] = p.n[1] = p.n[2] = 0;
-    uint32_t kind = t & 7u;
-    if (MODE == 1) { if (kind == TK_RAW) return p; kind = kind == TK_ACF ? uint32_t(TK_ACF) : uint32_t(TK_EOB); }
-    if (MODE == 2) { if (kind == TK_RAW) return p; kind = kind == TK_REF ? uint32_t(TK_REF) : uint32_t(TK_EOB); }
-    if (MODE == 3) kind = kind == TK_SYM ? uint32_t(TK_SYM) : uint32_t(TK_RAW);
-    if (kind == TK_SYM) {
-        const uint32_t e = x.lut[((t >> 11) & 3u) * x.lut_stride + ((t >> 3) & 255u)], nr = (t >> 13) & 15u;
-        p.v[0] = ((e & 0xFFFFu) << nr) | (t >> 17); p.n[0] = (e >> 16) + nr;
-    } else if (kind == TK_RAW) { p.v[0] = t >> 17; p.n[0] = (t >> 13) & 15u; }
-    else if (kind == TK_ACF) {
-        const uint32_t r = (t >> 3) & 63u, nb = (t >> 9) & 15u, zr = r >> 4;
-        if (zr) {
-            const uint32_t z = x.lut[0xF0], zc = z & 0xFFFFu, zl = z >> 16;
-            p.v[0] = zc; p.n[0] = zl;
-            if (zr > 1) { p.v[0] = (zc << zl) | zc; p.n[0] = 2 * zl; }
-            if (zr > 2) { p.v[1] = zc; p.n[1] = zl; }
-        }
-        const uint32_t e = x.lut[((r & 15u) << 4) | nb];
-        p.v[2] = ((e & 0xFFFFu) << nb) | ((t >> 13) & 0xFFFFu); p.n[2] = (e >> 16) + nb;
-    } else if (kind == TK_REF) {
-        const uint32_t unit = (t >> 3) & 255u;
-        if (t & (1u << 28)) { const uint32_t e = x.lut[0xF0]; p.v[0] = e & 0xFFFFu; p.n[0] = e >> 16; }
-        else { const uint32_t e = x.lut[(((t >> 11) & 15u) << 4) | 1u]; p.v[0] = ((e & 0xFFFFu) << 1) | ((t >> 15) & 1u); p.n[0] = (e >> 16) + 1; }
-        if ((t >> 16) & 63u) corr_pieces(p, x.corr[unit], t);
-    } else {
-        const uint32_t unit = (t >> 3) & 255u;
-        const uint32_t run = x.eobrun[unit];
-        if (run) {
-            const int nb = bitlen32(run) - 1;
-            const uint32_t e = x.lut[nb << 4];
-            p.v[0] = ((e & 0xFFFFu) << nb) | (run & ((1u << nb) - 1u)); p.n[0] = (e >> 16) + uint32_t(nb);
-        }
-        if ((t >> 16) & 63u) corr_pieces(p, x.corr[unit], t);
-    }
-    return p;
-}
 __device__ __forceinline__ static TokenCtx token_ctx(const EncCtx &c, const SlotRec &r) {
     TokenCtx x;
     x.lut = c.tables[r.table_base].lut; x.lut_stride = CSH_LUT_STRIDE;
@@ -947,43 +894,6 @@
     if (lo) atomicOr(words + (pos >> 5) + 1, lo);
 }
 #define CSH_WAVE_FENCE() do { __builtin_amdgcn_fence(__ATOMIC_ACQ_REL, "wavefront"); __builtin_amdgcn_wave_barrier(); } while (0)
-template <int MODE>
-__device__ __forceinline__ static bool token_main(uint32_t t, const TokenCtx &x, uint32_t &v, uint32_t &n) {
-    v = 0; n = 0;
-    const uint32_t kind = t & 7u;
-    if (kind == TK_RAW) { v = t >> 17; n = (t >> 13) & 15u; return true; }
-    if (MODE == 3) {
-        const uint32_t e = x.lut[((t >> 11) & 3u) * x.lut_stride + ((t >> 3) & 255u)], nr = (t >> 13) & 15u;
-        v = ((e & 0xFFFFu) << nr) | (t >> 17); n = (e >> 16) + nr;
-        return true;
-    }
-    if (MODE == 1 && kind == TK_ACF) {
-        const uint32_t r = (t >> 3) & 63u, nb = (t >> 9) & 15u;
-        if (r >> 4) return false;
-        const uint32_t e = x.lut[(r << 4) | nb];
-        v = ((e & 0xFFFFu) << nb) | ((t >> 13) & 0xFFFFu); n = (e >> 16) + nb;
-        return true;
-    }
-    const uint32_t unit = (t >> 3) & 255u, cnt = (t >> 16) & 63u, cur = (t >> 22) & 63u;
-    if (MODE == 2 && kind == TK_REF) {
-        if (t & (1u << 28)) { const uint32_t e = x.lut[0xF0]; v = e & 0xFFFFu; n = e >> 16; }
-        else { const uint32_t e = x.lut[(((t >> 11) & 15u) << 4) | 1u]; v = ((e & 0xFFFFu) << 1) | ((t >> 15) & 1u); n = (e >> 16) + 1; }
-    } else {
-        const uint32_t run = x.eobrun[unit];
-        if (run) {
-            const int nb = bitlen32(run) - 1;
-            const uint32_t e = x.lut[nb << 4];
-            v = ((e & 0xFFFFu) << nb) | (run & ((1u << nb) - 1u)); n = (e >> 16) + uint32_t(nb);
-        }
-    }
-    if (MODE == 2 && cnt) {
-        if (n + cnt > 32) return false;
-        const uint32_t bits = uint32_t((x.corr[unit] << cur) >> (64u - cnt));
-        v = (n ? (v << cnt) : 0u) | bits; n += cnt;
-    }
-    return true;
-}
-
 #ifndef CSH_EMUL
 struct PackState { uint32_t *buf, *out; uint64_t pos; uint32_t ww; bool first_flush; };
 template <int MODE>
diff --git a/caesium-clt_amd/csrc/kernels.h b/caesium-clt_amd/csrc/kernels.h
--- a/caesium-clt_amd/csrc/kernels.h
+++ b/caesium-clt_amd/csrc/kernels.h
@@ -151,6 +151,8 @@
     const uint32_t *ref_runs;
     uint32_t nref_runs;
     uint32_t list_run;
+    uint16_t *lastn;
+    uint32_t ref_pack;
     uint32_t ac_runs_slot;
     uint32_t nz_build, nz_filter;
 };
@@ -165,6 +167,7 @@
 void launch_list_stats(hipStream_t st, const EncCtx &c);
 void launch_list_refine(hipStream_t st, const EncCtx &c);
 void launch_list_pack(hipStream_t st, const EncCtx &c);
+void launch_list_refine_pack(hipStream_t st, const EncCtx &c);
 void launch_nz_to_tiles(hipStream_t st, const NzSet *nzsets, const NzList *nzlists, const uint32_t *nz_pool, const uint32_t *nz_chunk_off, const uint32_t *nz_chunk_cnt,
                         uint32_t set, uint32_t nchunks, int16_t *coef);
 void launch_reset_works(hipStream_t st, ScanWork *work, int nwork);
diff --git a/caesium-clt_amd/csrc/pipeline.cpp b/caesium-clt_amd/csrc/pipeline.cpp
--- a/caesium-clt_amd/csrc/pipeline.cpp
+++ b/caesium-clt_amd/csrc/pipeline.cpp
@@ -251,6 +251,7 @@
         t->n_list_refine = b->enc.last_run_refine;
         t->n_ac_in_lists = b->enc.last_run_ac_lists;
         t->n_list_runs = b->enc.last_run_list_runs;
+        t->n_ref_packed = b->enc.last_run_ref_packed;
         for (const Item &it : b->items) if (it.image < 0) t->n_failed++;
         for (int i = 0; i < b->nimg; i++) { t->out_bytes += b->out.h_img_size[i]; t->pixels += uint64_t(b->imgs[i].width) * b->imgs[i].height; }
         t->in_bytes = b->dec.bits_pool.size();
diff --git a/caesium-clt_amd/csrc/tok_bits.h b/caesium-clt_amd/csrc/tok_bits.h
--- /dev/null
+++ b/caesium-clt_amd/csrc/tok_bits.h
@@ -0,0 +1,97 @@
+#pragma once
+#include "kernels.h"
+
+namespace csh {
+
+struct Pieces { uint32_t v[3], n[3]; };
+struct TokenCtx {
+    const uint32_t *lut;
+    uint32_t lut_stride;
+    const uint16_t *eobrun;
+    const uint64_t *corr;
+};
+#define CSH_LUT_STRIDE uint32_t(sizeof(DevEncTable) / 4)
+__device__ __forceinline__ static void corr_pieces(Pieces &p, uint64_t corr, uint32_t t) {
+    const uint32_t cnt = (t >> 16) & 63u, cur = (t >> 22) & 63u;
+    if (!cnt) return;
+    const uint64_t bits = (corr << cur) >> (64u - cnt);
+    if (cnt > 32) { p.v[1] = uint32_t(bits >> 32); p.n[1] = cnt - 32; p.v[2] = uint32_t(bits); p.n[2] = 32; }
+    else { p.v[2] = uint32_t(bits); p.n[2] = cnt; }
+}
+template <int MODE = 0>
+__device__ __forceinline__ static Pieces token_pieces(uint32_t t, const TokenCtx &x) {
+    Pieces p;
+    p.v[0] = p.v[1] = p.v[2] = 0; p.n[0] = p.n[1] = p.n[2] = 0;
+    uint32_t kind = t & 7u;
+    if (MODE == 1) { if (kind == TK_RAW) return p; kind = kind == TK_ACF ? uint32_t(TK_ACF) : uint32_t(TK_EOB); }
+    if (MODE == 2) { if (kind == TK_RAW) return p; kind = kind == TK_REF ? uint32_t(TK_REF) : uint32_t(TK_EOB); }
+    if (MODE == 3) kind = kind == TK_SYM ? uint32_t(TK_SYM) : uint32_t(TK_RAW);
+    if (kind == TK_SYM) {
+        const uint32_t e = x.lut[((t >> 11) & 3u) * x.lut_stride + ((t >> 3) & 255u)], nr = (t >> 13) & 15u;
+        p.v[0] = ((e & 0xFFFFu) << nr) | (t >> 17); p.n[0] = (e >> 16) + nr;
+    } else if (kind == TK_RAW) { p.v[0] = t >> 17; p.n[0] = (t >> 13) & 15u; }
+    else if (kind == TK_ACF) {
+        const uint32_t r = (t >> 3) & 63u, nb = (t >> 9) & 15u, zr = r >> 4;
+        if (zr) {
+            const uint32_t z = x.lut[0xF0], zc = z & 0xFFFFu, zl = z >> 16;
+            p.v[0] = zc; p.n[0] = zl;
+            if (zr > 1) { p.v[0] = (zc << zl) | zc; p.n[0] = 2 * zl; }
+            if (zr > 2) { p.v[1] = zc; p.n[1] = zl; }
+        }
+        const uint32_t e = x.lut[((r & 15u) << 4) | nb];
+        p.v[2] = ((e & 0xFFFFu) << nb) | ((t >> 13) & 0xFFFFu); p.n[2] = (e >> 16) + nb;
+    } else if (kind == TK_REF) {
+        const uint32_t unit = (t >> 3) & 255u;
+        if (t & (1u << 28)) { const uint32_t e = x.lut[0xF0]; p.v[0] = e & 0xFFFFu; p.n[0] = e >> 16; }
+        else { const uint32_t e = x.lut[(((t >> 11) & 15u) << 4) | 1u]; p.v[0] = ((e & 0xFFFFu) << 1) | ((t >> 15) & 1u); p.n[0] = (e >> 16) + 1; }
+        if ((t >> 16) & 63u) corr_pieces(p, x.corr[unit], t);
+    } else {
+        const uint32_t unit = (t >> 3) & 255u;
+        const uint32_t run = x.eobrun[unit];
+        if (run) {
+            const uint32_t nb = 31u - uint32_t(__clz(run));
+            const uint32_t e = x.lut[nb << 4];
+            p.v[0] = ((e & 0xFFFFu) << nb) | (run & ((1u << nb) - 1u)); p.n[0] = (e >> 16) + nb;
+        }
+        if ((t >> 16) & 63u) corr_pieces(p, x.corr[unit], t);
+    }
+    return p;
+}
+template <int MODE>
+__device__ __forceinline__ static bool token_main(uint32_t t, const TokenCtx &x, uint32_t &v, uint32_t &n) {
+    v = 0; n = 0;
+    const uint32_t kind = t & 7u;
+    if (kind == TK_RAW) { v = t >> 17; n = (t >> 13) & 15u; return true; }
+    if (MODE == 3) {
+        const uint32_t e = x.lut[((t >> 11) & 3u) * x.lut_stride + ((t >> 3) & 255u)], nr = (t >> 13) & 15u;
+        v = ((e & 0xFFFFu) << nr) | (t >> 17); n = (e >> 16) + nr;
+        return true;
+    }
+    if (MODE == 1 && kind == TK_ACF) {
+        const uint32_t r = (t >> 3) & 63u, nb = (t >> 9) & 15u;
+        if (r >> 4) return false;
+        const uint32_t e = x.lut[(r << 4) | nb];
+        v = ((e & 0xFFFFu) << nb) | ((t >> 13) & 0xFFFFu); n = (e >> 16) + nb;
+        return true;
+    }
+    const uint32_t unit = (t >> 3) & 255u, cnt = (t >> 16) & 63u, cur = (t >> 22) & 63u;
+    if (MODE == 2 && kind == TK_REF) {
+        if (t & (1u << 28)) { const uint32_t e = x.lut[0xF0]; v = e & 0xFFFFu; n = e >> 16; }
+        else { const uint32_t e = x.lut[(((t >> 11) & 15u) << 4) | 1u]; v = ((e & 0xFFFFu) << 1) | ((t >> 15) & 1u); n = (e >> 16) + 1; }
+    } else {
+        const uint32_t run = x.eobrun[unit];
+        if (run) {
+            const uint32_t nb = 31u - uint32_t(__clz(run));
+            const uint32_t e = x.lut[nb << 4];
+            v = ((e & 0xFFFFu) << nb) | (run & ((1u << nb) - 1u)); n = (e >> 16) + nb;
+        }
+    }
+    if (MODE == 2 && cnt) {
+        if (n + cnt > 32) return false;
+        const uint32_t bits = uint32_t((x.corr[unit] << cur) >> (64u - cnt));
+        v = (n ? (v << cnt) : 0u) | bits; n += cnt;
+    }
+    return true;
+}
+
+}
diff --git a/include/caesium_hip.h b/include/caesium_hip.h
--- a/include/caesium_hip.h
+++ b/include/caesium_hip.h
@@ -93,6 +93,7 @@
     uint32_t n_list_refine;
     uint32_t n_ac_in_lists;
     uint32_t n_list_runs;
+    uint32_t n_ref_packed;
 } csh_timing;
 
 int csh_device_count(void);
```

After: 45510 (median of 6 runs). 1.01x the previous value.
